# ilya16/isp-tts

Hardware: AMD Instinct MI355X
Metric: mel-frames/s (whole node), batch=64 x 512-frame utterances per GPU, full forward incl. MAS (higher is better)
Workload: dtype bf16; 1 GPU; BASELINE config 3: AcousticModel.forward (TextEncoder + Aligner/MAS + TemporalAdaptor 1 flow eval + MelDecoder + to_mel), fixed-length synthetic random-phoneme batch, random-init weights of the recipe architecture (23.2 M params); batch_per_gpu=64, global_batch=64, text_len=100, mel_len=512, parallelism=single GPU, device=gfx950:sramecc+:xnack-, compute_units=256, launch=HIP graph replay, batches_in_flight=1

## Files before the change

### include/ispk.h

```cpp
#ifndef ISPK_H
#define ISPK_H

#include <stdint.h>

#ifdef __cplusplus
extern "C" {
#endif

typedef struct ihipStream_t* ispk_stream_t;

#define ISPK_ABI_VERSION 2

#define ISPK_E_NULL (-1)
#define ISPK_E_SHAPE (-2)
#define ISPK_E_ALIGN (-3)
#define ISPK_E_UNSUPPORTED (-4)

int32_t ispk_abi_version(void);
const char* ispk_last_error_string(void);
int32_t ispk_device_info(char* name, int32_t cap);

int32_t ispk_mas_f32(const float* logits, const int64_t* text_len, const int64_t* mel_len, int16_t* attn_hard,
                     int64_t* dur, int16_t* path, int32_t B, int32_t M_max, int32_t L_max, int64_t stride_b,
                     int64_t stride_m, ispk_stream_t stream);
// ... 12 lines not shown
#define ISPK_EP_MASK_ACC 4u
#define ISPK_EP_MASK_OUT 8u
#define ISPK_EP_BIAS_ROW 16u
#define ISPK_EP_MASK_COL 32u
#define ISPK_EP_OUT_BF16 64u
#define ISPK_EP_RESID_BF16 128u
#define ISPK_EP_DUAL_GELU 1024u
#define ISPK_EP_GELU_BWD 2048u
#define ISPK_EP_OUT_SPLIT 512u
#define ISPK_EP_ROWS_T 256u

int32_t ispk_gemm_f32_tile(int32_t M, int32_t N, int32_t K);
int32_t ispk_gemm_f32(const float* A, int64_t lda, const float* W, int64_t ldw, float* C, int64_t ldc, const float* bias,
                      const float* resid, int64_t ldr, const uint8_t* mask, int32_t M, int32_t N, int32_t K,
                      uint32_t flags, int32_t cols_per_batch, int64_t batch_stride, ispk_stream_t stream);
int32_t ispk_gemm_f32_batched(const float* A, int64_t lda, int64_t stride_a, const float* W, int64_t ldw, int64_t stride_w,
                              float* C, int64_t ldc, int64_t stride_c, int32_t batch, int32_t M, int32_t N, int32_t K,
                              ispk_stream_t stream);
int32_t ispk_gemm_bf16_gelu_train(const uint16_t* A, int64_t lda, const uint16_t* W, int64_t ldw, uint16_t* u, int64_t ldu,
                                  uint16_t* a, int64_t ld_a, int32_t M, int32_t N, int32_t K, float dropout_p, uint64_t seed,
                                  ispk_stream_t stream);
int32_t ispk_gemm_bf16_gelu_bwd(const uint16_t* dY, int64_t lddy, const uint16_t* W2t, int64_t ldw, const uint16_t* u,
                                int64_t ldu, uint16_t* du, int64_t lddu, const uint8_t* row_mask, int32_t M, int32_t N,
                                int32_t K, float dropout_p, uint64_t seed, ispk_stream_t stream);
int32_t ispk_gemm_bf16_last_variant(void);
int32_t ispk_gemm_bf16(const uint16_t* A, int64_t lda, const uint16_t* W, int64_t ldw, void* C, int64_t ldc,
                       const float* bias, const void* resid, int64_t ldr, const uint8_t* mask, int32_t M, int32_t N,
                       int32_t K, uint32_t flags, int32_t cols_per_batch, int64_t batch_stride, ispk_stream_t stream);
int32_t ispk_gemm_bf16_splitk_plan(int32_t M, int32_t N, int32_t K, uint32_t flags);
int32_t ispk_gemm_bf16_splitk(const uint16_t* A, int64_t lda, const uint16_t* W, int64_t ldw, void* C, int64_t ldc,
                              const float* bias, const void* resid, int64_t ldr, const uint8_t* mask, int32_t M, int32_t N,
                              int32_t K, uint32_t flags, float* workspace, int32_t ksplit, ispk_stream_t stream);

int32_t ispk_ffn_bf16(const uint16_t* x, int64_t ldx, const uint16_t* W1, int64_t ldw1, const float* bias1,
                      const uint16_t* W2, int64_t ldw2, const float* bias2, const float* resid, int64_t ldr,
                      const uint8_t* mask, float* out, int64_t ldo, int32_t rows, int32_t dim, int32_t inner, uint32_t flags,
                      ispk_stream_t stream);

int32_t ispk_ffn_bf16_prenorm(const float* x, int64_t ldx, const float* norm_gamma, const float* norm_beta, float norm_eps,
                              const uint16_t* W1, int64_t ldw1, const uint16_t* W2_packed, const float* bias2,
                              const uint8_t* mask, float* out, int64_t ldo, int32_t rows, int32_t dim, int32_t inner,
                              uint32_t flags, float* row_stats, float stats_eps, ispk_stream_t stream);

int32_t ispk_ffn_chunk_w2_bf16(const uint16_t* W2, int64_t ldw2, int32_t dim, int32_t inner, uint16_t* out,
                               ispk_stream_t stream);
int32_t ispk_ffn_bf16_prenorm2_split(const float* x, int64_t ldx, const float* norm_gamma, const float* norm_beta,
                                     float norm_eps, const uint16_t* W1, const uint16_t* W2_chunks, float* parts,
                                     int64_t part_stride, int32_t splits, int32_t rows, int32_t dim, int32_t inner,
                                     ispk_stream_t stream);
int32_t ispk_ffn_combine_ln_f32(const float* x, int64_t ldx, const float* parts, int64_t part_stride, int32_t splits,
                                const uint8_t* mask, float* y, int64_t ldy, const float* ln_gamma, const float* ln_beta,
                                float ln_eps, int32_t ln_mask, void* ln_out, int64_t ld_ln, int32_t ln_bf16, int32_t rows,
                                int32_t dim, ispk_stream_t stream);
int32_t ispk_ffn_bf16_prenorm2(const float* x, int64_t ldx, const float* norm_gamma, const float* norm_beta, float norm_eps,
                               const uint16_t* W1, const uint16_t* W2_chunks, const uint8_t* mask, float* out, int64_t ldo,
                               int32_t rows, int32_t dim, int32_t inner, uint32_t flags, float* row_stats, float stats_eps,
                               ispk_stream_t stream);
int32_t ispk_attn_out_ffn_bf16(const float* x, int64_t ldx, const uint16_t* attn_out, int64_t ld_attn,
                               const uint16_t* Wo_chunks, const float* norm_gamma, const float* norm_beta, float norm_eps,
                               const uint16_t* W1, const uint16_t* W2_chunks, const uint8_t* mask, float* out, int64_t ldo,
                               int32_t rows, int32_t dim, int32_t inner, uint32_t flags, float* row_stats, float stats_eps,
                               ispk_stream_t stream);

int32_t ispk_attn_out_ffn_norm_bf16(const float* x, int64_t ldx, const uint16_t* attn_out, int64_t ld_attn,
                                    const uint16_t* Wo_chunks, const float* norm_gamma, const float* norm_beta, float norm_eps,
                                    const uint16_t* W1, const uint16_t* W2_chunks, const uint8_t* mask, float* out, int64_t ldo,
                                    int32_t rows, int32_t dim, int32_t inner, uint32_t flags, const float* final_gamma,
                                    const float* final_beta, float final_eps, int32_t ln_mask, void* ln_out, int64_t ld_ln,
                                    int32_t ln_bf16, ispk_stream_t stream);
int32_t ispk_attn_out_ffn_split_bf16(const float* x, int64_t ldx, const uint16_t* attn_out, int64_t ld_attn,
                                     const uint16_t* Wo_chunks, const float* norm_gamma, const float* norm_beta, float norm_eps,
                                     const uint16_t* W1, const uint16_t* W2_chunks, const uint8_t* mask, uint32_t flags,
                                     float* parts, int64_t part_stride, int32_t splits, int32_t rows, int32_t dim, int32_t inner,
                                     ispk_stream_t stream);
int32_t ispk_chunk_k16_bf16(const uint16_t* W, int64_t ldw, int32_t N, int32_t K, uint16_t* out, ispk_stream_t stream);
int32_t ispk_attn_out_ffn_qkv_bf16(const float* x, int64_t ldx, const uint16_t* attn_out, int64_t ld_attn,
                                   const uint16_t* Wo_chunks, const float* norm_gamma, const float* norm_beta, float norm_eps,
                                   const uint16_t* W1, const uint16_t* W2_chunks, const uint8_t* mask, float* out, int64_t ldo,
                                   int32_t rows, int32_t dim, int32_t inner, uint32_t flags, const float* next_gamma,
                                   const float* next_beta, float next_eps, const uint16_t* Wqkv_chunks, uint16_t* qkv,
                                   int64_t ld_qkv, ispk_stream_t stream);

int32_t ispk_gemm_bf16_lnin(const float* x, int64_t ldx, const float* row_stats, const float* ln_gamma, const float* ln_beta,
                            float ln_eps, const uint16_t* W, int64_t ldw, void* C, int64_t ldc, const float* bias, const void* resid,
                            int64_t ldr, const uint8_t* mask, int32_t M, int32_t N, int32_t K, uint32_t flags,
                            ispk_stream_t stream);

int32_t ispk_ffn_pack_w2_bf16(const uint16_t* W2, int64_t ldw2, int32_t dim, int32_t inner, uint16_t* packed,
                              ispk_stream_t stream);

int32_t ispk_linear_small_f32(const float* a, int64_t lda, const float* w, int64_t ldw, const float* bias,
                              const float* resid, int64_t ldr, float* out, int64_t ldo, int32_t M, int32_t N, int32_t K,
                              uint32_t act, ispk_stream_t stream);

int32_t ispk_alibi_mqa_attn_f32(const float* q, int64_t ldq, const float* k, const float* v, int64_t ldkv,
                                const float* slopes, const int64_t* key_len, float* out, int64_t ldo, int32_t B,
                                int32_t N, int32_t H, ispk_stream_t stream);
int32_t ispk_alibi_mqa_attn_bf16(const uint16_t* q, int64_t ldq, const uint16_t* k, const uint16_t* v, int64_t ldkv,
                                 const float* slopes, const int64_t* key_len, uint16_t* out, int64_t ldo, int32_t B,
                                 int32_t N, int32_t H, ispk_stream_t stream);
int32_t ispk_alibi_mqa_attn_bf16_tiles(const uint16_t* q, int64_t ldq, const uint16_t* k, const uint16_t* v, int64_t ldkv,
                                       const float* slopes, const int64_t* key_len, uint16_t* out, int64_t ldo, int32_t B,
                                       int32_t N, int32_t H, int32_t q_tiles_per_workgroup, ispk_stream_t stream);

int32_t ispk_attn_block_short_bf16(const uint16_t* x, int64_t ldx, const uint16_t* Wqkv_chunks, uint16_t* qkv, int64_t ld_qkv,
                                   const float* slopes, const int64_t* key_len, const uint16_t* Wo_chunks, const float* resid,
                                   int64_t ldr, const uint8_t* mask, float* out, int64_t ldo, int32_t B, int32_t N, int32_t H,
                                   ispk_stream_t stream);

int32_t ispk_pad_rows_f32(const float* x, int64_t stride_b, int64_t stride_t, int64_t stride_c, const int64_t* len,
                          void* out, int32_t out_bf16, int32_t B, int32_t T, int32_t C, ispk_stream_t stream);
int32_t ispk_masked_instnorm_f32(const float* y, const float* weight, const float* bias, const int64_t* len, void* out,
                                 int32_t out_bf16, int32_t B, int32_t T, int32_t C, float eps, ispk_stream_t stream);
int32_t ispk_aligner_scores_f32(const float* q_enc, int64_t q_stride_b, const float* k_enc, int64_t k_stride_b,
                                const int64_t* text_len, const int64_t* mel_len, float* attn_logits, float* attn_soft,
                                int32_t B, int32_t M, int32_t L, int32_t D, ispk_stream_t stream);
int32_t ispk_aligner_scores_fast_f32(const float* q_enc, int64_t q_stride_b, const float* k_enc, int64_t k_stride_b,
                                const int64_t* text_len, const int64_t* mel_len, float* attn_logits, float* attn_soft,
                                int32_t B, int32_t M, int32_t L, int32_t D, ispk_stream_t stream);
int32_t ispk_soft_average_f32(const float* attn_soft, const float* pitch, const float* energy, const int64_t* duration,
                              const int64_t* text_len, float* feats, int32_t B, int32_t M, int32_t L,
                              ispk_stream_t stream);

int32_t ispk_flow_head_f32(const float* y, int64_t ldy, const float* norm_gamma, const float* norm_beta, float norm_eps,
                           const float* W, const float* bias, const float* flow, const float* x0, const uint8_t* mask,
                           float* pred, float* duration, float* loss_ratio, float* loss_mean, float* workspace, int32_t B,
                           int32_t L, int32_t D, int32_t C, ispk_stream_t stream);
int32_t ispk_flow_euler_f32(const float* x_t, const float* velocity, float dt, const uint8_t* mask, float* out, int32_t B,
                            int32_t L, int32_t C, ispk_stream_t stream);
int32_t ispk_infer_features_f32(const float* pred, const float* duration_target_f32, const int64_t* duration_target_i64,
                                const float* pitch_target, const float* energy_target, float duration_factor, float pitch_factor,
                                float pitch_delta, float energy_factor, float energy_delta, float* duration, float* features,
                                int32_t B, int32_t L, ispk_stream_t stream);
int32_t ispk_infer_features_round_f32(const float* pred, const float* duration_target_f32, const int64_t* duration_target_i64,
                                      const float* pitch_target, const float* energy_target, float duration_factor,
                                      float pitch_factor, float pitch_delta, float energy_factor, float energy_delta,
                                      float* duration, float* features, int32_t B, int32_t L, ispk_stream_t stream);
int32_t ispk_infer_features_items_f32(const float* pred, const float* duration_target_f32, const int64_t* duration_target_i64,
                                      const float* pitch_target, const float* energy_target, const float* controls,
                                      int32_t round, float* duration, float* features, int64_t* frames_wanted, int32_t B,
                                      int32_t L, ispk_stream_t stream);
int32_t ispk_infer_features_tokens_f32(const float* pred, const float* duration_target_f32, const int64_t* duration_target_i64,
                                       const float* pitch_target, const float* energy_target, const float* controls,
                                       int32_t round, float* duration, float* features, int64_t* frames_wanted, int32_t B,
                                       int32_t L, ispk_stream_t stream);
int32_t ispk_flow_mix_f32(const float* x0, const float* x1, const float* t, float sigma, float* x_t, float* flow, int32_t B,
                          int32_t L, int32_t C, ispk_stream_t stream);
int32_t ispk_flow_finish_f32(const float* pred_raw, const float* flow, const float* x0, const uint8_t* mask, float* pred,
                             float* duration, float* loss_ratio, float* loss_mean, int32_t B, int32_t L, int32_t C,
                             ispk_stream_t stream);

int32_t ispk_embed_tokens_f32(const int64_t* text, const float* table, int64_t ld_table, int32_t vocab,
                              const int64_t* text_len, float* emb, uint8_t* mask, int32_t B, int32_t L, int32_t D,
                              ispk_stream_t stream);
int32_t ispk_embed_tokens_qkv(const int64_t* text, const float* table, int64_t ld_table, int32_t vocab, const int64_t* text_len,
                              float* emb, uint8_t* mask, const uint16_t* qkv_table, int64_t ld_qkv_table, uint16_t* qkv,
                              int32_t B, int32_t L, int32_t D, int32_t N, ispk_stream_t stream);
int32_t ispk_add_speaker_f32(float* x, const float* table, int64_t ld_table, int32_t speakers, const int64_t* speaker,
                             int32_t id_stride, int32_t B, int32_t L, int32_t D, ispk_stream_t stream);
int32_t ispk_add_speaker_out_f32(const float* x, float* out, const float* table, int64_t ld_table, int32_t speakers,
                                 const int64_t* speaker, int32_t id_stride, int32_t B, int32_t L, int32_t D, ispk_stream_t stream);
int32_t ispk_speaker_grad_f32(const float* d_x, const int64_t* speaker, int32_t id_stride, const int64_t* text_len,
                              float* workspace, int64_t workspace_floats, float* d_table, int64_t ld_table, int32_t speakers,
                              int32_t B, int32_t L, int32_t D, int32_t accumulate, ispk_stream_t stream);
int32_t ispk_time_embedding_f32(const float* t, int32_t n, const float* inv_freq, const float* freq_scale, int32_t half_dim,
                                const float* w0, const float* b0, const float* w1, const float* b1, int32_t emb_dim,
                                float* out, ispk_stream_t stream);
int32_t ispk_length_regulate_f32(const float* alignment, const float* dur_f32, const int64_t* dur_i64, const int64_t* enc_len,
                                 const float* x, int64_t ldx, float* out, int64_t* dec_len, uint8_t* dec_mask, int32_t B,
                                 int32_t M, int32_t L, int32_t D, int32_t max_len, int32_t dur_cols, ispk_stream_t stream);
int32_t ispk_length_regulate_split_bf16(const float* alignment, const float* dur_f32, const int64_t* dur_i64, const int64_t* enc_len,
                                 const float* x, int64_t ldx, float* out, int64_t* dec_len, uint8_t* dec_mask, int32_t B,
                                 int32_t M, int32_t L, int32_t D, int32_t max_len, int32_t dur_cols, ispk_stream_t stream);
int32_t ispk_length_regulate_qkv_bf16(const float* alignment, const float* dur_f32, const int64_t* dur_i64, const int64_t* enc_len,
                                      const float* x, int64_t ldx, float* out, int64_t* dec_len, uint8_t* dec_mask,
                                      const float* norm_gamma, const float* norm_beta, float norm_eps, const uint16_t* Wqkv_chunks,
                                      uint16_t* qkv, int64_t ld_qkv, int32_t B, int32_t M, int32_t L, int32_t D, int32_t max_len,
                                      int32_t dur_cols, ispk_stream_t stream);
int32_t ispk_length_regulate_split_f16(const float* alignment, const float* dur_f32, const int64_t* dur_i64, const int64_t* enc_len,
                                const float* x, int64_t ldx, float* out, int64_t* dec_len, uint8_t* dec_mask, int32_t B,
                                int32_t M, int32_t L, int32_t D, int32_t max_len, int32_t dur_cols, ispk_stream_t stream);

int32_t ispk_hard_regulate_f32(const float* dur_f32, const int64_t* dur_i64, const float* x, int64_t ldx, float* out,
                               int64_t* dec_len, uint8_t* dec_mask, int32_t B, int32_t frames, int32_t L, int32_t D,
                               int32_t max_len, ispk_stream_t stream);
int32_t ispk_hard_regulate_bwd_f32(const float* dur_f32, const int64_t* dur_i64, const float* d_out, float* d_x, int32_t B,
                                   int32_t rows, int32_t L, int32_t D, int32_t max_len, ispk_stream_t stream);
int32_t ispk_hard_average_f32(const float* pitch, const float* energy, const int64_t* duration, const int64_t* text_len,
                              float* feats, int32_t B, int32_t M, int32_t L, ispk_stream_t stream);

int32_t ispk_transpose_f32(const float* x, int64_t ldx, float* y, int64_t ldy, int32_t rows, int32_t cols,
                           ispk_stream_t stream);
int32_t ispk_gemm_tn_f32(const float* A, int64_t lda, const float* B, int64_t ldb, float* C, int64_t ldc, int32_t M,
                         int32_t N1, int32_t N2, const uint8_t* row_mask, int32_t accumulate, float* workspace,
                         int64_t workspace_floats, ispk_stream_t stream);
int32_t ispk_gemm_tn_bf16(const float* A, int64_t lda, const float* B, int64_t ldb, float* C, int64_t ldc, int32_t M,
                          int32_t N1, int32_t N2, const uint8_t* row_mask, int32_t accumulate, float* workspace,
                          int64_t workspace_floats, ispk_stream_t stream);
int32_t ispk_gemm_tn_b16(const uint16_t* A, int64_t lda, const uint16_t* B, int64_t ldb, float* C, int64_t ldc, int32_t M,
                         int32_t N1, int32_t N2, const uint8_t* row_mask, int32_t accumulate, float* workspace,
// ... 229 lines not shown
```

### isp_tts_amd/acoustic/alignment.py

```python
from __future__ import annotations

from collections.abc import Sequence
from typing import NamedTuple, Optional

import torch
import torch.nn as nn
from torch import Tensor

from .. import runtime
from ..staging import StagedWeights
from ..modules.aligner import mas_device
from ..modules.constructor import Constructor


_NOT_A_PATH = ("{} only owns parameters (the reference's state_dict names); its arithmetic runs inside the fused HIP "
               "kernels that ConvAttention launches (csrc/aligner.hip) - there is no PyTorch/MIOpen path to fall back to")


class MaskedInstanceNorm1d(nn.Module):

    def __init__(self, num_features: int, eps: float = 1e-5):
        super().__init__()
        self.eps = eps
        self.weight = nn.Parameter(torch.ones(num_features))
# ... 22 lines not shown


class ConvAttention(nn.Module, Constructor):
    def __init__(self, mel_dim: int, text_dim: int = 512, attention_dim: int = 80, key_kernel_size: int = 3,
                 query_kernel_size=(3, 3), dropout: float = 0.0, normalization: Optional[str] = "instance",
                 activation: str = "relu", attention_prior: bool = True):
        super().__init__()
        self.mel_dim, self.text_dim = mel_dim, text_dim
        self.scale = attention_dim ** -0.5
        if isinstance(query_kernel_size, int):
            query_kernel_size = [query_kernel_size] * 2
        self.key_proj = nn.ModuleList([
            ConvBlock1D(text_dim, text_dim * 2, key_kernel_size, activation, normalization, bias=False),
            ConvBlock1D(text_dim * 2, attention_dim, 1, "linear", None, bias=False)])
        self.query_proj = nn.ModuleList([
            ConvBlock1D(mel_dim, mel_dim * 2, query_kernel_size[0], activation, normalization, bias=False),
            ConvBlock1D(mel_dim * 2, mel_dim, query_kernel_size[1], activation, normalization, bias=False),
            ConvBlock1D(mel_dim, attention_dim, 1, "linear", None, bias=False)])
        self.attention_prior = attention_prior
        self.compute_dtype = torch.float32
        self._cache = StagedWeights()

    def _staged(self):
        ps = [c.conv.weight for c in list(self.key_proj) + list(self.query_proj)]
        dt = self.compute_dtype

        def build():
            if dt == torch.float16:
                w2d = [runtime.split_f16(p.detach().permute(0, 2, 1).reshape(p.shape[0], -1).float().contiguous()) for p in ps]
            else:
                w2d = [p.detach().permute(0, 2, 1).reshape(p.shape[0], -1).to(dt).contiguous() for p in ps]
            return w2d[:2], w2d[2:]
        return self._cache.get(dt, ps, build)

    def project_queries(self, queries: Tensor, query_len: Tensor) -> Tensor:
        _, wq = self._staged()
        gelu, dt = runtime.EP_GELU, self.compute_dtype
        if dt == torch.float16:
            q = runtime.pad_rows(queries.float(), query_len, channel_first=True, out_dtype=dt)
            for i in (0, 1):
                q = runtime.conv5_padded_split(q, wq[i], gelu)
                q = runtime.masked_instnorm(q, self.query_proj[i].norm.weight, self.query_proj[i].norm.bias, query_len,
                                            out_dtype=dt)
            return runtime.conv5_padded_split(q, wq[2])
        q = runtime.pad_rows(queries.float(), query_len, channel_first=True, out_dtype=dt)
        q = runtime.conv5_padded(q, wq[0], gelu)
        q = runtime.masked_instnorm(q, self.query_proj[0].norm.weight, self.query_proj[0].norm.bias, query_len,
                                    out_dtype=dt)
        q = runtime.conv5_padded(q, wq[1], gelu)
        q = runtime.masked_instnorm(q, self.query_proj[1].norm.weight, self.query_proj[1].norm.bias, query_len,
                                    out_dtype=dt)
        return runtime.conv5_padded(q, wq[2])

    def forward(self, queries: Tensor, keys: Tensor, query_len: Tensor, key_len: Tensor, q_proj: Optional[Tensor] = None):
        if not self.attention_prior:
            raise NotImplementedError("the aligner is built with its diagonal prior (recipes: attention_prior default)")
        wk, _ = self._staged()
        max_q, max_k = queries.shape[2], keys.shape[2]
        gelu, dt = runtime.EP_GELU, self.compute_dtype
        if dt == torch.float16:
            k = runtime.pad_rows(keys.float(), key_len, channel_first=True, out_dtype=dt)
            k = runtime.conv5_padded_split(k, wk[0], gelu)
            k = runtime.masked_instnorm(k, self.key_proj[0].norm.weight, self.key_proj[0].norm.bias, key_len, out_dtype=dt)
            k = runtime.conv5_padded_split(k, wk[1])
            q = q_proj if q_proj is not None else self.project_queries(queries, query_len)
            return runtime.aligner_scores(q, k, key_len, query_len, max_q, max_k)
        k = runtime.pad_rows(keys.float(), key_len, channel_first=True, out_dtype=dt)
        k = runtime.conv5_padded(k, wk[0], gelu)
        k = runtime.masked_instnorm(k, self.key_proj[0].norm.weight, self.key_proj[0].norm.bias, key_len, out_dtype=dt)
        k = runtime.conv5_padded(k, wk[1])
        q = q_proj if q_proj is not None else self.project_queries(queries, query_len)
        return runtime.aligner_scores(q, k, key_len, query_len, max_q, max_k, fast=dt == torch.bfloat16)


class AlignerOutput(NamedTuple):
    attn_soft: Tensor
    attn_logits: Tensor
    attn_hard: Tensor
    attn_hard_duration: Tensor


class Aligner(nn.Module, Constructor):
    def __init__(self, mel_dim: int, text_dim: int = 512, attention_dim: int = 80, key_kernel_size: int = 3,
                 query_kernel_size=(3, 3), dropout: float = 0.0, normalization: Optional[str] = "instance",
                 activation: str = "relu", attention_prior: bool = True):
        super().__init__()
        self.attention = ConvAttention(mel_dim=mel_dim, text_dim=text_dim, attention_dim=attention_dim,
                                       key_kernel_size=key_kernel_size, query_kernel_size=query_kernel_size,
                                       dropout=dropout, normalization=normalization, activation=activation,
                                       attention_prior=attention_prior)

    def forward(self, mel: Tensor, enc_text: Tensor, mel_len: Tensor, text_len: Tensor,
                q_proj: Optional[Tensor] = None, mas_stream=None) -> AlignerOutput:
        attn_soft, attn_logits = self.attention(mel, enc_text, mel_len, text_len, q_proj=q_proj)
        if mas_stream is not None and attn_logits.is_cuda:
            mas_stream.wait_stream(torch.cuda.current_stream())
            with torch.cuda.stream(mas_stream):
                attn_hard, dur = self.binarize_attention_parallel(attn_logits, text_len, mel_len, return_duration=True)
            attn_logits.record_stream(mas_stream)
        else:
            attn_hard, dur = self.binarize_attention_parallel(attn_logits, text_len, mel_len, return_duration=True)
        return AlignerOutput(attn_soft=attn_soft, attn_logits=attn_logits, attn_hard=attn_hard, attn_hard_duration=dur)

    @torch.no_grad()
    def binarize_attention_parallel(self, attn_logits: Tensor, text_len: Tensor, mel_len: Tensor,
                                    return_duration: bool = False):
        hard, dur, _ = mas_device(attn_logits.detach(), text_len, mel_len, want_dur=return_duration)
        return (hard, dur) if return_duration else hard
```

### isp_tts_amd/acoustic/model.py

```python
from __future__ import annotations

import warnings
from typing import NamedTuple, Optional

import torch
import torch.nn as nn
import torch.nn.functional as F
from torch import Tensor

from .. import runtime
from ..staging import StagedWeights
from ..modules.constructor import Constructor
from ..modules.transformer import Transformer
from ..modules.transformer.plan import Hand, Handed
from ..utils import get_mask_from_lengths
from .alignment import Aligner, AlignerOutput
from .temporal_adaptor import FlowTemporalAdaptor, TemporalAdaptorOutput


class AcousticModelOutput(NamedTuple):
    mel: Tensor
    adaptor_output: TemporalAdaptorOutput
    aligner_output: AlignerOutput
    loss: Optional[Tensor] = None
    losses: Optional[dict] = None


class AcousticModel(nn.Module, Constructor):
    def __init__(self, encoding_map: dict, mel_dim: int, text_dim: int = 384, encoder=None, decoder=None,
                 temporal_adaptor=None, aligner=None, num_speakers: Optional[int] = 0, pitch_mean=None, pitch_std=None,
                 speaker_in_forward: bool = False):
        super().__init__()
        self.encoding_map = dict(encoding_map)
        self.mel_dim, self.text_dim = mel_dim, text_dim
        self.text_embedding = nn.Embedding(len(encoding_map), text_dim, padding_idx=0)
        self.encoder = Transformer.init(encoder, emb_dim=text_dim)
        enc_dim = self.encoder.dim
        self.aligner = Aligner.init(aligner, mel_dim=mel_dim, text_dim=enc_dim)
        self.speaker_embedding = None
        if (num_speakers or 0) > 0:
            self.speaker_embedding = nn.Embedding(num_speakers, enc_dim)
            nn.init.xavier_uniform_(self.speaker_embedding.weight)
        self.speaker_in_forward = bool(speaker_in_forward)
        self.train_amp: Optional[bool] = None
        self.temporal_adaptor = FlowTemporalAdaptor.init(temporal_adaptor, encoder_dim=enc_dim)
        self.decoder = Transformer.init(decoder, emb_dim=enc_dim)
        self.to_mel = nn.Linear(self.decoder.dim, mel_dim)
        self.token_qkv_table = True
        self.overlap_streams = True
        self._side_streams: dict = {}
        self.register_buffer("pitch_mean", torch.tensor(float(pitch_mean or 0.)))
        self.register_buffer("pitch_std", torch.tensor(float(pitch_std or 1.)))
        self.compute_dtype = torch.float32
        self._cache = StagedWeights()

    def set_compute_dtype(self, dtype: torch.dtype, *, alignment_dtype: Optional[torch.dtype] = None):
        chain = alignment_dtype if alignment_dtype is not None else dtype
        assert chain in (torch.float32, torch.bfloat16, torch.float16)
        self.encoder.set_compute_dtype(chain)
        self.decoder.set_compute_dtype(dtype)
        self.temporal_adaptor.predictor.transformer.set_compute_dtype(dtype)
        self.temporal_adaptor.embedding.transformer.set_compute_dtype(dtype)
        self.aligner.attention.compute_dtype = chain
        self.temporal_adaptor.length_regulator.split_bf16 = (True if dtype == torch.bfloat16 else
                                                             "f16" if dtype == torch.float16 else False)
        self.compute_dtype = dtype
        return self

    def _to_mel(self, dec_out: Tensor, dec_mask: Optional[Tensor]) -> Tensor:
        w = self.to_mel.weight
        if dec_out.dtype == torch.float16:
            ws = self._cache.get(torch.float16, (w,), lambda: runtime.split_f16(w.detach().float().contiguous()))
            return runtime.to_mel_split(dec_out, ws, self.to_mel.bias, dec_mask)
        if dec_out.dtype == torch.bfloat16:
            w = self._cache.get(torch.bfloat16, (w,), lambda: w.detach().to(torch.bfloat16).contiguous())
        return runtime.to_mel(dec_out, w, self.to_mel.bias, dec_mask)

    def _embed(self, text: Tensor, text_len: Optional[Tensor], want_mask: bool = True):
        table, enc = self.text_embedding.weight, self.encoder
        first = enc.layers[0]
        norm, att = first.attention_norm, first.attention
        if not (self.token_qkv_table and text.is_cuda and att.compute_dtype == torch.bfloat16 and not first.adaptive_norm
                and norm.weight is not None and norm.bias is not None and isinstance(enc.project_emb, nn.Identity)
                and (att.heads * 64 + 128) % 8 == 0):
            return (*runtime.embed_tokens(text, table, text_len, want_mask=want_mask), Handed())

        def build():
            with torch.no_grad():
                rows = runtime.layernorm(table.detach().float().contiguous(), norm.weight, norm.bias, eps=norm.eps,
                                         out_dtype=torch.bfloat16)
                return runtime.gemm(rows, att._staged(torch.bfloat16)[0])
        qkv_table = self._cache.get("token_qkv", (table, norm.weight, norm.bias, att.to_q.weight, att.to_kv.weight), build)
        emb, mask, qkv = runtime.embed_tokens_qkv(text, table, qkv_table, text_len, want_mask=want_mask)
        return emb, mask, Handed(Hand.QKV, qkv)

    def _decoder_first(self):
        dec = self.decoder
        first = dec.layers[0]
        norm, att = first.attention_norm, first.attention
        ok = (att.compute_dtype == torch.bfloat16 and not first.adaptive_norm and norm.weight is not None and norm.bias is not None
              and isinstance(dec.project_emb, nn.Identity) and dec.dim == 384 and att.heads * 64 + 128 == 512)
        return first if ok else None

    def _decoder_handed(self) -> Handed:
        qkv = self.temporal_adaptor.length_regulator.qkv
        return Handed(Hand.QKV, qkv) if qkv is not None else Handed()

    def forward(self, text: Tensor, text_len: Tensor, mel: Tensor, mel_len: Tensor, pitch: Optional[Tensor] = None,
                energy: Optional[Tensor] = None, speaker: Optional[Tensor] = None, sigma: float = 0., steps: int = 1, *,
                flow_noise: Optional[Tensor] = None, flow_time: Optional[Tensor] = None) -> AcousticModelOutput:
        if self.speaker_embedding is None:
            speaker = None
        elif not self.speaker_in_forward:
            raise AttributeError(f"'{type(self).__name__}' object has no attribute 'speaker_encoder'")
        elif speaker is None:
            raise ValueError("speaker_in_forward is on and the model has a speaker table: forward() needs `speaker` "
                             "([B, 1] int64 ids, or a single id for the whole batch)")
        if torch.is_grad_enabled() and text.is_cuda and any(p.requires_grad for p in self.parameters()):
            from ..train.model import acoustic_train_outputs
            amp = self.train_amp if self.train_amp is not None else torch.is_autocast_enabled("cuda")
            train_aligner = any(p.requires_grad for p in self.aligner.parameters())
            with torch.autocast("cuda", enabled=False):
                return acoustic_train_outputs(self, text, text_len, mel, mel_len, pitch, energy, flow_noise, flow_time, amp=amp,
                                              train_aligner=train_aligner, speaker=speaker)
        with torch.no_grad():
            return self._forward_values(text, text_len, mel, mel_len, pitch, energy, flow_noise=flow_noise, flow_time=flow_time,
                                        speaker=speaker)

    def _forward_values(self, text: Tensor, text_len: Tensor, mel: Tensor, mel_len: Tensor, pitch: Optional[Tensor] = None,
                        energy: Optional[Tensor] = None, *, flow_noise: Optional[Tensor] = None,
                        flow_time: Optional[Tensor] = None, speaker: Optional[Tensor] = None) -> AcousticModelOutput:
        q_proj = None
        if mel.is_cuda and self.overlap_streams:
            main = torch.cuda.current_stream()
            side = self._side_streams.setdefault(mel.device, torch.cuda.Stream(device=mel.device))
            side.wait_stream(main)
            with torch.cuda.stream(side):
                q_proj = self.aligner.attention.project_queries(mel, mel_len)
        token_emb, enc_mask, handed = self._embed(text, text_len)
        enc_out = self.encoder(token_emb, mask=enc_mask, key_len=text_len, handed=handed).out
        if q_proj is not None:
            main.wait_stream(side)
            q_proj.record_stream(main)
        branch = side if q_proj is not None else None
        hard = not self.temporal_adaptor.soft_duration
        aligner_output = self.aligner(mel=mel, enc_text=enc_out.transpose(1, 2).detach(), mel_len=mel_len,
                                      text_len=text_len, q_proj=q_proj, mas_stream=None if hard else branch)
        if speaker is not None:
            enc_out = runtime.add_speaker(enc_out, self.speaker_embedding.weight, speaker)
        adaptor_output = self.temporal_adaptor(
            enc_out=enc_out, enc_mask=enc_mask, max_dec_len=mel.size(2),
            duration_target=aligner_output.attn_hard_duration, alignment=aligner_output.attn_soft,
            pitch_target_dense=pitch, energy_target_dense=energy, noise=flow_noise, time_steps=flow_time,
            enc_len=text_len, predictor_stream=branch, duration_sum=mel_len if branch is not None and not hard else None,
            qkv_for=self._decoder_first())
        dec_len = adaptor_output.dec_lengths
        dec_mask = adaptor_output.dec_mask
        dec_out = self.decoder(adaptor_output.enc_out, mask=dec_mask, key_len=dec_len, out_dtype=self.compute_dtype,
                               handed=self._decoder_handed()).out
        mel_out = self._to_mel(dec_out, dec_mask)
        if q_proj is not None:
            main.wait_stream(side)
            for t in (adaptor_output.log_duration, adaptor_output.duration, adaptor_output.pitch, adaptor_output.energy,
                      aligner_output.attn_hard, aligner_output.attn_hard_duration, *(adaptor_output.losses or {}).values()):
                if isinstance(t, Tensor):
                    t.record_stream(main)
        return AcousticModelOutput(mel=mel_out, adaptor_output=adaptor_output, aligner_output=aligner_output)

    @torch.no_grad()
    def forward_front(self, text: Tensor, text_len: Tensor, mel: Tensor, mel_len: Tensor, pitch: Tensor, energy: Tensor):
        main = torch.cuda.current_stream()
        side = self._side_streams.setdefault(mel.device, torch.cuda.Stream(device=mel.device))
        side.wait_stream(main)
        with torch.cuda.stream(side):
            q_proj = self.aligner.attention.project_queries(mel, mel_len)
        token_emb, enc_mask, handed = self._embed(text, text_len)
        enc_out = self.encoder(token_emb, mask=enc_mask, key_len=text_len, handed=handed).out
        main.wait_stream(side)
        q_proj.record_stream(main)
        attn_soft, attn_logits = self.aligner.attention(mel, enc_out.transpose(1, 2).detach(), mel_len, text_len,
                                                        q_proj=q_proj)
        feats = runtime.soft_average(attn_soft, pitch, energy, None, text_len)
        return {"enc_out": enc_out, "enc_mask": enc_mask, "attn_soft": attn_soft, "attn_logits": attn_logits, "feats": feats}

    @torch.no_grad()
    def forward_side(self, st: dict, text_len: Tensor, mel_len: Tensor, pitch: Tensor, energy: Tensor,
                     flow_noise: Optional[Tensor], flow_time: Optional[Tensor]):
        attn_hard, dur = self.aligner.binarize_attention_parallel(st["attn_logits"], text_len, mel_len, return_duration=True)
        ad = self.temporal_adaptor
        targets = runtime.soft_average(st["attn_soft"], pitch, energy, dur, text_len)
        pred, losses = ad.predictor(st["enc_out"], targets, st["enc_mask"][..., None], noise=flow_noise, time_steps=flow_time,
                                    key_len=text_len)
        return {"attn_hard": attn_hard, "dur": dur, "pred": pred, "losses": losses,
                "duration_pred": ad.predictor._duration_estimate}

    @torch.no_grad()
    def forward_back(self, st: dict, text_len: Tensor, mel_len: Tensor, max_dec_len: int):
        ad = self.temporal_adaptor
        feats = st["feats"]
        x = ad.embedding(feats[..., 1:3], mask=st["enc_mask"][..., None], key_len=text_len, residual=st["enc_out"])
        dec_in, dec_len = ad.length_regulator(x, mel_len.view(-1, 1), max_len=max_dec_len, alignment=st["attn_soft"],
                                              qkv_for=self._decoder_first())
        dec_mask = ad.length_regulator.dec_mask
        dec_out = self.decoder(dec_in, mask=dec_mask, key_len=dec_len, out_dtype=self.compute_dtype,
                               handed=self._decoder_handed()).out
        return {"mel": self._to_mel(dec_out, dec_mask), "dec_in": dec_in, "dec_len": dec_len, "dec_mask": dec_mask}

    @staticmethod
# ... 97 lines not shown
```

### isp_tts_amd/acoustic/temporal_adaptor.py

```python
from __future__ import annotations

from typing import NamedTuple, Optional

import torch
import torch.nn as nn
import torch.nn.functional as F
from torch import Tensor

from .. import runtime
from ..staging import StagedWeights
from ..modules.constructor import Constructor
from ..modules.transformer import Transformer, TimePositionalEmbedding
from ..utils import get_float_mask_from_lengths, get_mask_3d, masked_mean


class TransformerTemporalModule(nn.Module, Constructor):

    def __init__(self, input_dim: int = 256, output_dim: int = 256, transformer=None, detach_inputs: bool = False):
        super().__init__()
        self.transformer = Transformer.init(transformer, emb_dim=input_dim)
        for layer in self.transformer.layers:
            layer.attention.short_block = False
        self.linear_layer = nn.Linear(self.transformer.dim, output_dim, bias=True)
        self.detach_inputs = detach_inputs
        self._cache = StagedWeights()

    def _weight(self, dtype: torch.dtype) -> Tensor:
        w = self.linear_layer.weight
        if dtype == torch.float16:
            return self._cache.get(dtype, (w,), lambda: runtime.split_f16(w.detach().float().contiguous()))
        return self._cache.get(dtype, (w,), lambda: w.detach().to(dtype).contiguous())

    def forward(self, x: Tensor, mask: Optional[Tensor] = None, *, key_len: Optional[Tensor] = None,
                residual: Optional[Tensor] = None) -> Tensor:
        m2 = mask[..., 0] if mask is not None else None
        cdt = self.transformer.layers[0].attention.compute_dtype
        out = self.transformer(x, mask=m2, out_dtype=cdt, key_len=key_len if m2 is not None else None).out
        flags = runtime.EP_MASK_ACC if m2 is not None else 0
        if cdt == torch.float16:
            return runtime.gemm_split(out, self._weight(cdt), bias=self.linear_layer.bias, mask=m2, flags=flags, resid=residual)
        return runtime.gemm(out, self._weight(cdt), bias=self.linear_layer.bias, mask=m2, flags=flags, resid=residual,
                            out_dtype=torch.float32)

    def infer(self, x: Tensor, mask: Optional[Tensor] = None, steps: int = 4) -> Tensor:
        return self.forward(x, mask)


class FlowTransformerTemporalModule(nn.Module, Constructor):

    def __init__(self, input_dim: int = 256, output_dim: int = 256, transformer=None,
                 time_embedding_dim: Optional[int] = None, sigma: float = 1e-5, detach_inputs: bool = False):
        super().__init__()
        time_embedding_dim = time_embedding_dim or input_dim
        self.time_embedding = TimePositionalEmbedding(freq_dim=64, emb_dim=time_embedding_dim, with_steps=True)
        self.transformer = Transformer.init(transformer, emb_dim=output_dim + input_dim, adaptive_norm=True,
                                            condition_dim=time_embedding_dim)
        self.linear_layer = nn.Linear(self.transformer.dim, output_dim, bias=True)
        self.output_dim, self.sigma, self.detach_inputs = output_dim, sigma, detach_inputs
        self.fused_head = True
        self._cache = StagedWeights()
        self._grids: dict = {}

    def _cond_weight(self, dtype: torch.dtype) -> Tensor:
        w = self.transformer.project_emb.weight
        if dtype == torch.float16:
            return self._cache.get(dtype, (w,), lambda: runtime.split_f16(w.detach()[:, self.output_dim:].float().contiguous()))
        return self._cache.get(dtype, (w,), lambda: w.detach()[:, self.output_dim:].to(dtype).contiguous())

    def _project(self, x_t: Tensor, cond_proj: Tensor) -> Tensor:
        w = self.transformer.project_emb.weight
        return runtime.linear_small(x_t.contiguous(), w[:, :self.output_dim], None, resid=cond_proj)

    def _cond_projection(self, cond: Tensor) -> Tensor:
        cdt = self.transformer.layers[0].attention.compute_dtype
        c = cond.float().contiguous()
        if cdt == torch.float16:
            return runtime.gemm_split(runtime.split_f16(c), self._cond_weight(cdt), bias=self.transformer.project_emb.bias)
        if cdt == torch.bfloat16:
            c = runtime.cast_bf16(c)
        return runtime.gemm(c, self._cond_weight(cdt), bias=self.transformer.project_emb.bias, out_dtype=torch.float32)

    def forward(self, x: Tensor, targets: Tensor, mask: Optional[Tensor] = None, *, noise: Optional[Tensor] = None,
                time_steps: Optional[Tensor] = None, key_len: Optional[Tensor] = None):
        cond = x
        have_mask = mask is not None
        if mask is None:
            mask = torch.ones(x.shape[:2], dtype=torch.bool, device=x.device)
        elif mask.ndim == 3:
            mask = mask[..., 0]
        x1 = targets.detach()
        x0 = torch.randn_like(x1) if noise is None else noise.to(x1)
        t = torch.rand((x1.shape[0],), dtype=x1.dtype, device=x1.device) if time_steps is None else time_steps.to(x1)
        time_emb = self.time_embedding(t)
        x_t, flow = runtime.flow_mix(x0, x1, t, self.sigma)
        proj = self._project(x_t, self._cond_projection(cond))
        tr = self.transformer
        head = (self.fused_head and tr.dim == 256 and self.output_dim == 3 and tr.norm.weight is not None and tr.norm.bias is not None
                and self.linear_layer.bias is not None)
        out = tr(None, mask=mask, adaptive_condition=time_emb, projected=proj, key_len=key_len if have_mask else None,
                 final_norm=not head).out
        if head:
            pred, self._duration_estimate, _, loss = runtime.flow_head(out, tr.norm.weight, tr.norm.bias, tr.norm.eps,
                                                                       self.linear_layer.weight, self.linear_layer.bias, flow, x0, mask)
            return pred, {"flow_loss": loss}
        raw = runtime.linear_small(out, self.linear_layer.weight, self.linear_layer.bias)
        pred, self._duration_estimate, _, loss = runtime.flow_finish(raw, flow, x0, mask)
        return pred, {"flow_loss": loss}

    def euler_grid(self, steps: int, step_factor: float, device=None) -> Tensor:
        assert step_factor <= 1.
        key = (int(steps), float(step_factor))
        grid = self._grids.get(key)
        if grid is None:
            if step_factor == 1.:
                grid = torch.linspace(0, 1, steps + 1)
            else:
                ts = -torch.diff(torch.logspace(0, steps, steps + 1, base=step_factor))
                ts = torch.cat([torch.zeros(1), ts])
                grid = torch.cumsum(ts / ts.sum(), dim=0)
            self._grids[key] = grid
        return grid if device is None else grid.to(device)

    def infer(self, x: Tensor, mask: Optional[Tensor] = None, steps: int = 4, step_factor: float = 0.75, *,
              noise: Optional[Tensor] = None, key_len: Optional[Tensor] = None) -> Tensor:
        dev = x.device
        if mask is not None and mask.ndim == 3:
            mask = mask.squeeze(-1)
        x_t = (torch.randn(x.shape[0], x.shape[1], self.output_dim, device=dev) if noise is None
               else noise.to(device=dev, dtype=torch.float32))
        dts = self._grids.get(("dt", int(steps), float(step_factor)))
        if dts is None:
            ts = self.euler_grid(steps, step_factor)
            dts = self._grids[("dt", int(steps), float(step_factor))] = (ts[1:] - ts[:-1]).tolist()
        temb = self.time_embedding(self._grid_on(dev, steps, step_factor)[:steps])
        cond_proj = self._cond_projection(x)
        if mask is not None and key_len is None:
            key_len = mask.sum(dim=1)
        for i in range(steps):
            out = self.transformer(None, mask=mask, adaptive_condition=temb[i].view(1, 1, -1),
                                   projected=self._project(x_t, cond_proj), key_len=key_len).out
            vel = runtime.linear_small(out, self.linear_layer.weight, self.linear_layer.bias)
            x_t = runtime.flow_euler(x_t, vel, dts[i], mask if i == steps - 1 else None)
        return x_t

    def _grid_on(self, device, steps: int, step_factor: float) -> Tensor:
        key = (str(device), int(steps), float(step_factor))
        g = self._grids.get(key)
        if g is None:
# ... 26 lines not shown
            if frames is None:
                frames = int((durations.float() + 0.5).long().sum(dim=1).max().item())
            if max_len is not None:
                frames = min(frames, max_len)
            if frames == 0:
                self.dec_mask = torch.zeros((x.shape[0], 0), dtype=torch.bool, device=x.device)
                return x.new_zeros((x.shape[0], 0, x.shape[2])), torch.zeros((x.shape[0],), dtype=torch.int64, device=x.device)
            out, dec_lens, self.dec_mask = runtime.hard_regulate(x.float(), durations, frames,
                                                                 max_len=-1 if max_len is None else max_len)
            return out, dec_lens
        rows = alignment.shape[1] if alignment is not None else frames
        if max_len is not None and alignment is not None:
            rows = min(rows, max_len)
            alignment = alignment[:, :rows]
        if self.hand_qkv and qkv_for is not None and self.split_bf16 is True and x.is_cuda and x.shape[-1] == 384:
            norm, att = qkv_for.attention_norm, qkv_for.attention
            out, dec_lens, self.dec_mask, self.qkv = runtime.length_regulate(
                x.float(), durations, alignment, rows, max_len=-1 if max_len is None else max_len, enc_len=enc_len,
                split_bf16=True, next_qkv=(norm.weight, norm.bias, norm.eps, att._chunked_wqkv()))
            return out, dec_lens
        out, dec_lens, self.dec_mask = runtime.length_regulate(x.float(), durations, alignment, rows,
                                                               max_len=-1 if max_len is None else max_len, enc_len=enc_len,
                                                               split_bf16=self.split_bf16)
        return out, dec_lens


class TemporalAverager(nn.Module):

    def forward(self, x: Tensor, durations: Tensor, alignment: Optional[Tensor] = None) -> Tensor:
        if alignment is None:
            b, c, _ = x.shape
            if durations.dtype != torch.int64:
                ends = torch.cumsum(durations, dim=1).long()
                durations = torch.diff(ends, dim=1, prepend=torch.zeros_like(ends[:, :1]))
            every = torch.full((b,), durations.shape[1], dtype=torch.int64, device=x.device)
            cols = []
            for i in range(0, c, 2):
                f = runtime.hard_average(x[:, i], x[:, min(i + 1, c - 1)], durations, every)
                cols.append(f[..., 1:min(3, 1 + c - i)])
            return torch.cat(cols, dim=-1).transpose(1, 2)
        return x @ alignment / (alignment.sum(dim=1, keepdim=True) + 1e-5)


def generate_soft_path(duration: Tensor, mask: Tensor) -> Tensor:
    b, t_x, t_y = mask.shape
    cum = torch.cumsum(duration, 1).view(b * t_x)
    path = get_float_mask_from_lengths(cum, t_y).to(mask.dtype).view(b, t_x, t_y)
    path = path - F.pad(path, [0, 0, 1, 0, 0, 0])[:, :-1]
    return path * mask


class FlowTemporalAdaptor(nn.Module, Constructor):
    predictor_first = False

    def __init__(self, encoder_dim: int = 384, predictor=None, embedding=None, pitch: bool = True, energy: bool = True,
                 soft_duration: bool = False):
        super().__init__()
        if not (pitch and energy):
            raise NotImplementedError("built with pitch and energy both on (either duration mode): without one of them the "
                                      "feature tensors change shape")
        self.length_regulator = LengthRegulator()
        self.averager = TemporalAverager()
        self.encoder_dim = encoder_dim
        self.feature_dim = 3
        self.pitch, self.energy, self.soft_duration = pitch, energy, soft_duration
        self.pitch_idx, self.energy_idx = 1, 2
        self.predictor = FlowTransformerTemporalModule.init(predictor, input_dim=encoder_dim, output_dim=self.feature_dim)
        self.embedding = TransformerTemporalModule.init(embedding, input_dim=self.feature_dim - 1, output_dim=encoder_dim)

    def _process_target(self, dense: Tensor, duration_target: Tensor, alignment: Tensor, enc_mask: Tensor) -> Tensor:
        if dense.ndim == 2:
            dense = dense[:, None]
        return self.averager(dense, duration_target, alignment).transpose(1, 2) * enc_mask

    def forward(self, enc_out: Tensor, enc_mask: Tensor, max_dec_len: int, duration_target: Optional[Tensor] = None,
                alignment: Optional[Tensor] = None, pitch_target_dense: Optional[Tensor] = None,
                energy_target_dense: Optional[Tensor] = None, *, noise: Optional[Tensor] = None,
                time_steps: Optional[Tensor] = None, enc_len: Optional[Tensor] = None,
                predictor_stream=None, duration_sum: Optional[Tensor] = None, qkv_for=None) -> TemporalAdaptorOutput:
        assert duration_target is not None and (alignment is not None or not self.soft_duration)
        assert pitch_target_dense is not None and energy_target_dense is not None
        hard = not self.soft_duration
        m3 = enc_mask[..., None]
        if enc_len is None:
            enc_len = enc_mask.sum(dim=1)
        side = predictor_stream if (predictor_stream is not None and enc_out.is_cuda) else None
        cond = enc_out
        if hard:
            alignment = None
            targets = runtime.hard_average(pitch_target_dense, energy_target_dense, duration_target, enc_len)
            feats = targets
            len_src = duration_target
        elif side is None or duration_sum is None:
            targets = runtime.soft_average(alignment, pitch_target_dense, energy_target_dense, duration_target, enc_len)
            feats = targets
            len_src = duration_target
        else:
            feats = runtime.soft_average(alignment, pitch_target_dense, energy_target_dense, None, enc_len)
            targets = None
            len_src = duration_sum.view(-1, 1)
        if side is not None:
            ready = torch.cuda.Event()
            ready.record()
        pitch_target, energy_target = feats[..., 1:2], feats[..., 2:3]
        features = feats[..., 1:3]

        def decoder_input(enc_out_):
            enc_out_ = self.embedding(features, mask=m3, key_len=enc_len, residual=enc_out_)
            return self.length_regulator(enc_out_, len_src, max_len=max_dec_len, alignment=alignment,
                                         frames=max_dec_len if hard else None, qkv_for=qkv_for)

        if not (side is not None and self.predictor_first):
            enc_out, dec_lens = decoder_input(enc_out)

        def predict():
            tg = targets
            if tg is None:
                tg = runtime.soft_average(alignment, pitch_target_dense, energy_target_dense, duration_target, enc_len)
            pred_, losses_ = self.predictor(cond, tg, m3, noise=noise, time_steps=time_steps, key_len=enc_len)
            return pred_, losses_, self.predictor._duration_estimate

        if side is not None:
            side.wait_event(ready)
            with torch.cuda.stream(side):
                pred, losses, duration_pred = predict()
            for t in (cond, feats, alignment, pitch_target_dense, energy_target_dense):
                if t is not None:
                    t.record_stream(side)
            if self.predictor_first:
                enc_out, dec_lens = decoder_input(enc_out)
        else:
            pred, losses, duration_pred = predict()
        log_duration_pred = pred[..., 0]
        return TemporalAdaptorOutput(enc_out=enc_out, log_duration=log_duration_pred, duration=duration_pred,
                                     dec_lengths=dec_lens, pitch=pred[..., 1], energy=pred[..., 2],
                                     pitch_target=pitch_target.squeeze(-1), energy_target=energy_target.squeeze(-1),
                                     losses=losses, dec_mask=self.length_regulator.dec_mask)

    def infer(self, enc_out: Tensor, enc_mask: Optional[Tensor] = None, duration_target: Optional[Tensor] = None,
              duration_factor: float = 1.0, pitch_target: Optional[Tensor] = None, pitch_factor: float = 1.0,
              pitch_delta: float = 0., energy_target: Optional[Tensor] = None, energy_factor: float = 1.0,
              energy_delta: float = 0., steps: int = 4, *, noise: Optional[Tensor] = None,
              max_dec_len: Optional[int] = None, enc_len: Optional[Tensor] = None, qkv_for=None,
              controls: Optional[Tensor] = None) -> TemporalAdaptorOutput:
        if controls is not None:
            return self._infer_items(enc_out, enc_mask, duration_target, pitch_target, energy_target, controls, steps, noise,
                                     max_dec_len, enc_len, qkv_for,
                                     (duration_factor, pitch_factor, pitch_delta, energy_factor, energy_delta))
        m3 = enc_mask[..., None] if enc_mask is not None else None
        pred = self.predictor.infer(enc_out, mask=m3, steps=steps, noise=noise, key_len=enc_len)
        duration_pred, feats = runtime.infer_features(pred, duration_target, pitch_target, energy_target, duration_factor,
                                                      pitch_factor, pitch_delta, energy_factor, energy_delta,
                                                      round_duration=not self.soft_duration)
        pitch, energy = feats[..., 0:1], feats[..., 1:2]
        enc_out = self.embedding(feats, residual=enc_out)
        enc_lens = enc_len
        if enc_lens is None and enc_mask is not None:
            enc_lens = enc_mask.sum(dim=1)
        if not self.soft_duration:
            enc_out, dec_lens = self.length_regulator(enc_out, duration_pred, alignment=None, frames=max_dec_len, hard=True)
            return TemporalAdaptorOutput(enc_out=enc_out, log_duration=None, duration=duration_pred, dec_lengths=dec_lens,
                                         pitch=pitch.squeeze(-1), energy=energy.squeeze(-1), pitch_target=pitch_target,
                                         energy_target=energy_target, dec_mask=self.length_regulator.dec_mask)
        if max_dec_len is None:
            max_dec_len = int((duration_pred.sum(dim=1) + 0.5).long().max().item())
        enc_out, dec_lens = self.length_regulator(enc_out, duration_pred, alignment=None, enc_len=enc_lens,
                                                  frames=max_dec_len, qkv_for=qkv_for)
        return TemporalAdaptorOutput(enc_out=enc_out, log_duration=None, duration=duration_pred, dec_lengths=dec_lens,
                                     pitch=pitch.squeeze(-1), energy=energy.squeeze(-1), pitch_target=pitch_target,
                                     energy_target=energy_target, dec_mask=self.length_regulator.dec_mask)

    frames_wanted: Optional[Tensor] = None

    def _infer_items(self, enc_out, enc_mask, duration_target, pitch_target, energy_target, controls, steps, noise, max_dec_len,
                     enc_len, qkv_for, scalars) -> TemporalAdaptorOutput:
        if tuple(float(v) for v in scalars) != (1.0, 1.0, 0.0, 1.0, 0.0):
            raise ValueError("infer: with `controls` the scalar controls stay at their defaults (duration_factor, pitch_factor, "
                             f"pitch_delta, energy_factor, energy_delta = 1, 1, 0, 1, 0), got {tuple(scalars)}")
        per_token = controls.ndim == 3
# ... 28 lines not shown
```

### isp_tts_amd/bindings/adaptor.py

```python
from typing import Optional

import torch
from torch import Tensor

from .. import runtime as _rt

__all__ = ["mas", "pad_rows", "conv5_padded", "masked_instnorm", "aligner_scores", "soft_average", "flow_mix", "flow_finish",
           "flow_head", "flow_euler", "infer_features", "infer_features_items", "infer_features_tokens", "embed_tokens", "embed_tokens_qkv", "_speaker_ids", "add_speaker_",
           "add_speaker", "speaker_grad", "time_embedding", "length_regulate", "_hard_durations", "hard_regulate",
           "hard_regulate_bwd", "hard_average"]


def mas(logits: Tensor, text_len: Tensor, mel_len: Tensor, want_dur: bool = True, want_path: bool = False):
    _rt._dev(logits, text_len, mel_len)
    assert logits.dtype == torch.float32 and logits.ndim == 3
    if logits.stride(2) != 1:
        logits = logits.contiguous()
    B, M, L = logits.shape
    text_len = _rt._i64(text_len)
    mel_len = _rt._i64(mel_len)
    hard = torch.empty((B, M, L), dtype=torch.int16, device=logits.device)
    dur = torch.empty((B, L), dtype=torch.int64, device=logits.device) if want_dur else None
    path = torch.empty((B, M), dtype=torch.int16, device=logits.device) if want_path else None
    _rt._launch(f"mas_kernel<{(L + 63) // 64}>", 0.0, 6.0 * B * M * L, _rt.lib().ispk_mas_f32, logits.data_ptr(),
                text_len.data_ptr(), mel_len.data_ptr(), hard.data_ptr(), _rt._ptr(dur), _rt._ptr(path), B, M, L, logits.stride(0),
                logits.stride(1), _rt._stream())
    return hard, dur, path


def pad_rows(x: Tensor, lengths: Tensor, channel_first: bool = False, out_dtype: torch.dtype = torch.float32) -> Tensor:
    _rt._dev(x, lengths)
    assert x.dtype == torch.float32 and x.ndim == 3
    if channel_first:
        B, C, T = x.shape
        sb, sc, st = x.stride()
    else:
        B, T, C = x.shape
        sb, st, sc = x.stride()
    lengths = _rt._i64(lengths)
    split = out_dtype == torch.float16
    out = torch.empty((2, B, T + 4, C) if split else (B, T + 4, C), dtype=out_dtype, device=x.device)
    _rt._launch("pad_rows_kernel", 0.0, 8.0 * B * T * C, _rt.lib().ispk_pad_rows_f32, x.data_ptr(), sb, st, sc,
                lengths.data_ptr(), out.data_ptr(), 2 if split else int(out_dtype == torch.bfloat16), B, T, C, _rt._stream())
    return out


def conv5_padded(xpad: Tensor, w2d: Tensor, flags: int = 0) -> Tensor:
    _rt._dev(xpad, w2d)
    B, TP, C = xpad.shape
    O, K = w2d.shape
    taps = K // C
    assert taps * C == K and taps in (1, 5) and xpad.is_contiguous() and w2d.is_contiguous()
    assert xpad.dtype == w2d.dtype
    bf16 = xpad.dtype == torch.bfloat16
    out = torch.empty((B, TP, O), dtype=torch.float32, device=xpad.device)
    a_ptr = xpad.data_ptr() + (0 if taps == 5 else 2 * C * xpad.element_size())
    M = B * TP - 4
    fn = _rt.lib().ispk_gemm_bf16 if bf16 else _rt.lib().ispk_gemm_f32
    _rt._launch(_rt._gemm_label(bf16, M, O, K), 2.0 * M * O * K, float(xpad.element_size()) * (M * C + O * K) + 4.0 * M * O, fn,
                a_ptr, C, w2d.data_ptr(), K, out.data_ptr(), O, None, None, 0, None, M, O, K, flags, 0, 0, _rt._stream())
    return out


def masked_instnorm(y: Tensor, weight: Tensor, bias: Tensor, lengths: Tensor, eps: float = 1e-5,
                    out_dtype: torch.dtype = torch.float32) -> Tensor:
    _rt._dev(y, weight, bias, lengths)
    B, TP, C = y.shape
    split = out_dtype == torch.float16
    out = torch.empty((2, *y.shape) if split else y.shape, dtype=out_dtype, device=y.device)
    lengths = _rt._i64(lengths)
    _rt._launch("masked_instnorm_kernel", 0.0, 16.0 * B * TP * C, _rt.lib().ispk_masked_instnorm_f32, y.data_ptr(),
                weight.data_ptr(), bias.data_ptr(), lengths.data_ptr(), out.data_ptr(), 2 if split else int(out_dtype == torch.bfloat16), B,
                TP - 4, C, eps, _rt._stream())
    return out


def aligner_scores(q_enc: Tensor, k_enc: Tensor, text_len: Tensor, mel_len: Tensor, M: int, L: int, fast: bool = False):
    _rt._dev(q_enc, k_enc, text_len, mel_len)
    B, D = q_enc.shape[0], q_enc.shape[2]
    logits = torch.empty((B, M, L), dtype=torch.float32, device=q_enc.device)
    soft = torch.empty((B, M, L), dtype=torch.float32, device=q_enc.device)
    text_len = _rt._i64(text_len)
    mel_len = _rt._i64(mel_len)
    _rt._launch("aligner_scores_kernel<bf16x3>" if fast else "aligner_scores_kernel", 2.0 * B * M * L * D, 4.0 * B * (M * D + L * D + 2 * M * L),
                _rt.lib().ispk_aligner_scores_fast_f32 if fast else _rt.lib().ispk_aligner_scores_f32, q_enc.data_ptr(), q_enc.stride(0),
                k_enc.data_ptr(), k_enc.stride(0), text_len.data_ptr(), mel_len.data_ptr(), logits.data_ptr(), soft.data_ptr(), B, M, L, D,
                _rt._stream())
    return soft, logits


def soft_average(attn_soft: Tensor, pitch: Tensor, energy: Tensor, duration: Optional[Tensor], text_len: Tensor) -> Tensor:
    _rt._dev(attn_soft, pitch, energy, duration, text_len)
    B, M, L = attn_soft.shape
    feats = torch.empty((B, L, 3), dtype=torch.float32, device=attn_soft.device)
    dur = _rt._i64(duration)
    if B == 0:
        return feats
    _rt._launch("soft_average_kernel", 0.0, 4.0 * B * M * L, _rt.lib().ispk_soft_average_f32, attn_soft.contiguous().data_ptr(),
                pitch.contiguous().data_ptr(), energy.contiguous().data_ptr(), _rt._ptr(dur),
                _rt._i64(text_len).data_ptr(), feats.data_ptr(), B, M, L, _rt._stream())
    return feats


def flow_mix(x0: Tensor, x1: Tensor, t: Tensor, sigma: float):
    _rt._dev(x0, x1, t)
    B, L, C = x1.shape
    x0c, x1c, tc = x0.float().contiguous(), x1.float().contiguous(), t.float().contiguous()
    xt, flow = torch.empty_like(x1c), torch.empty_like(x1c)
    if B == 0:
        return xt, flow
    _rt._launch("flow_mix_kernel", 0.0, 16.0 * B * L * C, _rt.lib().ispk_flow_mix_f32, x0c.data_ptr(), x1c.data_ptr(), tc.data_ptr(),
                float(sigma), xt.data_ptr(), flow.data_ptr(), B, L, C, _rt._stream())
    return xt, flow


def flow_finish(pred_raw: Tensor, flow: Tensor, x0: Tensor, mask: Tensor):
    _rt._dev(pred_raw, flow, x0, mask)
    B, L, C = pred_raw.shape
    assert mask.dtype == torch.bool and mask.shape == (B, L)
    pr, fl, x0c, mk = pred_raw.float().contiguous(), flow.contiguous(), x0.float().contiguous(), mask.contiguous()
    pred = torch.empty_like(pr)
    dur = torch.empty((B, L), dtype=torch.float32, device=pr.device)
    ratio = torch.empty((B,), dtype=torch.float32, device=pr.device)
    loss = torch.empty((), dtype=torch.float32, device=pr.device)
    if B == 0:
        return pred, dur, ratio, loss.fill_(float("nan"))
    _rt._launch("flow_finish_kernel", 0.0, 20.0 * B * L * C, _rt.lib().ispk_flow_finish_f32, pr.data_ptr(), fl.data_ptr(),
                x0c.data_ptr(), mk.data_ptr(), pred.data_ptr(), dur.data_ptr(), ratio.data_ptr(), loss.data_ptr(), B, L, C,
                _rt._stream())
    return pred, dur, ratio, loss


def flow_head(y: Tensor, norm_weight: Tensor, norm_bias: Tensor, norm_eps: float, weight: Tensor, bias: Tensor, flow: Tensor,
              x0: Tensor, mask: Tensor):
    _rt._dev(y, norm_weight, norm_bias, weight, bias, flow, x0, mask)
    B, L, D = y.shape
    C = weight.shape[0]
    assert y.dtype == torch.float32 and y.stride(2) == 1 and y.stride(0) == L * y.stride(1) and weight.shape == (C, D) and weight.is_contiguous()
    assert mask.dtype == torch.bool and mask.shape == (B, L)
    fl, x0c, mk = flow.contiguous(), x0.float().contiguous(), mask.contiguous()
    pred = torch.empty((B, L, C), dtype=torch.float32, device=y.device)
    dur = torch.empty((B, L), dtype=torch.float32, device=y.device)
    ratio = torch.empty((B,), dtype=torch.float32, device=y.device)
    loss = torch.empty((), dtype=torch.float32, device=y.device)
    if B == 0:
        return pred, dur, ratio, loss.fill_(float("nan"))
    ws = torch.empty((2 * B * ((L + 15) // 16),), dtype=torch.float32, device=y.device)
    _rt._launch("flow_head_kernels", 0.0, 4.0 * B * L * D, _rt.lib().ispk_flow_head_f32, y.data_ptr(), y.stride(1), norm_weight.data_ptr(),
                norm_bias.data_ptr(), float(norm_eps), weight.data_ptr(), bias.data_ptr(), fl.data_ptr(), x0c.data_ptr(), mk.data_ptr(),
                pred.data_ptr(), dur.data_ptr(), ratio.data_ptr(), loss.data_ptr(), ws.data_ptr(), B, L, D, C, _rt._stream())
    return pred, dur, ratio, loss


def flow_euler(x_t: Tensor, velocity: Tensor, dt: float, mask: Optional[Tensor] = None) -> Tensor:
# ... 295 lines not shown
```

### isp_tts_amd/bindings/layers.py

```python
from typing import Optional

import torch
from torch import Tensor

from .. import runtime as _rt

__all__ = ["layernorm", "ffn_pack_w2", "ffn_fused", "ffn_prenorm", "ffn_chunk_w2", "ffn_prenorm2", "chunk_k16", "attn_out_ffn",
           "ffn_prenorm2_split", "alibi_mqa_attention_raw", "alibi_mqa_attention", "attn_block_short", "split_f16", "layernorm_split", "_split_label",
           "gemm_split", "to_mel_split", "conv5_padded_split", "alibi_mqa_attention_split", "cast_bf16"]


def layernorm(x: Tensor, gamma: Optional[Tensor], beta: Optional[Tensor], ada_scale: Optional[Tensor] = None,
              ada_shift: Optional[Tensor] = None, rows_per_batch: int = 1, row_mask: Optional[Tensor] = None,
              eps: float = 1e-5, out_dtype: torch.dtype = torch.float32) -> Tensor:
    _rt._dev(x, gamma, beta, ada_scale, ada_shift, row_mask)
    assert x.dtype == torch.float32
    x2 = _rt._rows2d(x)
    rows, D = x2.shape
    y = torch.empty(x.shape, dtype=out_dtype, device=x.device)
    ada_stride = 0
    if ada_scale is not None:
        ada_scale = ada_scale.reshape(-1, D) if ada_scale.ndim != 2 else ada_scale
        if ada_scale.stride(1) != 1:
            ada_scale = ada_scale.contiguous()
# ... 111 lines not shown
                _rt._stream())
    return out


def attn_out_ffn(x: Tensor, attn_out: Tensor, woc: Tensor, norm_weight: Tensor, norm_bias: Tensor, w1: Tensor, w2c: Tensor,
                 mask: Optional[Tensor] = None, norm_eps: float = 1e-5, want_stats: bool = False, stats_eps: float = 1e-5,
                 next_qkv: Optional[tuple] = None, final_norm: Optional[tuple] = None, want_out: bool = True):
    _rt._dev(x, attn_out, woc, norm_weight, norm_bias, w1, w2c, mask)
    assert x.dtype == torch.float32 and attn_out.dtype == torch.bfloat16 and w1.dtype == torch.bfloat16
    assert woc.dtype == torch.bfloat16 and w2c.dtype == torch.bfloat16
    x2, o2 = _rt._rows2d(x), _rt._rows2d(attn_out)
    R, D = x2.shape
    Fi = w1.shape[0]
    assert o2.shape == (R, D) and woc.shape == (D // 32, D, 32) and woc.is_contiguous()
    assert w1.shape == (Fi, D) and w1.is_contiguous() and w2c.shape == (Fi // 32, D, 32) and w2c.is_contiguous()
    out = torch.empty((*x.shape[:-1], D), dtype=torch.float32, device=x.device)
    stats = torch.empty((R, 2), dtype=torch.float32, device=x.device) if want_stats else None
    flags = 0
    if mask is not None:
        mask = _rt._mask1d(mask)
        flags = _rt.EP_MASK_ACC | _rt.EP_MASK_OUT
    nb = x2.numel() * 4 + o2.numel() * 2 + (woc.numel() + w1.numel() + w2c.numel()) * 2 + out.numel() * 4 + (R * 8 if want_stats else 0)
    if final_norm is not None:
        assert not want_stats and next_qkv is None
        fw, fb, feps, fmask, fdtype = final_norm
        _rt._dev(fw, fb)
        assert fdtype in (torch.float32, torch.bfloat16)
        ln = torch.empty(x.shape, dtype=fdtype, device=x.device)
        outp = out if want_out else None
        _rt._launch("ffn2_bf16_kernel<50>", 4.0 * R * D * Fi + 2.0 * R * D * D,
                    float(nb - (0 if want_out else out.numel() * 4) + ln.numel() * ln.element_size()), _rt.lib().ispk_attn_out_ffn_norm_bf16,
                    x2.data_ptr(), x2.stride(0), o2.data_ptr(), o2.stride(0), woc.data_ptr(), norm_weight.data_ptr(), norm_bias.data_ptr(),
                    norm_eps, w1.data_ptr(), w2c.data_ptr(), _rt._ptr(mask), _rt._ptr(outp), D, R, D, Fi, flags, fw.data_ptr(), fb.data_ptr(), feps,
                    int(bool(fmask) and mask is not None), ln.data_ptr(), D, int(fdtype == torch.bfloat16), _rt._stream())
        return outp, ln
    if next_qkv is not None:
        assert not want_stats
        ng, nbeta, neps, wqc = next_qkv
        _rt._dev(ng, nbeta, wqc)
        assert wqc.dtype == torch.bfloat16 and wqc.shape == (D // 16, 512, 16) and wqc.is_contiguous()
        qkv = torch.empty((*x.shape[:-1], 512), dtype=torch.bfloat16, device=x.device)
        _rt._launch("ffn2_bf16_kernel<51>", 4.0 * R * D * Fi + 2.0 * R * D * D + 2.0 * R * D * 512, float(nb + wqc.numel() * 2 + R * 1024),
                    _rt.lib().ispk_attn_out_ffn_qkv_bf16, x2.data_ptr(), x2.stride(0), o2.data_ptr(), o2.stride(0), woc.data_ptr(),
                    norm_weight.data_ptr(), norm_bias.data_ptr(), norm_eps, w1.data_ptr(), w2c.data_ptr(), _rt._ptr(mask), out.data_ptr(), D,
                    R, D, Fi, flags, ng.data_ptr(), nbeta.data_ptr(), neps, wqc.data_ptr(), qkv.data_ptr(), 512, _rt._stream())
        return out, qkv
    _rt._launch("ffn2_bf16_kernel<50>", 4.0 * R * D * Fi + 2.0 * R * D * D, float(nb), _rt.lib().ispk_attn_out_ffn_bf16, x2.data_ptr(),
                x2.stride(0), o2.data_ptr(), o2.stride(0), woc.data_ptr(), norm_weight.data_ptr(), norm_bias.data_ptr(), norm_eps,
                w1.data_ptr(), w2c.data_ptr(), _rt._ptr(mask), out.data_ptr(), D, R, D, Fi, flags, _rt._ptr(stats), stats_eps, _rt._stream())
    return (out, stats) if want_stats else out


def ffn_prenorm2_split(x: Tensor, norm_weight: Tensor, norm_bias: Tensor, w1: Tensor, w2c: Tensor, mask: Optional[Tensor],
                       splits: int, next_norm: Optional[tuple] = None, norm_eps: float = 1e-5, attn_proj: Optional[tuple] = None):
    _rt._dev(x, norm_weight, norm_bias, w1, w2c, mask)
    assert x.dtype == torch.float32 and w1.dtype == torch.bfloat16 and w2c.dtype == torch.bfloat16
    x2 = _rt._rows2d(x)
    R, D = x2.shape
    Fi = w1.shape[0]
    parts = torch.empty((splits, R, D), dtype=torch.float32, device=x.device)
    if attn_proj is not None:
        o, woc = attn_proj
        _rt._dev(o, woc)
        o2 = _rt._rows2d(o)
        assert o.dtype == torch.bfloat16 and o2.shape == (R, D) and woc.dtype == torch.bfloat16 and woc.shape == (D // 32, D, 32)
        mflat = _rt._mask1d(mask)
        _rt._launch("ffn2_bf16_kernel<21>", (4.0 * R * D * Fi) + 2.0 * R * D * D * splits,
                    float((x2.numel() * 4 + o2.numel() * 2 + woc.numel() * 2) * splits + (w1.numel() + w2c.numel()) * 2 + splits * R * D * 4),
                    _rt.lib().ispk_attn_out_ffn_split_bf16, x2.data_ptr(), x2.stride(0), o2.data_ptr(), o2.stride(0), woc.data_ptr(),
                    norm_weight.data_ptr(), norm_bias.data_ptr(), norm_eps, w1.data_ptr(), w2c.data_ptr(), _rt._ptr(mflat),
                    _rt.EP_MASK_ACC if mflat is not None else 0, parts.data_ptr(), R * D, splits, R, D, Fi, _rt._stream())
    else:
        nbytes = x2.numel() * 4 * splits + (w1.numel() + w2c.numel()) * 2 + splits * R * D * 4
        _rt._launch("ffn2_bf16_kernel<20>", 4.0 * R * D * Fi, float(nbytes), _rt.lib().ispk_ffn_bf16_prenorm2_split, x2.data_ptr(),
                    x2.stride(0), norm_weight.data_ptr(), norm_bias.data_ptr(), norm_eps, w1.data_ptr(), w2c.data_ptr(),
                    parts.data_ptr(), R * D, splits, R, D, Fi, _rt._stream())
    y = torch.empty(x.shape, dtype=torch.float32, device=x.device)
    mask = _rt._mask1d(mask)
    ln = None
    nw = nb = None
    neps, nmask, nbf16 = 1e-5, 0, 0
    if next_norm is not None:
        nw, nb, neps, apply_mask, ndtype = next_norm
        ln = torch.empty(x.shape, dtype=ndtype, device=x.device)
        nmask, nbf16 = int(bool(apply_mask) and mask is not None), int(ndtype == torch.bfloat16)
    _rt._launch("ffn_combine_ln_kernel", 0.0, float(R * D * 4 * (2 + splits) + (R * D * ln.element_size() if ln is not None else 0)),
                _rt.lib().ispk_ffn_combine_ln_f32, None if attn_proj is not None else x2.data_ptr(), x2.stride(0), parts.data_ptr(), R * D,
                splits, _rt._ptr(mask), y.data_ptr(),
                D, _rt._ptr(nw), _rt._ptr(nb), neps, nmask, _rt._ptr(ln), D, nbf16, R, D, _rt._stream())
    return y, ln


def alibi_mqa_attention_raw(q: Tensor, ldq: int, k: Tensor, v: Tensor, ldkv: int, slopes: Tensor,
                            key_len: Optional[Tensor], B: int, N: int, heads: int, q_tiles: int = 0) -> Tensor:
    _rt._dev(q, k, v, slopes, key_len)
    out = torch.empty((B, N, heads * 64), dtype=q.dtype, device=q.device)
    if B == 0:
        return out
    key_len = _rt._i64(key_len)
    slopes = slopes.to(torch.float32).contiguous()
    es = q.element_size()
    if es == 4:
        label = "attn_f32_kernel" + ("<384,16>" if heads <= 3 else "<768>" if heads <= 6 else "<1024>")
    else:
        label = "attn_bf16_kernel" + ("<768>" if heads <= 6 else "<1024>")
    flops, nbytes = 256.0 * B * N * N * heads, float(B) * N * (2 * heads * 64 + 128) * es
    if q_tiles:
        assert es == 2
        _rt._launch(label, flops, nbytes, _rt.lib().ispk_alibi_mqa_attn_bf16_tiles, q.data_ptr(), ldq, k.data_ptr(), v.data_ptr(),
                    ldkv, slopes.data_ptr(), _rt._ptr(key_len), out.data_ptr(), heads * 64, B, N, heads, q_tiles, _rt._stream())
        return out
    fn = _rt.lib().ispk_alibi_mqa_attn_f32 if es == 4 else _rt.lib().ispk_alibi_mqa_attn_bf16
    _rt._launch(label, flops, nbytes, fn, q.data_ptr(), ldq, k.data_ptr(), v.data_ptr(), ldkv,
                slopes.data_ptr(), _rt._ptr(key_len), out.data_ptr(), heads * 64, B, N, heads, _rt._stream())
    return out


def alibi_mqa_attention(qkv: Tensor, heads: int, slopes: Tensor, key_len: Optional[Tensor], q_tiles: int = 0) -> Tensor:
    B, N, W = qkv.shape
    assert W == heads * 64 + 128 and qkv.is_contiguous()
    return _rt.alibi_mqa_attention_raw(qkv, W, qkv[..., heads * 64:], qkv[..., heads * 64 + 64:], W, slopes, key_len, B, N,
                                       heads, q_tiles)


def attn_block_short(x: Optional[Tensor], wqkv_c: Optional[Tensor], qkv: Optional[Tensor], heads: int, slopes: Tensor,
                     key_len: Optional[Tensor], wo_c: Tensor, resid: Tensor, mask: Optional[Tensor]):
    _rt._dev(x, wqkv_c, qkv, slopes, key_len, wo_c, resid, mask)
    D = heads * 64
    src = x if x is not None else qkv
    B, N = src.shape[:2]
    assert (x is None) != (qkv is None) and src.dim() == 3 and src.dtype == torch.bfloat16 and src.is_contiguous()
    assert resid.dtype == torch.float32 and resid.shape == (B, N, D) and resid.is_contiguous()
    assert wo_c.dtype == torch.bfloat16 and wo_c.shape == (D // 16, D, 16) and wo_c.is_contiguous()
    if x is not None:
        assert x.shape == (B, N, D) and wqkv_c.dtype == torch.bfloat16 and wqkv_c.shape == (D // 16, D + 128, 16) and wqkv_c.is_contiguous()
        qkv = torch.empty((B, N, D + 128), dtype=torch.bfloat16, device=x.device)
    else:
        assert qkv.shape == (B, N, D + 128)
# ... 141 lines not shown
```

### isp_tts_amd/csrc/aligner.hip

```cpp
#include "common.h"
#include "dec_len.h"

namespace {

template <typename T_> __device__ __forceinline__ void put(T_* p, float v);
template <> __device__ __forceinline__ void put<float>(float* p, float v) { *p = v; }
template <> __device__ __forceinline__ void put<uint16_t>(uint16_t* p, float v) { *p = f32_to_bf16(v); }
__device__ __forceinline__ void put_split(_Float16* p, float v, int64_t plane) {
    v = __builtin_amdgcn_fmed3f(v, -65504.0f, 65504.0f);
    const _Float16 hi = (_Float16)v;
    p[0] = hi;
    p[plane] = (_Float16)(v - (float)hi);
}
template <typename OutT> __device__ __forceinline__ void put_any(OutT* p, float v, int64_t plane) {
    if constexpr (std::is_same<OutT, _Float16>::value) put_split(p, v, plane);
    else put<OutT>(p, v);
}

template <typename OutT>
__global__ __launch_bounds__(256) void pad_rows_kernel(const float* __restrict__ x, int64_t sb, int64_t st, int64_t sc,
                                                       const int64_t* __restrict__ len, OutT* __restrict__ out, int T,
                                                       int C, int64_t total, int64_t plane) {
    const int64_t idx = (int64_t)blockIdx.x * 256 + threadIdx.x;
    if (idx >= total) return;
    const int c = (int)(idx % C);
    const int64_t row = idx / C;
    const int tp = (int)(row % (T + 4)), b = (int)(row / (T + 4));
    const int t = tp - 2;
    float v = 0.f;
    if (t >= 0 && t < T && t < (int)len[b]) v = x[b * sb + t * st + c * sc];
    put_any<OutT>(out + idx, v, plane);
}

template <typename OutT>
__global__ __launch_bounds__(256) void pad_rows_cf_kernel(const float* __restrict__ x, int64_t sb, int64_t sc,
                                                          const int64_t* __restrict__ len, OutT* __restrict__ out, int T,
                                                          int C, int64_t plane) {
    __shared__ float tile[32][33];
    const int tx = threadIdx.x, ty = threadIdx.y, b = blockIdx.z;
    const int tp0 = blockIdx.x * 32, c0 = blockIdx.y * 32;
    int n = (int)len[b];
    n = n < T ? n : T;
#pragma unroll
    for (int k = 0; k < 4; ++k) {
        const int c = c0 + ty + 8 * k, t = tp0 + tx - 2;
        tile[ty + 8 * k][tx] = (c < C && t >= 0 && t < n) ? x[b * sb + c * sc + t] : 0.f;
    }
    __syncthreads();
#pragma unroll
    for (int k = 0; k < 4; ++k) {
        const int tp = tp0 + ty + 8 * k, c = c0 + tx;
        if (tp < T + 4 && c < C) put_any<OutT>(out + ((int64_t)b * (T + 4) + tp) * C + c, tile[tx][ty + 8 * k], plane);
    }
}
// ... 241 lines not shown
        }
    smax = fmaxf(smax, __shfl_xor(smax, 32, 64));
    float esum = 0.f;
#pragma unroll
    for (int kb_ = 0; kb_ < NB; ++kb_)
#pragma unroll
        for (int r = 0; r < 16; ++r) {
            const int key = kb_ * 32 + (r & 3) + 8 * (r >> 2) + 4 * h;
            if (key < tl) esum += as_exp<kFast>(s[kb_][r] - smax);
        }
    esum += __shfl_xor(esum, 32, 64);
    const float einv = (m < ml) ? 1.0f / esum : 0.f;

    float* lb = logits + (int64_t)b * M * L;
    float* sbp = soft + (int64_t)b * M * L;
    const int c = lane & 7;
    const bool vec = (L % 4) == 0;
#pragma unroll
    for (int kb_ = 0; kb_ < NB; ++kb_) {
#pragma unroll
        for (int pass = 0; pass < 2; ++pass) {
#pragma unroll
            for (int g = 0; g < 4; ++g) {
                float4 v;
                float* pv = &v.x;
#pragma unroll
                for (int e = 0; e < 4; ++e) {
                    const int key = kb_ * 32 + 8 * g + 4 * h + e;
                    const float lg = s[kb_][4 * g + e];
                    pv[e] = pass == 0 ? lg : (key < tl ? as_exp<kFast>(lg - smax) * einv : 0.f);
                }
                *reinterpret_cast<float4*>(stage + l31 * 144 + (8 * g + 4 * h) * 4) = v;
            }
            float* dst = pass == 0 ? lb : sbp;
#pragma unroll
            for (int i = 0; i < 4; ++i) {
                const int r = 8 * i + (lane >> 3), mm = m0 + r, key = kb_ * 32 + 4 * c;
                const float4 v = *reinterpret_cast<const float4*>(stage + r * 144 + c * 16);
                if (mm < M && key < L) {
                    float* o = dst + (int64_t)mm * L + key;
                    if (vec) {
                        *reinterpret_cast<float4*>(o) = v;
                    } else {
                        const float* pv = &v.x;
                        for (int e = 0; e < 4 && key + e < L; ++e) o[e] = pv[e];
                    }
                }
            }
        }
    }
}

constexpr int kSaLanes = 16;
__global__ __launch_bounds__(64 * kSaLanes) void soft_average_kernel(const float* __restrict__ attn,
                                                                     const float* __restrict__ pitch,
                                                                     const float* __restrict__ energy,
                                                                     const int64_t* __restrict__ dur,
                                                                     const int64_t* __restrict__ text_len,
                                                                     float* __restrict__ feats, int M, int L) {
    __shared__ float red[3][kSaLanes][64];
    const int b = blockIdx.y, j = threadIdx.x & 63, l = blockIdx.x * 64 + j, ml = threadIdx.x >> 6;
    const bool ok = l < L;
    const float* ab = attn + (int64_t)b * M * L;
    const float* pb = pitch + (int64_t)b * M;
    const float* eb = energy + (int64_t)b * M;
    float sa = 0.f, sp = 0.f, se = 0.f;
    if (ok) {
        int mm = ml;
        for (; mm + 7 * kSaLanes < M; mm += 8 * kSaLanes) {
            float a[8], pv[8], ev[8];
#pragma unroll
            for (int u = 0; u < 8; ++u) {
                a[u] = ab[(int64_t)(mm + u * kSaLanes) * L + l];
                pv[u] = pb[mm + u * kSaLanes];
                ev[u] = eb[mm + u * kSaLanes];
            }
#pragma unroll
            for (int u = 0; u < 8; ++u) {
                sa += a[u];
                sp = fmaf(pv[u], a[u], sp);
                se = fmaf(ev[u], a[u], se);
            }
        }
        for (; mm < M; mm += kSaLanes) {
            const float a = ab[(int64_t)mm * L + l];
            sa += a;
            sp = fmaf(pb[mm], a, sp);
            se = fmaf(eb[mm], a, se);
        }
    }
    red[0][ml][j] = sa;
    red[1][ml][j] = sp;
    red[2][ml][j] = se;
    __syncthreads();
    if (ml == 0 && ok) {
        float a = 0.f, pp = 0.f, ee = 0.f;
#pragma unroll
        for (int u = 0; u < kSaLanes; ++u) {
            a += red[0][u][j];
            pp += red[1][u][j];
            ee += red[2][u][j];
        }
        const float mk = l < (int)text_len[b] ? 1.0f : 0.0f;
        float* f = feats + ((int64_t)b * L + l) * 3;
        f[0] = dur ? log1pf((float)dur[(int64_t)b * L + l]) : 0.0f;
        f[1] = pp / (a + 1e-5f) * mk;
        f[2] = ee / (a + 1e-5f) * mk;
    }
}


__global__ __launch_bounds__(256) void flow_mix_kernel(const float* __restrict__ x0, const float* __restrict__ x1,
                                                       const float* __restrict__ t, float s, float* __restrict__ xt,
                                                       float* __restrict__ flow, int per_batch, int64_t total) {
#pragma clang fp contract(off)
    const int64_t i = (int64_t)blockIdx.x * 256 + threadIdx.x;
    if (i >= total) return;
    const float tb = t[i / per_batch], a = x0[i], b = x1[i];
    const float w0 = 1.0f - s * tb;
    const float p0 = w0 * a, p1 = tb * b;
    xt[i] = p0 + p1;
    const float sa = s * a;
    flow[i] = b - sa;
}

__global__ __launch_bounds__(1024) void flow_finish_kernel(const float* __restrict__ raw, const float* __restrict__ flow,
                                                           const float* __restrict__ x0, const uint8_t* __restrict__ mask,
                                                           float* __restrict__ pred, float* __restrict__ dur,
                                                           float* __restrict__ ratio, float* __restrict__ loss, int B, int L,
                                                           int C) {
    __shared__ float sratio[1024];
    const int tid = threadIdx.x, sub = tid & 15, grp = tid >> 4;
    const int n = L * C;
    for (int b0 = 0; b0 < B; b0 += 64) {
        const int b = b0 + grp;
        float num = 0.f, den = 0.f;
        if (b < B) {
            const float* rb = raw + (int64_t)b * n;
            const float* fb = flow + (int64_t)b * n;
            const float* xb = x0 + (int64_t)b * n;
            const uint8_t* mb = mask + (int64_t)b * L;
            float* pb = pred + (int64_t)b * n;
#pragma unroll 4
            for (int e = sub; e < n; e += 16) {
                const int l = e / C, c = e - l * C;
                const bool m = mb[l] != 0;
                const float r = rb[e], f = fb[e], x = xb[e];
                const float pf = m ? r : 0.f;
                const float pr = m ? x + pf : 0.f;
                pb[e] = pr;
                if (c == 0) dur[(int64_t)b * L + l] = fmaxf(expf(pr) - 1.0f, 0.f);
                const float d = pf - f;
                num += m ? d * d : 0.f;
                den += m ? 1.0f : 0.f;
            }
        }
#pragma unroll
        for (int off = 8; off > 0; off >>= 1) {
            num += __shfl_xor(num, off, 64);
            den += __shfl_xor(den, off, 64);
        }
        if (b < B && sub == 0) {
            const float q = num / fmaxf(den, 1e-5f);
            ratio[b] = q;
            if (b < 1024) sratio[b] = q;
        }
    }
    __syncthreads();
    if (loss && tid == 0) {
        float s = 0.f;
        if (B <= 1024) {
            for (int b = 0; b < B; ++b) s += sratio[b];
        } else {
            for (int b = 0; b < B; ++b) s += ratio[b];
        }
        loss[0] = s / (float)B;
// ... 261 lines not shown
    ISPK_REQUIRE(ispk_aligned(q_enc, 16) && ispk_aligned(k_enc, 16) && ispk_aligned(attn_logits, 16) &&
                     ispk_aligned(attn_soft, 16) && q_stride_b % 4 == 0 && k_stride_b % 4 == 0,
                 ISPK_E_ALIGN, "aligner_scores: 16-byte alignment required");
    if (B == 0) return 0;
    const int nb = (L + 31) / 32;
    size_t lds = (size_t)nb * 32 * kAD * 4;
    if (lds < kAsWaves * 32 * 144) lds = kAsWaves * 32 * 144;
    const float scale = 1.0f / sqrtf((float)D);
    dim3 grid((M + 32 * kAsWaves - 1) / (32 * kAsWaves), B), block(64 * kAsWaves);
    hipStream_t s = reinterpret_cast<hipStream_t>(stream);
#define ISPK_AL_CASE(NB)                                                                                              \
    case NB:                                                                                                          \
        if (fast) {                                                                                                   \
            ISPK_RESERVE_LDS((&aligner_scores_kernel<NB, true>), lds, "aligner_scores");                              \
            hipLaunchKernelGGL((aligner_scores_kernel<NB, true>), grid, block, lds, s, q_enc, q_stride_b, k_enc,      \
                               k_stride_b, text_len, mel_len, attn_logits, attn_soft, M, L, scale);                   \
        } else {                                                                                                      \
            ISPK_RESERVE_LDS((&aligner_scores_kernel<NB, false>), lds, "aligner_scores");                             \
            hipLaunchKernelGGL((aligner_scores_kernel<NB, false>), grid, block, lds, s, q_enc, q_stride_b, k_enc,     \
                               k_stride_b, text_len, mel_len, attn_logits, attn_soft, M, L, scale);                   \
        }                                                                                                             \
        break;
    switch (nb) {
        ISPK_AL_CASE(1) ISPK_AL_CASE(2) ISPK_AL_CASE(3) ISPK_AL_CASE(4) ISPK_AL_CASE(5) ISPK_AL_CASE(6) ISPK_AL_CASE(7)
        ISPK_AL_CASE(8) ISPK_AL_CASE(9) ISPK_AL_CASE(10)
        default: ISPK_FAIL(ISPK_E_SHAPE, "aligner_scores: unsupported L=%d", L);
    }
#undef ISPK_AL_CASE
    return ispk_launch_status();
}

extern "C" int32_t ispk_aligner_scores_f32(const float* q_enc, int64_t q_stride_b, const float* k_enc,
                                           int64_t k_stride_b, const int64_t* text_len, const int64_t* mel_len,
                                           float* attn_logits, float* attn_soft, int32_t B, int32_t M, int32_t L,
                                           int32_t D, ispk_stream_t stream) {
    return aligner_scores_launch(q_enc, q_stride_b, k_enc, k_stride_b, text_len, mel_len, attn_logits, attn_soft, B, M, L, D, stream,
                                 false);
}

extern "C" int32_t ispk_aligner_scores_fast_f32(const float* q_enc, int64_t q_stride_b, const float* k_enc,
                                                int64_t k_stride_b, const int64_t* text_len, const int64_t* mel_len,
                                                float* attn_logits, float* attn_soft, int32_t B, int32_t M, int32_t L,
                                                int32_t D, ispk_stream_t stream) {
    return aligner_scores_launch(q_enc, q_stride_b, k_enc, k_stride_b, text_len, mel_len, attn_logits, attn_soft, B, M, L, D, stream,
                                 true);
}

extern "C" int32_t ispk_soft_average_f32(const float* attn_soft, const float* pitch, const float* energy,
                                         const int64_t* duration, const int64_t* text_len, float* feats, int32_t B,
                                         int32_t M, int32_t L, ispk_stream_t stream) {
    ISPK_REQUIRE(attn_soft && pitch && energy && text_len && feats, ISPK_E_NULL, "soft_average: null pointer");
    ISPK_REQUIRE(B >= 0 && M >= 1 && L >= 1 && B <= 65535, ISPK_E_SHAPE, "soft_average: bad shape B=%d M=%d L=%d", B, M, L);
    if (B == 0) return 0;
    hipLaunchKernelGGL(soft_average_kernel, dim3((L + 63) / 64, B), dim3(64 * kSaLanes), 0, reinterpret_cast<hipStream_t>(stream),
                       attn_soft, pitch, energy, duration, text_len, feats, M, L);
    return ispk_launch_status();
}

extern "C" int32_t ispk_flow_mix_f32(const float* x0, const float* x1, const float* t, float sigma, float* x_t, float* flow,
                                     int32_t B, int32_t L, int32_t C, ispk_stream_t stream) {
    ISPK_REQUIRE(x0 && x1 && t && x_t && flow, ISPK_E_NULL, "flow_mix: null pointer");
    ISPK_REQUIRE(B >= 0 && L >= 1 && C >= 1, ISPK_E_SHAPE, "flow_mix: bad shape B=%d L=%d C=%d", B, L, C);
    if (B == 0) return 0;
    const int64_t total = (int64_t)B * L * C;
    const float s = (float)(1.0 - (double)sigma);
    hipLaunchKernelGGL(flow_mix_kernel, dim3((unsigned)((total + 255) / 256)), dim3(256), 0,
                       reinterpret_cast<hipStream_t>(stream), x0, x1, t, s, x_t, flow, L * C, total);
    return ispk_launch_status();
}

extern "C" int32_t ispk_flow_finish_f32(const float* pred_raw, const float* flow, const float* x0, const uint8_t* mask,
                                        float* pred, float* duration, float* loss_ratio, float* loss_mean, int32_t B,
                                        int32_t L, int32_t C, ispk_stream_t stream) {
    ISPK_REQUIRE(pred_raw && flow && x0 && mask && pred && duration && loss_ratio, ISPK_E_NULL, "flow_finish: null pointer");
    ISPK_REQUIRE(B >= 0 && L >= 1 && C >= 1 && B <= 65535, ISPK_E_SHAPE, "flow_finish: bad shape B=%d L=%d C=%d", B, L, C);
    if (B == 0) return 0;
    hipLaunchKernelGGL(flow_finish_kernel, dim3(1), dim3(1024), 0, reinterpret_cast<hipStream_t>(stream), pred_raw, flow, x0,
                       mask, pred, duration, loss_ratio, loss_mean, B, L, C);
    return ispk_launch_status();
}

extern "C" int32_t ispk_flow_head_f32(const float* y, int64_t ldy, const float* norm_gamma, const float* norm_beta, float norm_eps,
                                      const float* W, const float* bias, const float* flow, const float* x0, const uint8_t* mask,
                                      float* pred, float* duration, float* loss_ratio, float* loss_mean, float* workspace,
                                      int32_t B, int32_t L, int32_t D, int32_t C, ispk_stream_t stream) {
    ISPK_REQUIRE(y && norm_gamma && norm_beta && W && bias && flow && x0 && mask && pred && duration && loss_ratio && workspace,
                 ISPK_E_NULL, "flow_head: null pointer");
    ISPK_REQUIRE(D == 256 && C == 3, ISPK_E_UNSUPPORTED, "flow_head: built for dim 256 -> 3 flow channels (got %d -> %d)", D, C);
    ISPK_REQUIRE(B >= 0 && L >= 1 && B <= 65535 && ldy >= D && ldy % 4 == 0, ISPK_E_SHAPE, "flow_head: bad shape B=%d L=%d", B, L);
    ISPK_REQUIRE(ispk_aligned(y, 16) && ispk_aligned(norm_gamma, 16) && ispk_aligned(norm_beta, 16) && ispk_aligned(W, 16), ISPK_E_ALIGN,
                 "flow_head: y / gamma / beta / W must be 16-byte aligned");
    if (B == 0) return 0;
    const int nblk = (L + kFhRows - 1) / kFhRows;
    hipStream_t s = reinterpret_cast<hipStream_t>(stream);
    hipLaunchKernelGGL(flow_head_kernel, dim3(nblk, B), dim3(256), 0, s, y, ldy, norm_gamma, norm_beta, norm_eps, W, bias, flow, x0, mask,
                       pred, duration, workspace, L, nblk);
    if (int32_t rc = ispk_launch_status()) return rc;
    hipLaunchKernelGGL(flow_head_finalize_kernel, dim3(1), dim3(1024), 0, s, workspace, nblk, loss_ratio, loss_mean, B);
    return ispk_launch_status();
}

extern "C" int32_t ispk_flow_euler_f32(const float* x_t, const float* velocity, float dt, const uint8_t* mask, float* out,
                                       int32_t B, int32_t L, int32_t C, ispk_stream_t stream) {
    ISPK_REQUIRE(x_t && velocity && out, ISPK_E_NULL, "flow_euler: null pointer");
    ISPK_REQUIRE(B >= 0 && L >= 1 && C >= 1, ISPK_E_SHAPE, "flow_euler: bad shape B=%d L=%d C=%d", B, L, C);
    if (B == 0) return 0;
    const int64_t total = (int64_t)B * L * C;
    hipLaunchKernelGGL(flow_euler_kernel, dim3((unsigned)((total + 255) / 256)), dim3(256), 0,
                       reinterpret_cast<hipStream_t>(stream), x_t, velocity, dt, mask, out, C, total);
    return ispk_launch_status();
}

static int32_t infer_features_launch(const float* pred, const float* duration_target_f32, const int64_t* duration_target_i64,
                                     const float* pitch_target, const float* energy_target, float duration_factor,
                                     float pitch_factor, float pitch_delta, float energy_factor, float energy_delta,
                                     float* duration, float* features, int32_t B, int32_t L, ispk_stream_t stream, bool round) {
    ISPK_REQUIRE(pred && duration && features, ISPK_E_NULL, "infer_features: null pointer");
    ISPK_REQUIRE(!(duration_target_f32 && duration_target_i64), ISPK_E_UNSUPPORTED, "infer_features: one duration target at most");
    ISPK_REQUIRE(B >= 0 && L >= 1, ISPK_E_SHAPE, "infer_features: bad shape B=%d L=%d", B, L);
    if (B == 0) return 0;
// ... 71 lines not shown
```

### isp_tts_amd/csrc/ffn2.hip

```cpp
#include "common.h"

namespace {

constexpr int kD = 384, kHC = 32;
constexpr int kW1Row = kD * 2 + 16;
constexpr int kW1Dma = 25;
constexpr int kW1Bytes = kW1Dma * 1024;
constexpr int kW1Src = kHC * kD * 2;
constexpr int kW2Bytes = kD * kHC * 2;
constexpr int kWbuf = kW1Bytes + kW2Bytes;
constexpr int kDmaPerWave = 7;
constexpr int kPOff = 2 * kWbuf;
constexpr int kXcOff = kPOff + 2 * 4 * 2048;
constexpr int kLds = kXcOff + 2 * 8 * 2048;
constexpr int kXtOff = kWbuf;
constexpr int kLdT = 388;
static_assert(kXtOff + 128 * kD * 2 <= kLds && 64 * kLdT * 4 <= kLds, "LDS carve-up");

constexpr int kSplitMode = 20;
constexpr int kProjMode = 50;
constexpr int kSplitProjMode = 21;
constexpr int kProjQkvMode = 51;
constexpr int kProbeNoDma = 1;
constexpr int kProbeDmaOnly = 2;
// ... 740 lines not shown
        }
    }
}

__global__ __launch_bounds__(256) void ffn_chunk_w2_kernel(const uint16_t* __restrict__ W2, int64_t ldw2,
                                                           uint16_t* __restrict__ out, int dim, int inner) {
    const int64_t i = (int64_t)blockIdx.x * 256 + threadIdx.x;
    const int64_t total = (int64_t)dim * inner / 8;
    if (i >= total) return;
    const int piece = (int)(i & 3);
    const int64_t rest = i >> 2;
    const int d = (int)(rest % dim), c = (int)(rest / dim);
    *reinterpret_cast<u32x4*>(out + (((int64_t)c * dim + d) * 32 + piece * 8)) =
        *reinterpret_cast<const u32x4*>(W2 + (int64_t)d * ldw2 + c * 32 + piece * 8);
}

__global__ __launch_bounds__(256) void chunk_k16_kernel(const uint16_t* __restrict__ W, int64_t ldw, uint16_t* __restrict__ out,
                                                        int N, int K) {
    const int64_t i = (int64_t)blockIdx.x * 256 + threadIdx.x;
    const int64_t total = (int64_t)N * K / 8;
    if (i >= total) return;
    const int piece = (int)(i & 1);
    const int64_t rest = i >> 1;
    const int n = (int)(rest % N), c = (int)(rest / N);
    *reinterpret_cast<u32x4*>(out + (((int64_t)c * N + n) * 16 + piece * 8)) =
        *reinterpret_cast<const u32x4*>(W + (int64_t)n * ldw + c * 16 + piece * 8);
}

}

extern "C" int32_t ispk_chunk_k16_bf16(const uint16_t* W, int64_t ldw, int32_t N, int32_t K, uint16_t* out, ispk_stream_t stream) {
    ISPK_REQUIRE(W && out, ISPK_E_NULL, "chunk_k16: null pointer");
    ISPK_REQUIRE(N >= 1 && K >= 16 && K % 16 == 0 && ldw >= K, ISPK_E_SHAPE, "chunk_k16: bad shape %d x %d", N, K);
    ISPK_REQUIRE(ldw % 8 == 0 && ispk_aligned(W, 16) && ispk_aligned(out, 16), ISPK_E_ALIGN, "chunk_k16: 16-byte alignment required");
    const int64_t total = (int64_t)N * K / 8;
    hipLaunchKernelGGL(chunk_k16_kernel, dim3((unsigned)((total + 255) / 256)), dim3(256), 0, reinterpret_cast<hipStream_t>(stream),
                       W, ldw, out, N, K);
    return ispk_launch_status();
}

extern "C" int32_t ispk_ffn_chunk_w2_bf16(const uint16_t* W2, int64_t ldw2, int32_t dim, int32_t inner, uint16_t* out,
                                          ispk_stream_t stream) {
    ISPK_REQUIRE(W2 && out, ISPK_E_NULL, "ffn_chunk_w2: null pointer");
    ISPK_REQUIRE(dim >= 1 && inner >= 32 && inner % 32 == 0 && ldw2 >= inner, ISPK_E_SHAPE, "ffn_chunk_w2: bad shape %d x %d",
                 dim, inner);
    ISPK_REQUIRE(ldw2 % 8 == 0 && ispk_aligned(W2, 16) && ispk_aligned(out, 16), ISPK_E_ALIGN,
                 "ffn_chunk_w2: 16-byte alignment required");
    const int64_t total = (int64_t)dim * inner / 8;
    hipLaunchKernelGGL(ffn_chunk_w2_kernel, dim3((unsigned)((total + 255) / 256)), dim3(256), 0,
                       reinterpret_cast<hipStream_t>(stream), W2, ldw2, out, dim, inner);
    return ispk_launch_status();
}

template <typename TOut>
__global__ __launch_bounds__(256) void ffn_combine_ln_kernel(const float* __restrict__ x, int64_t ldx, const float* __restrict__ part,
                                                             int64_t part_stride, int splits, const uint8_t* __restrict__ mask,
                                                             float* __restrict__ y, int64_t ldy, const float* __restrict__ gamma,
                                                             const float* __restrict__ beta, float eps, int ln_mask,
                                                             TOut* __restrict__ ln_out, int64_t ld_ln, int rows) {
    const int row = blockIdx.x * 8 + (threadIdx.x >> 5), l = threadIdx.x & 31;
    if (row >= rows) return;
    const float mk = mask ? (mask[row] ? 1.f : 0.f) : 1.f;
    f32x4 v[3];
#pragma unroll
    for (int j = 0; j < 3; ++j)
        v[j] = x ? *reinterpret_cast<const f32x4*>(x + (int64_t)row * ldx + 4 * (l + 32 * j)) : f32x4{0.f, 0.f, 0.f, 0.f};
    for (int s = 0; s < splits; ++s) {
        const float* ps = part + (int64_t)s * part_stride + (int64_t)row * kD;
#pragma unroll
        for (int j = 0; j < 3; ++j) v[j] += *reinterpret_cast<const f32x4*>(ps + 4 * (l + 32 * j));
    }
    float sum = 0.f;
#pragma unroll
    for (int j = 0; j < 3; ++j) {
        v[j] *= mk;
        *reinterpret_cast<f32x4*>(y + (int64_t)row * ldy + 4 * (l + 32 * j)) = v[j];
        sum += (v[j][0] + v[j][1]) + (v[j][2] + v[j][3]);
    }
    if (!ln_out) return;
#pragma unroll
    for (int off = 16; off > 0; off >>= 1) sum += __shfl_xor(sum, off, 64);
    const float mean = sum * (1.0f / kD);
    float q = 0.f;
#pragma unroll
    for (int j = 0; j < 3; ++j)
#pragma unroll
        for (int e = 0; e < 4; ++e) {
            const float d = v[j][e] - mean;
            q = fmaf(d, d, q);
        }
#pragma unroll
    for (int off = 16; off > 0; off >>= 1) q += __shfl_xor(q, off, 64);
    const float rstd = 1.0f / sqrtf(q * (1.0f / kD) + eps), om = ln_mask ? mk : 1.f;
#pragma unroll
    for (int j = 0; j < 3; ++j) {
        const int c = 4 * (l + 32 * j);
        const f32x4 g = *reinterpret_cast<const f32x4*>(gamma + c), bt = *reinterpret_cast<const f32x4*>(beta + c);
        float o[4];
#pragma unroll
        for (int e = 0; e < 4; ++e) o[e] = ((v[j][e] - mean) * rstd * g[e] + bt[e]) * om;
        if constexpr (std::is_same<TOut, float>::value) {
            *reinterpret_cast<f32x4*>(ln_out + (int64_t)row * ld_ln + c) = f32x4{o[0], o[1], o[2], o[3]};
        } else {
            uint2 pk;
            pk.x = (uint32_t)f32_to_bf16(o[0]) | ((uint32_t)f32_to_bf16(o[1]) << 16);
            pk.y = (uint32_t)f32_to_bf16(o[2]) | ((uint32_t)f32_to_bf16(o[3]) << 16);
            *reinterpret_cast<uint2*>(ln_out + (int64_t)row * ld_ln + c) = pk;
        }
    }
}

struct Ffn2Entry {
    const char* name;
    int min_inner;
    uint32_t flags_ok;
    bool proj;
    bool out_optional = false;
    int32_t no_mask = ISPK_E_NULL;
};

static int32_t ffn2_check(const Ffn2Entry& e, const Ffn2Params& p, int32_t dim, bool more_present = true, bool more_shape = true,
                          bool more_aligned = true) {
    ISPK_REQUIRE(p.x && p.gamma && p.beta && p.W1 && p.W2c && (!e.proj || (p.o && p.WoC)) && (e.out_optional || p.out) && more_present,
                 ISPK_E_NULL, "%s: null pointer", e.name);
    ISPK_REQUIRE(dim == kD, ISPK_E_UNSUPPORTED, "%s: dim %d (built for 384)", e.name, dim);
    ISPK_REQUIRE(p.rows >= 0 && p.inner >= e.min_inner && p.inner % 32 == 0 && more_shape, ISPK_E_SHAPE,
                 "%s: bad shape rows=%d inner=%d (inner: a multiple of 32, at least %d; split: the chunks of 32 divide evenly among "
                 "the splits, >= 2 each, and part_stride >= rows * 384)", e.name, p.rows, p.inner, e.min_inner);
    ISPK_REQUIRE((p.flags & ~e.flags_ok) == 0, ISPK_E_UNSUPPORTED, "%s: unsupported flags", e.name);
    ISPK_REQUIRE(!(((p.flags & (ISPK_EP_MASK_OUT | ISPK_EP_MASK_ACC)) || p.ln_mask) && !p.mask), e.no_mask,
                 "%s: mask flag without mask", e.name);
    ISPK_REQUIRE(p.ldx % 4 == 0 && p.ldx >= dim && ispk_aligned(p.x, 16) && ispk_aligned(p.W1, 16) && ispk_aligned(p.W2c, 16) &&
                     ispk_aligned(p.gamma, 16) && ispk_aligned(p.beta, 16) &&
                     (!e.proj || (p.ld_o % 8 == 0 && p.ld_o >= dim && ispk_aligned(p.o, 16) && ispk_aligned(p.WoC, 16))) &&
                     (!p.out || (p.ldo % 4 == 0 && p.ldo >= dim && ispk_aligned(p.out, 16))) &&
                     (!p.stats || ispk_aligned(p.stats, 8)) && more_aligned,
                 ISPK_E_ALIGN, "%s: 16-byte alignment / strides that are multiples of 4 (fp32) and 8 (bf16) required", e.name);
    return 0;
}

template <int MODE>
static int32_t ffn2_launch(const Ffn2Params& p, dim3 grid, hipStream_t stream, const char* what) {
    static std::atomic<bool> reserved{false};
    if (!reserved.load(std::memory_order_acquire)) {
        const hipError_t e = hipFuncSetAttribute(reinterpret_cast<const void*>(&ffn2_bf16_kernel<MODE>),
                                                 hipFuncAttributeMaxDynamicSharedMemorySize, kLds);
        if (e != hipSuccess) ISPK_FAIL((int32_t)e, "%s: cannot reserve %d B of LDS: %s", what, kLds, hipGetErrorString(e));
        reserved.store(true, std::memory_order_release);
    }
    hipLaunchKernelGGL(ffn2_bf16_kernel<MODE>, grid, dim3(512), kLds, stream, p);
    return ispk_launch_status();
}

static bool ffn2_splits_ok(int32_t splits, int32_t rows, int32_t inner, int64_t part_stride) {
    return splits >= 1 && (inner / 32) % splits == 0 && (inner / 32) / splits >= 2 && part_stride >= (int64_t)rows * kD;
}

extern "C" int32_t ispk_ffn_bf16_prenorm2_split(const float* x, int64_t ldx, const float* norm_gamma, const float* norm_beta,
                                                float norm_eps, const uint16_t* W1, const uint16_t* W2_chunks, float* parts,
                                                int64_t part_stride, int32_t splits, int32_t rows, int32_t dim, int32_t inner,
                                                ispk_stream_t stream) {
    Ffn2Params p{x, ldx, norm_gamma, norm_beta, norm_eps, W1, W2_chunks, nullptr, parts, kD, rows, inner, 0u, nullptr, 0.f};
    if (int32_t rc = ffn2_check({"ffn_prenorm2_split", 32, 0u, false}, p, dim, true, ffn2_splits_ok(splits, rows, inner, part_stride),
                                part_stride % 4 == 0))
        return rc;
    if (rows == 0) return 0;
    p.chunk_count = (inner / 32) / splits;
    p.part_stride = part_stride;
    return ffn2_launch<kSplitMode>(p, dim3((rows + 127) / 128, splits), reinterpret_cast<hipStream_t>(stream), "ffn_prenorm2_split");
}

extern "C" int32_t ispk_attn_out_ffn_split_bf16(const float* x, int64_t ldx, const uint16_t* attn_out, int64_t ld_attn,
                                                const uint16_t* Wo_chunks, const float* norm_gamma, const float* norm_beta,
                                                float norm_eps, const uint16_t* W1, const uint16_t* W2_chunks,
                                                const uint8_t* mask, uint32_t flags, float* parts, int64_t part_stride,
                                                int32_t splits, int32_t rows, int32_t dim, int32_t inner, ispk_stream_t stream) {
    Ffn2Params p{x, ldx, norm_gamma, norm_beta, norm_eps, W1, W2_chunks, mask, parts, kD, rows, inner, flags, nullptr, 0.f};
    p.o = attn_out;
    p.ld_o = ld_attn;
    p.WoC = Wo_chunks;
    if (int32_t rc = ffn2_check({"attn_out_ffn_split", 32, ISPK_EP_MASK_ACC, true, false, ISPK_E_UNSUPPORTED}, p, dim, true,
                                ffn2_splits_ok(splits, rows, inner, part_stride), part_stride % 4 == 0))
        return rc;
    if (rows == 0) return 0;
    p.chunk_count = (inner / 32) / splits;
    p.part_stride = part_stride;
    return ffn2_launch<kSplitProjMode>(p, dim3((rows + 127) / 128, splits), reinterpret_cast<hipStream_t>(stream), "attn_out_ffn_split");
}

extern "C" int32_t ispk_ffn_combine_ln_f32(const float* x, int64_t ldx, const float* parts, int64_t part_stride, int32_t splits,
                                           const uint8_t* mask, float* y, int64_t ldy, const float* ln_gamma,
                                           const float* ln_beta, float ln_eps, int32_t ln_mask, void* ln_out, int64_t ld_ln,
                                           int32_t ln_bf16, int32_t rows, int32_t dim, ispk_stream_t stream) {
    ISPK_REQUIRE(parts && y, ISPK_E_NULL, "ffn_combine_ln: null pointer");
    if (!x) ldx = dim;
    ISPK_REQUIRE(dim == kD && rows >= 0 && splits >= 1 && ldx >= dim && ldy >= dim && ldx % 4 == 0 && ldy % 4 == 0 &&
                     part_stride % 4 == 0, ISPK_E_SHAPE, "ffn_combine_ln: bad shape rows=%d dim=%d splits=%d", rows, dim, splits);
    ISPK_REQUIRE(!ln_out || (ln_gamma && ln_beta && ld_ln >= dim && ld_ln % 4 == 0), ISPK_E_NULL,
                 "ffn_combine_ln: LayerNorm output without gamma / beta");
    ISPK_REQUIRE((!x || ispk_aligned(x, 16)) && ispk_aligned(parts, 16) && ispk_aligned(y, 16) && (!ln_out || ispk_aligned(ln_out, 8)),
                 ISPK_E_ALIGN, "ffn_combine_ln: 16-byte alignment required");
    if (rows == 0) return 0;
    hipStream_t s = reinterpret_cast<hipStream_t>(stream);
    const dim3 grid((rows + 7) / 8);
    if (ln_out && ln_bf16)
        hipLaunchKernelGGL(ffn_combine_ln_kernel<uint16_t>, grid, dim3(256), 0, s, x, ldx, parts, part_stride, splits, mask, y, ldy,
                           ln_gamma, ln_beta, ln_eps, ln_mask, static_cast<uint16_t*>(ln_out), ld_ln, rows);
    else
        hipLaunchKernelGGL(ffn_combine_ln_kernel<float>, grid, dim3(256), 0, s, x, ldx, parts, part_stride, splits, mask, y, ldy,
                           ln_gamma, ln_beta, ln_eps, ln_mask, static_cast<float*>(ln_out), ld_ln, rows);
    return ispk_launch_status();
}

static int32_t attn_out_ffn_launch(const float* x, int64_t ldx, const uint16_t* attn_out, int64_t ld_attn,
                                   const uint16_t* Wo_chunks, const float* norm_gamma, const float* norm_beta, float norm_eps,
                                   const uint16_t* W1, const uint16_t* W2_chunks, const uint8_t* mask, float* out, int64_t ldo,
                                   int32_t rows, int32_t dim, int32_t inner, uint32_t flags, float* row_stats, float stats_eps,
                                   const float* next_gamma, const float* next_beta, float next_eps, const uint16_t* Wqkv_chunks,
                                   uint16_t* qkv, int64_t ld_qkv, bool with_qkv, ispk_stream_t stream) {
    Ffn2Params p{x, ldx, norm_gamma, norm_beta, norm_eps, W1, W2_chunks, mask, out, ldo, rows, inner, flags, row_stats, stats_eps};
    p.o = attn_out;
    p.ld_o = ld_attn;
    p.WoC = Wo_chunks;
    if (int32_t rc = ffn2_check({"attn_out_ffn", 64, ISPK_EP_MASK_OUT | ISPK_EP_MASK_ACC, true}, p, dim)) return rc;
    if (with_qkv) {
        ISPK_REQUIRE(next_gamma && next_beta && Wqkv_chunks && qkv, ISPK_E_NULL, "attn_out_ffn_qkv: null pointer");
        ISPK_REQUIRE(ld_qkv >= kNq && ld_qkv % 8 == 0 && ispk_aligned(qkv, 16) && ispk_aligned(Wqkv_chunks, 16) &&
                         ispk_aligned(next_gamma, 16) && ispk_aligned(next_beta, 16),
                     ISPK_E_ALIGN, "attn_out_ffn_qkv: q/kv rows of 512 bf16, 16-byte aligned, row stride a multiple of 8");
    }
    if (rows == 0) return 0;
    const dim3 grid((rows + 127) / 128);
    hipStream_t s = reinterpret_cast<hipStream_t>(stream);
    if (!with_qkv) return ffn2_launch<kProjMode>(p, grid, s, "attn_out_ffn");
    p.gamma2 = next_gamma;
    p.beta2 = next_beta;
    p.eps2 = next_eps;
    p.WqC = Wqkv_chunks;
    p.qkv = qkv;
    p.ld_qkv = ld_qkv;
    return ffn2_launch<kProjQkvMode>(p, grid, s, "attn_out_ffn_qkv");
}

extern "C" int32_t ispk_attn_out_ffn_bf16(const float* x, int64_t ldx, const uint16_t* attn_out, int64_t ld_attn,
                                          const uint16_t* Wo_chunks, const float* norm_gamma, const float* norm_beta,
                                          float norm_eps, const uint16_t* W1, const uint16_t* W2_chunks, const uint8_t* mask,
                                          float* out, int64_t ldo, int32_t rows, int32_t dim, int32_t inner, uint32_t flags,
                                          float* row_stats, float stats_eps, ispk_stream_t stream) {
    return attn_out_ffn_launch(x, ldx, attn_out, ld_attn, Wo_chunks, norm_gamma, norm_beta, norm_eps, W1, W2_chunks, mask, out, ldo,
                               rows, dim, inner, flags, row_stats, stats_eps, nullptr, nullptr, 0.f, nullptr, nullptr, 0, false, stream);
}

extern "C" int32_t ispk_attn_out_ffn_norm_bf16(const float* x, int64_t ldx, const uint16_t* attn_out, int64_t ld_attn,
                                               const uint16_t* Wo_chunks, const float* norm_gamma, const float* norm_beta,
                                               float norm_eps, const uint16_t* W1, const uint16_t* W2_chunks, const uint8_t* mask,
                                               float* out, int64_t ldo, int32_t rows, int32_t dim, int32_t inner, uint32_t flags,
                                               const float* final_gamma, const float* final_beta, float final_eps, int32_t ln_mask,
                                               void* ln_out, int64_t ld_ln, int32_t ln_bf16, ispk_stream_t stream) {
    Ffn2Params p{x, ldx, norm_gamma, norm_beta, norm_eps, W1, W2_chunks, mask, out, ldo, rows, inner, flags, nullptr, 0.f};
    p.o = attn_out;
    p.ld_o = ld_attn;
    p.WoC = Wo_chunks;
    p.gamma2 = final_gamma;
// ... 50 lines not shown
```

### isp_tts_amd/csrc/norm.hip

```cpp
#include "common.h"

namespace {

template <typename OutT>
__device__ __forceinline__ void store_out(OutT* p, float v);
template <>
__device__ __forceinline__ void store_out<float>(float* p, float v) { *p = v; }
template <>
__device__ __forceinline__ void store_out<uint16_t>(uint16_t* p, float v) { *p = f32_to_bf16(v); }

template <int NV, typename OutT>
__global__ __launch_bounds__(256) void layernorm_kernel(const float* __restrict__ x, int64_t ldx,
                                                        const float* __restrict__ gamma, const float* __restrict__ beta,
                                                        const float* __restrict__ ada_scale,
                                                        const float* __restrict__ ada_shift, int64_t ada_stride,
                                                        int rows_per_batch, const uint8_t* __restrict__ row_mask,
                                                        OutT* __restrict__ y, int64_t ldy, int rows, float eps,
                                                        int64_t y_plane) {
    const int lane = threadIdx.x & 63;
    const int row = blockIdx.x * 4 + (threadIdx.x >> 6);
    if (row >= rows) return;
    constexpr int D = NV * 64;
    const float* xr = x + (int64_t)row * ldx;
    float v[NV];
    float s = 0.f;
#pragma unroll
    for (int c = 0; c < NV; ++c) {
        v[c] = xr[lane + 64 * c];
        s += v[c];
    }
    const float mean = wave_sum(s) * (1.0f / D);
    float ss = 0.f;
#pragma unroll
    for (int c = 0; c < NV; ++c) {
        const float d = v[c] - mean;
        ss += d * d;
    }
    const float rstd = 1.0f / sqrtf(wave_sum(ss) * (1.0f / D) + eps);
    const float mk = row_mask ? (row_mask[row] ? 1.0f : 0.0f) : 1.0f;
    const float* sc = gamma;
    const float* sh = beta;
    if (ada_scale) {
        const int64_t off = (int64_t)(row / rows_per_batch) * ada_stride;
        sc = ada_scale + off;
        sh = ada_shift ? ada_shift + off : nullptr;
    }
    OutT* yr = y + (int64_t)row * ldy;
#pragma unroll
    for (int c = 0; c < NV; ++c) {
        const int col = lane + 64 * c;
        float o = (v[c] - mean) * rstd;
        if (sc) o *= sc[col];
        if (sh) o += sh[col];
// ... 100 lines not shown
                           OutT* y, int64_t ldy, int32_t rows, int32_t D, float eps, ispk_stream_t stream,
                           int64_t y_plane = 0) {
    ISPK_REQUIRE(x && y, ISPK_E_NULL, "layernorm: null x/y");
    ISPK_REQUIRE(y_plane % 4 == 0 && (y_plane == 0 || sizeof(OutT) == 2), ISPK_E_ALIGN, "layernorm: y_plane %% 4 (split output)");
    ISPK_REQUIRE(rows >= 0 && D >= 64 && D <= 1024 && D % 64 == 0, ISPK_E_SHAPE,
                 "layernorm: D=%d must be a multiple of 64 in [64, 1024]", D);
    ISPK_REQUIRE(ldx >= D && ldy >= D, ISPK_E_SHAPE, "layernorm: leading stride < D");
    ISPK_REQUIRE(!ada_scale || rows_per_batch >= 1, ISPK_E_SHAPE, "layernorm: rows_per_batch must be >= 1");
    if (rows == 0) return 0;
    hipStream_t s = reinterpret_cast<hipStream_t>(stream);
    const bool vec_ok = D % 128 == 0 && D <= 512 && ldx % 4 == 0 && ldy % 4 == 0 && ispk_aligned(x, 16) &&
                        ispk_aligned(y, sizeof(OutT) * 4) && (!gamma || ispk_aligned(gamma, 16)) &&
                        (!beta || ispk_aligned(beta, 16)) &&
                        (!ada_scale || (ispk_aligned(ada_scale, 16) && ada_stride % 4 == 0)) &&
                        (!ada_shift || ispk_aligned(ada_shift, 16)) && ispk_knob("ISPK_LN_SCALAR") == nullptr;
    if (vec_ok) {
        dim3 grid8((rows + 7) / 8), block8(256);
#define ISPK_LNV_CASE(NV4)                                                                                               \
    case NV4:                                                                                                           \
        hipLaunchKernelGGL((layernorm_vec_kernel<NV4, OutT>), grid8, block8, 0, s, x, ldx, gamma, beta, ada_scale,      \
                           ada_shift, ada_stride, rows_per_batch, row_mask, y, ldy, rows, eps, y_plane);                \
        break;
        switch (D / 128) { ISPK_LNV_CASE(1) ISPK_LNV_CASE(2) ISPK_LNV_CASE(3) ISPK_LNV_CASE(4) }
#undef ISPK_LNV_CASE
        return ispk_launch_status();
    }
    dim3 grid((rows + 3) / 4), block(256);
#define ISPK_LN_CASE(NV)                                                                                              \
    case NV:                                                                                                          \
        hipLaunchKernelGGL((layernorm_kernel<NV, OutT>), grid, block, 0, s, x, ldx, gamma, beta, ada_scale, ada_shift, \
                           ada_stride, rows_per_batch, row_mask, y, ldy, rows, eps, y_plane);                         \
        break;
    switch (D / 64) {
        ISPK_LN_CASE(1) ISPK_LN_CASE(2) ISPK_LN_CASE(3) ISPK_LN_CASE(4) ISPK_LN_CASE(5) ISPK_LN_CASE(6)
        ISPK_LN_CASE(7) ISPK_LN_CASE(8) ISPK_LN_CASE(9) ISPK_LN_CASE(10) ISPK_LN_CASE(11) ISPK_LN_CASE(12)
        ISPK_LN_CASE(13) ISPK_LN_CASE(14) ISPK_LN_CASE(15) ISPK_LN_CASE(16)
        default: ISPK_FAIL(ISPK_E_SHAPE, "layernorm: unsupported D=%d", D);
    }
#undef ISPK_LN_CASE
    return ispk_launch_status();
}

__global__ __launch_bounds__(256) void linear_small_kernel(const float* __restrict__ a, int64_t lda,
                                                           const float* __restrict__ w, int64_t ldw,
                                                           const float* __restrict__ bias,
                                                           const float* __restrict__ resid, int64_t ldr,
                                                           float* __restrict__ out, int64_t ldo, int M, int N, int K,
                                                           uint32_t act) {
    const int64_t idx = (int64_t)blockIdx.x * 256 + threadIdx.x;
    if (idx >= (int64_t)M * N) return;
    const int i = (int)(idx / N), j = (int)(idx - (int64_t)i * N);
    const float* ar = a + (int64_t)i * lda;
    const float* wr = w + (int64_t)j * ldw;
    float acc = 0.f;
    int k = 0;
    for (; k + 8 <= K; k += 8) {
        float av[8], wv[8];
#pragma unroll
        for (int u = 0; u < 8; ++u) { av[u] = ar[k + u]; wv[u] = wr[k + u]; }
#pragma unroll
        for (int u = 0; u < 8; ++u) acc = fmaf(av[u], wv[u], acc);
    }
    if (k < K) {
        float av[8], wv[8];
#pragma unroll
        for (int u = 0; u < 7; ++u) {
            const int kk = k + u < K ? k + u : K - 1;
            av[u] = ar[kk];
            wv[u] = k + u < K ? wr[kk] : 0.0f;
        }
#pragma unroll
        for (int u = 0; u < 7; ++u) acc = fmaf(av[u], wv[u], acc);
    }
    if (bias) acc += bias[j];
    if (act & ISPK_EP_GELU) acc = gelu_erf(acc);
    if (act & ISPK_EP_SILU) acc = silu(acc);
    if (resid) acc += resid[(int64_t)i * ldr + j];
    out[(int64_t)i * ldo + j] = acc;
}

__global__ __launch_bounds__(256) void cast_bf16_kernel(const float* __restrict__ x, int64_t ldx,
                                                        uint16_t* __restrict__ y, int64_t ldy, int rows, int cols4) {
    const int64_t idx = (int64_t)blockIdx.x * 256 + threadIdx.x;
    if (idx >= (int64_t)rows * cols4) return;
    const int r = (int)(idx / cols4), c = (int)(idx - (int64_t)r * cols4) * 4;
    const float4 v = *reinterpret_cast<const float4*>(x + (int64_t)r * ldx + c);
    uint2 o;
    o.x = f32_to_bf16(v.x) | ((uint32_t)f32_to_bf16(v.y) << 16);
    o.y = f32_to_bf16(v.z) | ((uint32_t)f32_to_bf16(v.w) << 16);
    *reinterpret_cast<uint2*>(y + (int64_t)r * ldy + c) = o;
}

}

extern "C" int32_t ispk_layernorm_f32(const float* x, int64_t ldx, const float* gamma, const float* beta,
                                      const float* ada_scale, const float* ada_shift, int64_t ada_stride,
                                      int32_t rows_per_batch, const uint8_t* row_mask, float* y, int64_t ldy,
                                      int32_t rows, int32_t D, float eps, ispk_stream_t stream) {
    return layernorm_dispatch<float>(x, ldx, gamma, beta, ada_scale, ada_shift, ada_stride, rows_per_batch, row_mask, y,
                                     ldy, rows, D, eps, stream);
}

extern "C" int32_t ispk_layernorm_f32_bf16(const float* x, int64_t ldx, const float* gamma, const float* beta,
                                           const float* ada_scale, const float* ada_shift, int64_t ada_stride,
                                           int32_t rows_per_batch, const uint8_t* row_mask, uint16_t* y, int64_t ldy,
                                           int32_t rows, int32_t D, float eps, ispk_stream_t stream) {
    return layernorm_dispatch<uint16_t>(x, ldx, gamma, beta, ada_scale, ada_shift, ada_stride, rows_per_batch, row_mask,
                                        y, ldy, rows, D, eps, stream);
}

extern "C" int32_t ispk_layernorm_f32_split(const float* x, int64_t ldx, const float* gamma, const float* beta,
                                            const float* ada_scale, const float* ada_shift, int64_t ada_stride,
                                            int32_t rows_per_batch, const uint8_t* row_mask, uint16_t* y_hi, int64_t ldy,
                                            int64_t y_plane, int32_t rows, int32_t D, float eps, ispk_stream_t stream) {
    ISPK_REQUIRE(y_plane > 0, ISPK_E_SHAPE, "layernorm_split: y_plane must be positive");
    return layernorm_dispatch<uint16_t>(x, ldx, gamma, beta, ada_scale, ada_shift, ada_stride, rows_per_batch, row_mask,
                                        y_hi, ldy, rows, D, eps, stream, y_plane);
}

extern "C" int32_t ispk_linear_small_f32(const float* a, int64_t lda, const float* w, int64_t ldw, const float* bias,
                                         const float* resid, int64_t ldr, float* out, int64_t ldo, int32_t M, int32_t N,
                                         int32_t K, uint32_t act, ispk_stream_t stream) {
    ISPK_REQUIRE(a && w && out, ISPK_E_NULL, "linear_small: null pointer");
    ISPK_REQUIRE(M >= 0 && N >= 1 && K >= 1, ISPK_E_SHAPE, "linear_small: bad shape M=%d N=%d K=%d", M, N, K);
    ISPK_REQUIRE(lda >= K && ldw >= K && ldo >= N && (!resid || ldr >= N), ISPK_E_SHAPE, "linear_small: bad strides");
    if (M == 0) return 0;
// ... 19 lines not shown
```

### isp_tts_amd/modules/transformer/feedforward.py

```python
from __future__ import annotations

from dataclasses import dataclass
from typing import Optional

import torch
import torch.nn as nn
from torch import Tensor

from ... import runtime
from ...staging import StagedWeights
from ..constructor import Constructor, ModuleConfig
from . import plan
from .plan import Consumer, Form

_ACTS = {"gelu": runtime.EP_GELU, "swish": runtime.EP_SILU, "linear": 0}


@dataclass
class FeedForwardConfig(ModuleConfig):
    dim: int = 384
    inner_dim: int = 1536
    dropout: float = 0.0
    activation: str = "relu"
    bias: bool = False
# ... 10 lines not shown
        self.act_flag = _ACTS[activation]
        self.dropout_p = dropout
        self.net = nn.Sequential(nn.Linear(dim, inner_dim, bias=bias), nn.GELU() if activation == "gelu" else nn.Identity(),
                                 nn.Dropout(dropout) if dropout > 0. else nn.Identity(),
                                 nn.Linear(inner_dim, dim, bias=bias))
        self.compute_dtype = torch.float32
        self._cache = StagedWeights()

    def _staged(self, dtype: torch.dtype):
        ps = (self.net[0].weight, self.net[3].weight)
        if dtype == torch.float16:
            return self._cache.get(dtype, ps, lambda: (runtime.split_f16(ps[0].detach().float().contiguous()),
                                                       runtime.split_f16(ps[1].detach().float().contiguous())))
        if dtype == torch.bfloat16 and ps[0].is_cuda and ps[0].dtype == torch.float32:
            return self._cache.get(dtype, ps, lambda: (runtime.cast_bf16(ps[0].detach()), runtime.cast_bf16(ps[1].detach())))
        return self._cache.get(dtype, ps, lambda: (ps[0].detach().to(dtype).contiguous(),
                                                   ps[1].detach().to(dtype).contiguous()))

    def _packed_w2(self) -> Tensor:
        return self._cache.get("w2p", (self.net[3].weight,),
                               lambda: runtime.ffn_pack_w2(self._staged(torch.bfloat16)[1]))

    def _chunked_w2(self) -> Tensor:
        return self._cache.get("w2c", (self.net[3].weight,),
                               lambda: runtime.ffn_chunk_w2(self._staged(torch.bfloat16)[1]))


    def attn_out_ffn(self, x: Tensor, attn_out: Tensor, woc: Tensor, norm, mask: Optional[Tensor], form: Form,
                     consumer: Optional[Consumer] = None, store_out: bool = True):
        w1, _ = self._staged(torch.bfloat16)
        kw = {}
        if form is Form.ATTN_OUT_FFN_NORM:
            kw = dict(final_norm=(consumer.weight, consumer.bias, consumer.eps, consumer.apply_mask, consumer.dtype),
                      want_out=store_out)
        elif form is Form.ATTN_OUT_FFN_QKV:
            kw = dict(next_qkv=(consumer.weight, consumer.bias, consumer.eps, consumer.attention._chunked_wqkv()))
        elif form is Form.ATTN_OUT_FFN_STATS:
            kw = dict(want_stats=True, stats_eps=consumer.eps)
        res = runtime.attn_out_ffn(x, attn_out, woc, norm.weight, norm.bias, w1, self._chunked_w2(), mask=mask,
                                   norm_eps=norm.eps, **kw)
        return (res, None) if form is Form.ATTN_OUT_FFN else res

    def prenorm(self, x: Tensor, norm, mask: Optional[Tensor], pair: bool, stats_eps: Optional[float] = None):
        w1, _ = self._staged(torch.bfloat16)
        kw = dict(mask=mask, flags=runtime.EP_MASK_OUT if mask is not None else 0, norm_eps=norm.eps,
                  want_stats=stats_eps is not None, stats_eps=1e-5 if stats_eps is None else stats_eps)
        if pair:
            res = runtime.ffn_prenorm2(x, norm.weight, norm.bias, w1, self._chunked_w2(), **kw)
        else:
            res = runtime.ffn_prenorm(x, norm.weight, norm.bias, w1, self._packed_w2(), bias2=self.net[3].bias, **kw)
        return (res, None) if stats_eps is None else res

    def prenorm_split(self, x: Tensor, norm, mask: Optional[Tensor], splits: int, consumer: Optional[Consumer] = None,
                      dtype: Optional[torch.dtype] = None, attn_proj: Optional[tuple] = None):
        w1, _ = self._staged(torch.bfloat16)
        nn_ = None if consumer is None else (consumer.weight, consumer.bias, consumer.eps, consumer.apply_mask, dtype)
        return runtime.ffn_prenorm2_split(x, norm.weight, norm.bias, w1, self._chunked_w2(), mask, splits, next_norm=nn_,
                                          norm_eps=norm.eps, attn_proj=attn_proj)

    def lnin_gemm(self, x: Tensor, norm, mask: Optional[Tensor]) -> Tensor:
        w1, w2 = self._staged(torch.bfloat16)
        hidden = runtime.gemm_lnin(x, None, norm.weight, norm.bias, w1, bias=self.net[0].bias, flags=self.act_flag,
                                   ln_eps=norm.eps)
        return runtime.gemm(hidden, w2, bias=self.net[3].bias, resid=x, mask=mask,
                            flags=runtime.EP_MASK_OUT if mask is not None else 0, out_dtype=torch.float32)

    def forward(self, x: Tensor, *, residual: Optional[Tensor] = None, mask: Optional[Tensor] = None,
                fused: Optional[bool] = None) -> Tensor:
        if self.training and self.dropout_p > 0:
            raise NotImplementedError("feed-forward dropout (training) is outside the forward-path scope")
        dt = self.compute_dtype
        w1, w2 = self._staged(dt)
        flags = runtime.EP_MASK_OUT if mask is not None else 0
        if dt == torch.float16:
            xs = x if x.dtype == torch.float16 else runtime.split_f16(x.float().contiguous())
            hidden = runtime.gemm_split(xs, w1, bias=self.net[0].bias, flags=self.act_flag, out_split=True)
            return runtime.gemm_split(hidden, w2, bias=self.net[3].bias, resid=residual, mask=mask, flags=flags)
        if x.dtype != dt:
            x = runtime.cast_bf16(x) if dt == torch.bfloat16 else x.float()
        if fused is None:
            fused = plan.ffn_fused_ok(dt, self.act_flag == runtime.EP_GELU, x.shape[-1], x.numel() // x.shape[-1], plan.SEAMS)
        if fused:
            return runtime.ffn_fused(x, w1, self._packed_w2(), resid=residual, mask=mask, bias1=self.net[0].bias,
                                     bias2=self.net[3].bias, flags=flags)
        hidden = runtime.gemm(x, w1, bias=self.net[0].bias, flags=self.act_flag)
        return runtime.gemm(hidden, w2, bias=self.net[3].bias, resid=residual, mask=mask, flags=flags,
                            out_dtype=torch.float32)
```

### isp_tts_amd/modules/transformer/transformer.py

```python
from __future__ import annotations

from dataclasses import dataclass, field
from typing import NamedTuple, Optional, Union

import torch
import torch.nn as nn
from torch import Tensor

from ... import runtime
from ...staging import StagedWeights
from ..constructor import Constructor, ModuleConfig
from .attend import AttentionIntermediates
from .attention import Attention, AttentionConfig, AttentionSharedIntermediates
from .feedforward import FeedForward, FeedForwardConfig
from .normalization import AdaptiveLayerNorm, LayerNorm
from .plan import ATTN_OUT_FFN_FORMS, Consumer, Form, Hand, Handed, Next, Plan, Qkv, Seams, select_plan


class TransformerLayerIntermediates(NamedTuple):
    attention: Optional[AttentionIntermediates] = None


class TransformerLayerOutput(NamedTuple):
    out: Optional[Tensor]
    intermediates: Optional[TransformerLayerIntermediates] = None
    shared_intermediates: Optional[AttentionSharedIntermediates] = None
    handed: Handed = Handed()


@dataclass
class TransformerLayerConfig(ModuleConfig):
    dim: int = 384
    attention: Union[AttentionConfig, dict] = field(default_factory=AttentionConfig)
    feed_forward: Union[FeedForwardConfig, dict] = field(default_factory=FeedForwardConfig)
    pre_norm: bool = True
    adaptive_norm: bool = False
    condition_dim: Optional[int] = None


class TransformerLayer(nn.Module, Constructor):
    def __init__(self, dim: int = 384, attention=None, feed_forward=None, pre_norm: bool = True,
                 adaptive_norm: bool = False, condition_dim: Optional[int] = None):
        super().__init__()
        if not pre_norm:
            raise NotImplementedError("post-norm layers are unused by the recipes and not built")
        assert not adaptive_norm or condition_dim is not None
        self.pre_norm, self.adaptive_norm = pre_norm, adaptive_norm
        norm = (lambda: AdaptiveLayerNorm(dim, condition_dim=condition_dim)) if adaptive_norm else (lambda: LayerNorm(dim))
        self.attention_norm = norm()
        self.attention = Attention.init(attention if attention is not None else AttentionConfig(), dim=dim)
        self.feed_forward_norm = norm()
        self.feed_forward = FeedForward.init(feed_forward if feed_forward is not None else FeedForwardConfig(), dim=dim)

    def _plan(self, dim: int, rows: int, prev: Handed, consumer: Consumer, seams: Optional[Seams]) -> Plan:
        att, ff = self.attention, self.feed_forward
        plain = all(isinstance(n, nn.LayerNorm) and n.weight is not None and n.bias is not None
                    for n in (self.attention_norm, self.feed_forward_norm))
        nxt = consumer.attention
        return select_plan(cdt=att.compute_dtype, dim=dim, heads=att.heads, out_dim=att.out_dim, inner=ff.net[0].weight.shape[0],
                           rows=rows, plain_norms=plain, bias1=ff.net[0].bias is not None, bias2=ff.net[3].bias is not None,
                           gelu=ff.act_flag == runtime.EP_GELU, dropout=ff.training and ff.dropout_p > 0, prev=prev.kind,
                           consumer=consumer.kind, consumer_dtype=consumer.dtype, next_heads=nxt.heads if nxt is not None else 0,
                           next_dim=nxt.dim if nxt is not None else 0, only_normed=consumer.only_normed, seams=seams)

    def forward(self, x: Tensor, mask: Optional[Tensor] = None, context: Optional[Tensor] = None,
                context_mask: Optional[Tensor] = None, attention_mask: Optional[Tensor] = None,
                adaptive_condition: Optional[Tensor] = None, cache: Optional[TransformerLayerIntermediates] = None,
                shared_cache: Optional[AttentionSharedIntermediates] = None, *, key_len: Optional[Tensor] = None,
                ada: Optional[tuple] = None, prev: Handed = Handed(), consumer: Consumer = Consumer(),
                seams: Optional[Seams] = None):
        assert not self.adaptive_norm or adaptive_condition is not None or ada is not None, \
            "`adaptive_condition` should be provided for AdaptiveLayerNorm"
        if cache is not None:
            raise NotImplementedError("KV caches are not on the acoustic-model forward path")
        if context is not None or context_mask is not None or attention_mask is not None:
            raise NotImplementedError("cross-attention / explicit attention masks are not on the forward path")
        x = x.float().contiguous()
        if mask is not None and key_len is None:
            key_len = mask.sum(dim=1)
        att, ff, fn = self.attention, self.feed_forward, self.feed_forward_norm
        cdt = att.compute_dtype
        p = self._plan(x.shape[-1], x.numel() // x.shape[-1], prev, consumer, seams)

        def norm(n, t: Tensor, scale_shift: Optional[tuple], row_mask: Optional[Tensor] = None) -> Tensor:
            if cdt == torch.float16:
                return self._norm_split(n, t, adaptive_condition, scale_shift, row_mask)
            kw = {} if scale_shift is None else {"scale_shift": scale_shift}
            return n(t, adaptive_condition, row_mask=row_mask, out_dtype=cdt, **kw)

        qkv = None
        if p.qkv is Qkv.HANDED_QKV:
            qkv = prev.tensor
        elif p.qkv in (Qkv.LNIN_STATS, Qkv.LNIN_SELF):
            qkv = att.qkv_lnin(x, self.attention_norm, prev.tensor if p.qkv is Qkv.LNIN_STATS else None)
        h = x if qkv is not None else prev.tensor if p.qkv is Qkv.HANDED_ROWS else norm(self.attention_norm, x, ada and ada[0])
        x1, inter, shared = att(h, mask=mask, key_len=key_len, residual=x, qkv=qkv, defer_out=p.defer_out)

        second = None
        served = consumer if p.hands is not Hand.NONE else None
        if p.form in ATTN_OUT_FFN_FORMS:
            y, second = ff.attn_out_ffn(x, x1, att._chunked_wo(), fn, mask, p.form, served, p.store_out)
        elif p.form in (Form.FFN_PRENORM2, Form.FFN_PRENORM):
            y, second = ff.prenorm(x1, fn, mask, p.form is Form.FFN_PRENORM2, served.eps if served is not None else None)
        elif p.form is Form.SPLIT_PROJ:
            y, second = ff.prenorm_split(x, fn, mask, p.splits, served, p.hand_dtype, attn_proj=(x1, att._chunked_wo()))
        elif p.form is Form.SPLIT:
            y, second = ff.prenorm_split(x1, fn, mask, p.splits, served, p.hand_dtype)
        elif p.form is Form.LNIN_GEMM:
            y = ff.lnin_gemm(x1, fn, mask)
        else:
            y = ff(norm(fn, x1, ada and ada[1], mask), residual=x1, mask=mask, fused=p.form is Form.NORM_FFN_FUSED)
        return TransformerLayerOutput(out=y, intermediates=TransformerLayerIntermediates(attention=inter),
                                      shared_intermediates=shared, handed=Handed(p.hands, second))

    def _norm_split(self, norm, x: Tensor, condition: Optional[Tensor], scale_shift: Optional[tuple],
                    row_mask: Optional[Tensor]) -> Tensor:
        if isinstance(norm, AdaptiveLayerNorm):
            if scale_shift is None and condition is not None:
                cond = condition.reshape(-1, condition.shape[-1]).float().contiguous()
                scale_shift = (runtime.linear_small(cond, norm.weight.weight, norm.weight.bias),
                               runtime.linear_small(cond, norm.bias.weight, norm.bias.bias) if norm.bias is not None else None)
            if scale_shift is None:
                return runtime.layernorm_split(x, None, None, row_mask=row_mask, eps=norm.eps)
            rows_per_batch = x.numel() // (x.shape[0] * x.shape[-1])
            return runtime.layernorm_split(x, None, None, scale_shift[0], scale_shift[1], rows_per_batch, row_mask, norm.eps)
        return runtime.layernorm_split(x, norm.weight, norm.bias, row_mask=row_mask, eps=norm.eps)


class TransformerOutput(NamedTuple):
    out: Tensor
    intermediates: Optional[list] = None


@dataclass
class TransformerConfig(ModuleConfig):
    dim: int = 384
    depth: int = 6
    transformer_layer: Union[TransformerLayerConfig, dict] = field(default_factory=TransformerLayerConfig)
    emb_dim: Optional[int] = None
    use_abs_pos_emb: bool = True
    adaptive_norm: bool = False
    condition_dim: Optional[int] = None


class Transformer(nn.Module, Constructor):
    seams: Optional[Seams] = None

    def __init__(self, dim: int = 384, depth: int = 6, transformer_layer=None, emb_dim: Optional[int] = None,
                 use_abs_pos_emb: bool = True, adaptive_norm: bool = False, condition_dim: Optional[int] = None):
        super().__init__()
        self.dim = dim
        self.emb_dim = emb_dim = emb_dim or dim
        self.adaptive_norm = adaptive_norm
        layer_cfg = transformer_layer if transformer_layer is not None else TransformerLayerConfig()
        self.layers = nn.ModuleList([
            TransformerLayer.init(layer_cfg, dim=dim, adaptive_norm=adaptive_norm, condition_dim=condition_dim)
            for _ in range(depth)])
        if use_abs_pos_emb and self.layers[0].attention.rel_pos is None:
            raise NotImplementedError("absolute sinusoidal position embeddings (no ALiBi) are unused by the recipes")
        self.pos_emb = None
        self.project_emb = nn.Linear(emb_dim, dim) if emb_dim != dim else nn.Identity()
        self.norm = nn.LayerNorm(dim)
        self._ada_cache = StagedWeights()

    def _ada_all(self, condition: Tensor):
        norms = [n for layer in self.layers for n in (layer.attention_norm, layer.feed_forward_norm)]
        ps = [p for n in norms for p in (n.weight.weight, n.weight.bias, n.bias.weight, n.bias.bias)]

        def build():
            with torch.no_grad():
                return (torch.cat([torch.cat([n.weight.weight, n.bias.weight]) for n in norms]).contiguous(),
                        torch.cat([torch.cat([n.weight.bias, n.bias.bias]) for n in norms]).contiguous())
        w_all, b_all = self._ada_cache.get("ada", ps, build)
        cond = condition.reshape(-1, condition.shape[-1]).float().contiguous()
        proj = runtime.linear_small(cond, w_all, b_all)
        d = self.dim
        parts = [(proj[:, (2 * i) * d:(2 * i + 1) * d], proj[:, (2 * i + 1) * d:(2 * i + 2) * d])
                 for i in range(len(norms))]
        return [(parts[2 * li], parts[2 * li + 1]) for li in range(len(self.layers))]

    def set_compute_dtype(self, dtype: torch.dtype):
        assert dtype in (torch.float32, torch.bfloat16, torch.float16)
        for layer in self.layers:
            layer.attention.compute_dtype = dtype
            layer.feed_forward.compute_dtype = dtype
        return self

    def _consumer(self, li: int, mask: Optional[Tensor], out_dtype: torch.dtype, final_norm: bool) -> Consumer:
        if li + 1 < len(self.layers):
            nxt = self.layers[li + 1]
            c = Consumer(Next.LAYER, nxt.attention_norm.weight, nxt.attention_norm.bias, nxt.attention_norm.eps,
                         attention=nxt.attention)
        else:
            c = Consumer(Next.FINAL, self.norm.weight, self.norm.bias, self.norm.eps, mask is not None, out_dtype,
                         only_normed=True)
        served = not self.adaptive_norm and (li + 1 < len(self.layers) or final_norm)
        return c if served and c.weight is not None and c.bias is not None else Consumer()

    def forward(self, x: Tensor, mask: Optional[Tensor] = None, context: Optional[Tensor] = None,
                context_mask: Optional[Tensor] = None, attention_mask: Optional[Tensor] = None,
                adaptive_condition: Optional[Tensor] = None, return_intermediates: bool = False, *,
                key_len: Optional[Tensor] = None, projected: Optional[Tensor] = None,
                out_dtype: torch.dtype = torch.float32, final_norm: bool = True, handed: Handed = Handed()):
        if projected is not None:
            out = projected
        elif isinstance(self.project_emb, nn.Identity):
            out = x.float()
        else:
            out = runtime.linear(x.float(), self.project_emb.weight, self.project_emb.bias)
        if mask is not None and key_len is None:
            key_len = mask.sum(dim=1)
        intermediates = []
        ada = self._ada_all(adaptive_condition) if (self.adaptive_norm and adaptive_condition is not None) else None
        for li, layer in enumerate(self.layers):
            res = layer(out, mask=mask, context=context, context_mask=context_mask, attention_mask=attention_mask,
                        adaptive_condition=adaptive_condition, key_len=key_len, ada=None if ada is None else ada[li],
                        prev=handed, consumer=self._consumer(li, mask, out_dtype, final_norm), seams=self.seams)
            out, handed = res.out, res.handed
            if return_intermediates:
                intermediates.append(res.intermediates)
        if not final_norm:
            return TransformerOutput(out=out, intermediates=intermediates)
        if handed.kind is Hand.ROWS:
            normed = handed.tensor
        elif out_dtype == torch.float16:
            normed = runtime.layernorm_split(out, self.norm.weight, self.norm.bias, row_mask=mask, eps=self.norm.eps)
        else:
            normed = runtime.layernorm(out, self.norm.weight, self.norm.bias, row_mask=mask, eps=self.norm.eps,
                                       out_dtype=out_dtype)
        return TransformerOutput(out=normed, intermediates=intermediates)
```

Baseline: 16.87 million mel-frames/s.

## Fan out encoder final-norm into padded bf16 keys and fuse soft-average projection

The last encoder layer's FFN combine+LayerNorm kernel now also writes a channel-padded bf16 copy for the aligner key projection and a bf16 row copy for the flow predictor's condition projection. This removes the separate pad_rows and cast_bf16 launches. The soft average of pitch and energy is fused with the two-input embedding projection, so the embedding transformer receives the projected input directly. A flow_mix_targets path is also added but is disabled by default. Together these cut several small kernel launches and memory round trips, at the cost of more plumbing through the transformer and adaptor interfaces.

```diff
diff --git a/include/ispk.h b/include/ispk.h
--- a/include/ispk.h
+++ b/include/ispk.h
@@ -88,6 +88,11 @@
                                 const uint8_t* mask, float* y, int64_t ldy, const float* ln_gamma, const float* ln_beta,
                                 float ln_eps, int32_t ln_mask, void* ln_out, int64_t ld_ln, int32_t ln_bf16, int32_t rows,
                                 int32_t dim, ispk_stream_t stream);
+int32_t ispk_ffn_combine_ln_fan_f32(const float* x, int64_t ldx, const float* parts, int64_t part_stride, int32_t splits,
+                                    const uint8_t* mask, float* y, int64_t ldy, const float* ln_gamma, const float* ln_beta,
+                                    float ln_eps, int32_t ln_mask, float* ln_out, int64_t ld_ln, const int64_t* key_len,
+                                    int32_t positions, uint16_t* padded_bf16, uint16_t* rows_bf16, int64_t ld_rows, int32_t rows,
+                                    int32_t dim, ispk_stream_t stream);
 int32_t ispk_ffn_bf16_prenorm2(const float* x, int64_t ldx, const float* norm_gamma, const float* norm_beta, float norm_eps,
                                const uint16_t* W1, const uint16_t* W2_chunks, const uint8_t* mask, float* out, int64_t ldo,
                                int32_t rows, int32_t dim, int32_t inner, uint32_t flags, float* row_stats, float stats_eps,
@@ -157,6 +162,9 @@
 int32_t ispk_soft_average_f32(const float* attn_soft, const float* pitch, const float* energy, const int64_t* duration,
                               const int64_t* text_len, float* feats, int32_t B, int32_t M, int32_t L,
                               ispk_stream_t stream);
+int32_t ispk_soft_average_proj_f32(const float* attn_soft, const float* pitch, const float* energy, const int64_t* duration,
+                                   const int64_t* text_len, float* feats, const float* w, int64_t ldw, const float* bias,
+                                   float* proj, int64_t ldp, int32_t B, int32_t M, int32_t L, int32_t N, ispk_stream_t stream);
 
 int32_t ispk_flow_head_f32(const float* y, int64_t ldy, const float* norm_gamma, const float* norm_beta, float norm_eps,
                            const float* W, const float* bias, const float* flow, const float* x0, const uint8_t* mask,
@@ -182,6 +190,8 @@
                                        int32_t L, ispk_stream_t stream);
 int32_t ispk_flow_mix_f32(const float* x0, const float* x1, const float* t, float sigma, float* x_t, float* flow, int32_t B,
                           int32_t L, int32_t C, ispk_stream_t stream);
+int32_t ispk_flow_mix_targets_f32(const float* x0, const float* feats, const int64_t* duration, const float* t, float sigma,
+                                  float* x_t, float* flow, int32_t B, int32_t L, ispk_stream_t stream);
 int32_t ispk_flow_finish_f32(const float* pred_raw, const float* flow, const float* x0, const uint8_t* mask, float* pred,
                              float* duration, float* loss_ratio, float* loss_mean, int32_t B, int32_t L, int32_t C,
                              ispk_stream_t stream);
diff --git a/isp_tts_amd/acoustic/alignment.py b/isp_tts_amd/acoustic/alignment.py
--- a/isp_tts_amd/acoustic/alignment.py
+++ b/isp_tts_amd/acoustic/alignment.py
@@ -98,7 +98,8 @@
                                     out_dtype=dt)
         return runtime.conv5_padded(q, wq[2])
 
-    def forward(self, queries: Tensor, keys: Tensor, query_len: Tensor, key_len: Tensor, q_proj: Optional[Tensor] = None):
+    def forward(self, queries: Tensor, keys: Tensor, query_len: Tensor, key_len: Tensor, q_proj: Optional[Tensor] = None, *,
+                k_padded: Optional[Tensor] = None):
         if not self.attention_prior:
             raise NotImplementedError("the aligner is built with its diagonal prior (recipes: attention_prior default)")
         wk, _ = self._staged()
@@ -111,7 +112,10 @@
             k = runtime.conv5_padded_split(k, wk[1])
             q = q_proj if q_proj is not None else self.project_queries(queries, query_len)
             return runtime.aligner_scores(q, k, key_len, query_len, max_q, max_k)
-        k = runtime.pad_rows(keys.float(), key_len, channel_first=True, out_dtype=dt)
+        if k_padded is not None and dt == torch.bfloat16:
+            k = k_padded
+        else:
+            k = runtime.pad_rows(keys.float(), key_len, channel_first=True, out_dtype=dt)
         k = runtime.conv5_padded(k, wk[0], gelu)
         k = runtime.masked_instnorm(k, self.key_proj[0].norm.weight, self.key_proj[0].norm.bias, key_len, out_dtype=dt)
         k = runtime.conv5_padded(k, wk[1])
@@ -137,8 +141,8 @@
                                        attention_prior=attention_prior)
 
     def forward(self, mel: Tensor, enc_text: Tensor, mel_len: Tensor, text_len: Tensor,
-                q_proj: Optional[Tensor] = None, mas_stream=None) -> AlignerOutput:
-        attn_soft, attn_logits = self.attention(mel, enc_text, mel_len, text_len, q_proj=q_proj)
+                q_proj: Optional[Tensor] = None, mas_stream=None, *, k_padded: Optional[Tensor] = None) -> AlignerOutput:
+        attn_soft, attn_logits = self.attention(mel, enc_text, mel_len, text_len, q_proj=q_proj, k_padded=k_padded)
         if mas_stream is not None and attn_logits.is_cuda:
             mas_stream.wait_stream(torch.cuda.current_stream())
             with torch.cuda.stream(mas_stream):
diff --git a/isp_tts_amd/acoustic/model.py b/isp_tts_amd/acoustic/model.py
--- a/isp_tts_amd/acoustic/model.py
+++ b/isp_tts_amd/acoustic/model.py
@@ -48,6 +48,7 @@
         self.to_mel = nn.Linear(self.decoder.dim, mel_dim)
         self.token_qkv_table = True
         self.overlap_streams = True
+        self.encoder_fanout = True
         self._side_streams: dict = {}
         self.register_buffer("pitch_mean", torch.tensor(float(pitch_mean or 0.)))
         self.register_buffer("pitch_std", torch.tensor(float(pitch_std or 1.)))
@@ -138,14 +139,20 @@
             with torch.cuda.stream(side):
                 q_proj = self.aligner.attention.project_queries(mel, mel_len)
         token_emb, enc_mask, handed = self._embed(text, text_len)
-        enc_out = self.encoder(token_emb, mask=enc_mask, key_len=text_len, handed=handed).out
+        ad = self.temporal_adaptor
+        bf_keys = self.aligner.attention.compute_dtype == torch.bfloat16
+        bf_cond = ad.predictor.transformer.layers[0].attention.compute_dtype == torch.bfloat16 and speaker is None
+        fan = (text_len, bf_keys, bf_cond) if self.encoder_fanout and text.is_cuda and (bf_keys or bf_cond) else None
+        enc = self.encoder(token_emb, mask=enc_mask, key_len=text_len, handed=handed, fan=fan)
+        enc_out = enc.out
+        k_padded, cond_bf16 = enc.fanned if enc.fanned is not None else (None, None)
         if q_proj is not None:
             main.wait_stream(side)
             q_proj.record_stream(main)
         branch = side if q_proj is not None else None
         hard = not self.temporal_adaptor.soft_duration
         aligner_output = self.aligner(mel=mel, enc_text=enc_out.transpose(1, 2).detach(), mel_len=mel_len,
-                                      text_len=text_len, q_proj=q_proj, mas_stream=None if hard else branch)
+                                      text_len=text_len, q_proj=q_proj, mas_stream=None if hard else branch, k_padded=k_padded)
         if speaker is not None:
             enc_out = runtime.add_speaker(enc_out, self.speaker_embedding.weight, speaker)
         adaptor_output = self.temporal_adaptor(
@@ -153,7 +160,7 @@
             duration_target=aligner_output.attn_hard_duration, alignment=aligner_output.attn_soft,
             pitch_target_dense=pitch, energy_target_dense=energy, noise=flow_noise, time_steps=flow_time,
             enc_len=text_len, predictor_stream=branch, duration_sum=mel_len if branch is not None and not hard else None,
-            qkv_for=self._decoder_first())
+            qkv_for=self._decoder_first(), cond_bf16=cond_bf16)
         dec_len = adaptor_output.dec_lengths
         dec_mask = adaptor_output.dec_mask
         dec_out = self.decoder(adaptor_output.enc_out, mask=dec_mask, key_len=dec_len, out_dtype=self.compute_dtype,
diff --git a/isp_tts_amd/acoustic/temporal_adaptor.py b/isp_tts_amd/acoustic/temporal_adaptor.py
--- a/isp_tts_amd/acoustic/temporal_adaptor.py
+++ b/isp_tts_amd/acoustic/temporal_adaptor.py
@@ -32,10 +32,10 @@
         return self._cache.get(dtype, (w,), lambda: w.detach().to(dtype).contiguous())
 
     def forward(self, x: Tensor, mask: Optional[Tensor] = None, *, key_len: Optional[Tensor] = None,
-                residual: Optional[Tensor] = None) -> Tensor:
+                residual: Optional[Tensor] = None, projected: Optional[Tensor] = None) -> Tensor:
         m2 = mask[..., 0] if mask is not None else None
         cdt = self.transformer.layers[0].attention.compute_dtype
-        out = self.transformer(x, mask=m2, out_dtype=cdt, key_len=key_len if m2 is not None else None).out
+        out = self.transformer(x, mask=m2, out_dtype=cdt, key_len=key_len if m2 is not None else None, projected=projected).out
         flags = runtime.EP_MASK_ACC if m2 is not None else 0
         if cdt == torch.float16:
             return runtime.gemm_split(out, self._weight(cdt), bias=self.linear_layer.bias, mask=m2, flags=flags, resid=residual)
@@ -71,29 +71,33 @@
         w = self.transformer.project_emb.weight
         return runtime.linear_small(x_t.contiguous(), w[:, :self.output_dim], None, resid=cond_proj)
 
-    def _cond_projection(self, cond: Tensor) -> Tensor:
+    def _cond_projection(self, cond: Tensor, cond_bf16: Optional[Tensor] = None) -> Tensor:
         cdt = self.transformer.layers[0].attention.compute_dtype
         c = cond.float().contiguous()
         if cdt == torch.float16:
             return runtime.gemm_split(runtime.split_f16(c), self._cond_weight(cdt), bias=self.transformer.project_emb.bias)
         if cdt == torch.bfloat16:
-            c = runtime.cast_bf16(c)
+            c = cond_bf16 if cond_bf16 is not None else runtime.cast_bf16(c)
         return runtime.gemm(c, self._cond_weight(cdt), bias=self.transformer.project_emb.bias, out_dtype=torch.float32)
 
-    def forward(self, x: Tensor, targets: Tensor, mask: Optional[Tensor] = None, *, noise: Optional[Tensor] = None,
-                time_steps: Optional[Tensor] = None, key_len: Optional[Tensor] = None):
+    def forward(self, x: Tensor, targets: Optional[Tensor], mask: Optional[Tensor] = None, *, noise: Optional[Tensor] = None,
+                time_steps: Optional[Tensor] = None, key_len: Optional[Tensor] = None, cond_bf16: Optional[Tensor] = None,
+                target_parts: Optional[tuple] = None):
         cond = x
         have_mask = mask is not None
         if mask is None:
             mask = torch.ones(x.shape[:2], dtype=torch.bool, device=x.device)
         elif mask.ndim == 3:
             mask = mask[..., 0]
-        x1 = targets.detach()
+        x1 = (targets if targets is not None else target_parts[0]).detach()
         x0 = torch.randn_like(x1) if noise is None else noise.to(x1)
         t = torch.rand((x1.shape[0],), dtype=x1.dtype, device=x1.device) if time_steps is None else time_steps.to(x1)
         time_emb = self.time_embedding(t)
-        x_t, flow = runtime.flow_mix(x0, x1, t, self.sigma)
-        proj = self._project(x_t, self._cond_projection(cond))
+        if targets is None:
+            x_t, flow = runtime.flow_mix_targets(x0, x1, target_parts[1], t, self.sigma)
+        else:
+            x_t, flow = runtime.flow_mix(x0, x1, t, self.sigma)
+        proj = self._project(x_t, self._cond_projection(cond, cond_bf16))
         tr = self.transformer
         head = (self.fused_head and tr.dim == 256 and self.output_dim == 3 and tr.norm.weight is not None and tr.norm.bias is not None
                 and self.linear_layer.bias is not None)
@@ -226,6 +230,8 @@
 
 class FlowTemporalAdaptor(nn.Module, Constructor):
     predictor_first = False
+    average_projects = True
+    mix_targets = False
 
     def __init__(self, encoder_dim: int = 384, predictor=None, embedding=None, pitch: bool = True, energy: bool = True,
                  soft_duration: bool = False):
@@ -251,7 +257,8 @@
                 alignment: Optional[Tensor] = None, pitch_target_dense: Optional[Tensor] = None,
                 energy_target_dense: Optional[Tensor] = None, *, noise: Optional[Tensor] = None,
                 time_steps: Optional[Tensor] = None, enc_len: Optional[Tensor] = None,
-                predictor_stream=None, duration_sum: Optional[Tensor] = None, qkv_for=None) -> TemporalAdaptorOutput:
+                predictor_stream=None, duration_sum: Optional[Tensor] = None, qkv_for=None,
+                cond_bf16: Optional[Tensor] = None) -> TemporalAdaptorOutput:
         assert duration_target is not None and (alignment is not None or not self.soft_duration)
         assert pitch_target_dense is not None and energy_target_dense is not None
         hard = not self.soft_duration
@@ -260,6 +267,7 @@
             enc_len = enc_mask.sum(dim=1)
         side = predictor_stream if (predictor_stream is not None and enc_out.is_cuda) else None
         cond = enc_out
+        projected = target_parts = None
         if hard:
             alignment = None
             targets = runtime.hard_average(pitch_target_dense, energy_target_dense, duration_target, enc_len)
@@ -270,9 +278,17 @@
             feats = targets
             len_src = duration_target
         else:
-            feats = runtime.soft_average(alignment, pitch_target_dense, energy_target_dense, None, enc_len)
+            emb = self.embedding.transformer
+            bf16 = emb.layers[0].attention.compute_dtype == torch.bfloat16
+            if self.average_projects and bf16 and isinstance(emb.project_emb, nn.Linear) and emb.project_emb.in_features == 2:
+                feats, projected = runtime.soft_average_proj(alignment, pitch_target_dense, energy_target_dense, enc_len,
+                                                             emb.project_emb.weight, emb.project_emb.bias)
+            else:
+                feats = runtime.soft_average(alignment, pitch_target_dense, energy_target_dense, None, enc_len)
             targets = None
             len_src = duration_sum.view(-1, 1)
+            if self.mix_targets and self.predictor.transformer.layers[0].attention.compute_dtype == torch.bfloat16:
+                target_parts = (feats, duration_target)
         if side is not None:
             ready = torch.cuda.Event()
             ready.record()
@@ -280,7 +296,8 @@
         features = feats[..., 1:3]
 
         def decoder_input(enc_out_):
-            enc_out_ = self.embedding(features, mask=m3, key_len=enc_len, residual=enc_out_)
+            enc_out_ = self.embedding(features, mask=m3, key_len=enc_len, residual=enc_out_,
+                                      projected=projected)
             return self.length_regulator(enc_out_, len_src, max_len=max_dec_len, alignment=alignment,
                                          frames=max_dec_len if hard else None, qkv_for=qkv_for)
 
@@ -289,16 +306,17 @@
 
         def predict():
             tg = targets
-            if tg is None:
+            if tg is None and target_parts is None:
                 tg = runtime.soft_average(alignment, pitch_target_dense, energy_target_dense, duration_target, enc_len)
-            pred_, losses_ = self.predictor(cond, tg, m3, noise=noise, time_steps=time_steps, key_len=enc_len)
+            pred_, losses_ = self.predictor(cond, tg, m3, noise=noise, time_steps=time_steps, key_len=enc_len, cond_bf16=cond_bf16,
+                                            target_parts=target_parts if tg is None else None)
             return pred_, losses_, self.predictor._duration_estimate
 
         if side is not None:
             side.wait_event(ready)
             with torch.cuda.stream(side):
                 pred, losses, duration_pred = predict()
-            for t in (cond, feats, alignment, pitch_target_dense, energy_target_dense):
+            for t in (cond, cond_bf16, feats, alignment, pitch_target_dense, energy_target_dense):
                 if t is not None:
                     t.record_stream(side)
             if self.predictor_first:
diff --git a/isp_tts_amd/bindings/adaptor.py b/isp_tts_amd/bindings/adaptor.py
--- a/isp_tts_amd/bindings/adaptor.py
+++ b/isp_tts_amd/bindings/adaptor.py
@@ -5,7 +5,7 @@
 
 from .. import runtime as _rt
 
-__all__ = ["mas", "pad_rows", "conv5_padded", "masked_instnorm", "aligner_scores", "soft_average", "flow_mix", "flow_finish",
+__all__ = ["mas", "pad_rows", "conv5_padded", "masked_instnorm", "aligner_scores", "soft_average", "soft_average_proj", "flow_mix", "flow_mix_targets", "flow_finish",
            "flow_head", "flow_euler", "infer_features", "infer_features_items", "infer_features_tokens", "embed_tokens", "embed_tokens_qkv", "_speaker_ids", "add_speaker_",
            "add_speaker", "speaker_grad", "time_embedding", "length_regulate", "_hard_durations", "hard_regulate",
            "hard_regulate_bwd", "hard_average"]
@@ -100,6 +100,35 @@
                 pitch.contiguous().data_ptr(), energy.contiguous().data_ptr(), _rt._ptr(dur),
                 _rt._i64(text_len).data_ptr(), feats.data_ptr(), B, M, L, _rt._stream())
     return feats
+
+
+def soft_average_proj(attn_soft: Tensor, pitch: Tensor, energy: Tensor, text_len: Tensor, w: Tensor, bias: Optional[Tensor]):
+    _rt._dev(attn_soft, pitch, energy, text_len, w, bias)
+    assert w.dtype == torch.float32 and w.ndim == 2 and w.shape[1] == 2 and w.stride(1) == 1
+    B, M, L = attn_soft.shape
+    N = w.shape[0]
+    feats = torch.empty((B, L, 3), dtype=torch.float32, device=attn_soft.device)
+    proj = torch.empty((B, L, N), dtype=torch.float32, device=attn_soft.device)
+    if B == 0:
+        return feats, proj
+    _rt._launch("soft_average_proj_kernel", 4.0 * B * L * N, 4.0 * B * (M * L + L * N), _rt.lib().ispk_soft_average_proj_f32,
+                attn_soft.contiguous().data_ptr(), pitch.contiguous().data_ptr(), energy.contiguous().data_ptr(), None,
+                _rt._i64(text_len).data_ptr(), feats.data_ptr(), w.data_ptr(), w.stride(0), _rt._ptr(bias), proj.data_ptr(), N,
+                B, M, L, N, _rt._stream())
+    return feats, proj
+
+
+def flow_mix_targets(x0: Tensor, feats: Tensor, duration: Tensor, t: Tensor, sigma: float):
+    _rt._dev(x0, feats, duration, t)
+    B, L, C = feats.shape
+    assert C == 3 and feats.dtype == torch.float32 and tuple(duration.shape) == (B, L)
+    x0c, fc, tc, dur = x0.float().contiguous(), feats.contiguous(), t.float().contiguous(), _rt._i64(duration)
+    xt, flow = torch.empty_like(fc), torch.empty_like(fc)
+    if B == 0:
+        return xt, flow
+    _rt._launch("flow_mix_targets_kernel", 0.0, 4.0 * B * L * (4 * C + 2), _rt.lib().ispk_flow_mix_targets_f32, x0c.data_ptr(),
+                fc.data_ptr(), dur.data_ptr(), tc.data_ptr(), float(sigma), xt.data_ptr(), flow.data_ptr(), B, L, _rt._stream())
+    return xt, flow
 
 
 def flow_mix(x0: Tensor, x1: Tensor, t: Tensor, sigma: float):
diff --git a/isp_tts_amd/bindings/layers.py b/isp_tts_amd/bindings/layers.py
--- a/isp_tts_amd/bindings/layers.py
+++ b/isp_tts_amd/bindings/layers.py
@@ -187,7 +187,8 @@
 
 
 def ffn_prenorm2_split(x: Tensor, norm_weight: Tensor, norm_bias: Tensor, w1: Tensor, w2c: Tensor, mask: Optional[Tensor],
-                       splits: int, next_norm: Optional[tuple] = None, norm_eps: float = 1e-5, attn_proj: Optional[tuple] = None):
+                       splits: int, next_norm: Optional[tuple] = None, norm_eps: float = 1e-5, attn_proj: Optional[tuple] = None,
+                       fan: Optional[tuple] = None):
     _rt._dev(x, norm_weight, norm_bias, w1, w2c, mask)
     assert x.dtype == torch.float32 and w1.dtype == torch.bfloat16 and w2c.dtype == torch.bfloat16
     x2 = _rt._rows2d(x)
@@ -210,7 +211,7 @@
         _rt._launch("ffn2_bf16_kernel<20>", 4.0 * R * D * Fi, float(nbytes), _rt.lib().ispk_ffn_bf16_prenorm2_split, x2.data_ptr(),
                     x2.stride(0), norm_weight.data_ptr(), norm_bias.data_ptr(), norm_eps, w1.data_ptr(), w2c.data_ptr(),
                     parts.data_ptr(), R * D, splits, R, D, Fi, _rt._stream())
-    y = torch.empty(x.shape, dtype=torch.float32, device=x.device)
+    y = torch.empty(x.shape, dtype=torch.float32, device=x.device) if fan is None or fan[3] else None
     mask = _rt._mask1d(mask)
     ln = None
     nw = nb = None
@@ -219,6 +220,20 @@
         nw, nb, neps, apply_mask, ndtype = next_norm
         ln = torch.empty(x.shape, dtype=ndtype, device=x.device)
         nmask, nbf16 = int(bool(apply_mask) and mask is not None), int(ndtype == torch.bfloat16)
+    if fan is not None:
+        key_len, want_padded, want_rows, want_y = fan
+        assert ln is not None and ln.dtype == torch.float32 and x.ndim == 3
+        _rt._dev(key_len)
+        B, N = x.shape[:2]
+        key_len = _rt._i64(key_len)
+        padded = torch.empty((B, N + 4, D), dtype=torch.bfloat16, device=x.device) if want_padded else None
+        rows16 = torch.empty(x.shape, dtype=torch.bfloat16, device=x.device) if want_rows else None
+        _rt._launch("ffn_combine_ln_fan_kernel", 0.0,
+                    float(R * D * 4 * (2 + int(want_y) + splits) + R * D * 2 * (int(want_padded) + int(want_rows))),
+                    _rt.lib().ispk_ffn_combine_ln_fan_f32, None if attn_proj is not None else x2.data_ptr(), x2.stride(0),
+                    parts.data_ptr(), R * D, splits, _rt._ptr(mask), _rt._ptr(y), D, nw.data_ptr(), nb.data_ptr(), neps, nmask,
+                    ln.data_ptr(), D, key_len.data_ptr(), N, _rt._ptr(padded), _rt._ptr(rows16), D, R, D, _rt._stream())
+        return y, ln, padded, rows16
     _rt._launch("ffn_combine_ln_kernel", 0.0, float(R * D * 4 * (2 + splits) + (R * D * ln.element_size() if ln is not None else 0)),
                 _rt.lib().ispk_ffn_combine_ln_f32, None if attn_proj is not None else x2.data_ptr(), x2.stride(0), parts.data_ptr(), R * D,
                 splits, _rt._ptr(mask), y.data_ptr(),
diff --git a/isp_tts_amd/csrc/aligner.hip b/isp_tts_amd/csrc/aligner.hip
--- a/isp_tts_amd/csrc/aligner.hip
+++ b/isp_tts_amd/csrc/aligner.hip
@@ -1,5 +1,6 @@
 #include "common.h"
 #include "dec_len.h"
+#include "seam_core.h"
 
 namespace {
 
@@ -347,12 +348,21 @@
 }
 
 constexpr int kSaLanes = 16;
+struct SaProj {
+    const float* w;
+    int64_t ldw;
+    const float* bias;
+    float* out;
+    int64_t ldo;
+    int N;
+};
+template <bool kProj>
 __global__ __launch_bounds__(64 * kSaLanes) void soft_average_kernel(const float* __restrict__ attn,
                                                                      const float* __restrict__ pitch,
                                                                      const float* __restrict__ energy,
                                                                      const int64_t* __restrict__ dur,
                                                                      const int64_t* __restrict__ text_len,
-                                                                     float* __restrict__ feats, int M, int L) {
+                                                                     float* __restrict__ feats, int M, int L, SaProj pj) {
     __shared__ float red[3][kSaLanes][64];
     const int b = blockIdx.y, j = threadIdx.x & 63, l = blockIdx.x * 64 + j, ml = threadIdx.x >> 6;
     const bool ok = l < L;
@@ -398,9 +408,39 @@
         }
         const float mk = l < (int)text_len[b] ? 1.0f : 0.0f;
         float* f = feats + ((int64_t)b * L + l) * 3;
-        f[0] = dur ? log1pf((float)dur[(int64_t)b * L + l]) : 0.0f;
-        f[1] = pp / (a + 1e-5f) * mk;
-        f[2] = ee / (a + 1e-5f) * mk;
+        const float f1 = pp / (a + 1e-5f) * mk, f2 = ee / (a + 1e-5f) * mk;
+        f[0] = dur ? log1p_duration(dur[(int64_t)b * L + l]) : 0.0f;
+        f[1] = f1;
+        f[2] = f2;
+        if constexpr (kProj) {
+            red[0][0][j] = f1;
+            red[0][1][j] = f2;
+        }
+    }
+    if constexpr (kProj) {
+        __syncthreads();
+        constexpr int kThreads = 64 * kSaLanes;
+        const int cols = min(64, L - (int)blockIdx.x * 64);
+        float* ob = pj.out + ((int64_t)b * L + blockIdx.x * 64) * pj.ldo;
+        if (kThreads % pj.N == 0) {
+            const int n = threadIdx.x % pj.N;
+            const float wr[2] = {pj.w[(int64_t)n * pj.ldw], pj.w[(int64_t)n * pj.ldw + 1]};
+            const float bn = pj.bias ? pj.bias[n] : 0.f;
+            for (int col = threadIdx.x / pj.N; col < cols; col += kThreads / pj.N) {
+                const float ar[2] = {red[0][0][col], red[0][1][col]};
+                float acc = linear_small_dot(ar, wr, 2);
+                if (pj.bias) acc += bn;
+                ob[(int64_t)col * pj.ldo + n] = acc;
+            }
+        } else {
+            for (int idx = threadIdx.x; idx < cols * pj.N; idx += kThreads) {
+                const int col = idx / pj.N, n = idx - col * pj.N;
+                const float ar[2] = {red[0][0][col], red[0][1][col]};
+                float acc = linear_small_dot(ar, pj.w + (int64_t)n * pj.ldw, 2);
+                if (pj.bias) acc += pj.bias[n];
+                ob[(int64_t)col * pj.ldo + n] = acc;
+            }
+        }
     }
 }
 
@@ -408,15 +448,20 @@
 __global__ __launch_bounds__(256) void flow_mix_kernel(const float* __restrict__ x0, const float* __restrict__ x1,
                                                        const float* __restrict__ t, float s, float* __restrict__ xt,
                                                        float* __restrict__ flow, int per_batch, int64_t total) {
-#pragma clang fp contract(off)
     const int64_t i = (int64_t)blockIdx.x * 256 + threadIdx.x;
     if (i >= total) return;
-    const float tb = t[i / per_batch], a = x0[i], b = x1[i];
-    const float w0 = 1.0f - s * tb;
-    const float p0 = w0 * a, p1 = tb * b;
-    xt[i] = p0 + p1;
-    const float sa = s * a;
-    flow[i] = b - sa;
+    flow_mix_one(x0[i], x1[i], t[i / per_batch], s, xt + i, flow + i);
+}
+
+__global__ __launch_bounds__(256) void flow_mix_targets_kernel(const float* __restrict__ x0, const float* __restrict__ feats,
+                                                               const int64_t* __restrict__ dur, const float* __restrict__ t, float s,
+                                                               float* __restrict__ xt, float* __restrict__ flow, int per_batch,
+                                                               int64_t total) {
+    const int64_t i = (int64_t)blockIdx.x * 256 + threadIdx.x;
+    if (i >= total) return;
+    const int64_t row = i / 3;
+    const float x1 = i - row * 3 == 0 ? log1p_duration(dur[row]) : feats[i];
+    flow_mix_one(x0[i], x1, t[i / per_batch], s, xt + i, flow + i);
 }
 
 __global__ __launch_bounds__(1024) void flow_finish_kernel(const float* __restrict__ raw, const float* __restrict__ flow,
@@ -784,8 +829,25 @@
     ISPK_REQUIRE(attn_soft && pitch && energy && text_len && feats, ISPK_E_NULL, "soft_average: null pointer");
     ISPK_REQUIRE(B >= 0 && M >= 1 && L >= 1 && B <= 65535, ISPK_E_SHAPE, "soft_average: bad shape B=%d M=%d L=%d", B, M, L);
     if (B == 0) return 0;
-    hipLaunchKernelGGL(soft_average_kernel, dim3((L + 63) / 64, B), dim3(64 * kSaLanes), 0, reinterpret_cast<hipStream_t>(stream),
-                       attn_soft, pitch, energy, duration, text_len, feats, M, L);
+    hipLaunchKernelGGL(soft_average_kernel<false>, dim3((L + 63) / 64, B), dim3(64 * kSaLanes), 0,
+                       reinterpret_cast<hipStream_t>(stream), attn_soft, pitch, energy, duration, text_len, feats, M, L, SaProj{});
+    return ispk_launch_status();
+}
+
+extern "C" int32_t ispk_soft_average_proj_f32(const float* attn_soft, const float* pitch, const float* energy,
+                                              const int64_t* duration, const int64_t* text_len, float* feats, const float* w,
+                                              int64_t ldw, const float* bias, float* proj, int64_t ldp, int32_t B, int32_t M,
+                                              int32_t L, int32_t N, ispk_stream_t stream) {
+    ISPK_REQUIRE(attn_soft && pitch && energy && text_len && feats && w && proj, ISPK_E_NULL, "soft_average_proj: null pointer");
+    ISPK_REQUIRE(B >= 0 && M >= 1 && L >= 1 && B <= 65535 && N >= 1 && N <= 4096, ISPK_E_SHAPE,
+                 "soft_average_proj: bad shape B=%d M=%d L=%d N=%d", B, M, L, N);
+    ISPK_REQUIRE(ldw >= 2 && ldp >= N, ISPK_E_SHAPE, "soft_average_proj: bad strides (weight rows of >= 2, output rows of >= %d)", N);
+    ISPK_REQUIRE(ispk_aligned(w, 4) && ispk_aligned(proj, 4) && ispk_aligned(feats, 4) && (!bias || ispk_aligned(bias, 4)),
+                 ISPK_E_ALIGN, "soft_average_proj: 4-byte alignment required");
+    if (B == 0) return 0;
+    hipLaunchKernelGGL(soft_average_kernel<true>, dim3((L + 63) / 64, B), dim3(64 * kSaLanes), 0,
+                       reinterpret_cast<hipStream_t>(stream), attn_soft, pitch, energy, duration, text_len, feats, M, L,
+                       SaProj{w, ldw, bias, proj, ldp, N});
     return ispk_launch_status();
 }
 
@@ -798,6 +860,20 @@
     const float s = (float)(1.0 - (double)sigma);
     hipLaunchKernelGGL(flow_mix_kernel, dim3((unsigned)((total + 255) / 256)), dim3(256), 0,
                        reinterpret_cast<hipStream_t>(stream), x0, x1, t, s, x_t, flow, L * C, total);
+    return ispk_launch_status();
+}
+
+extern "C" int32_t ispk_flow_mix_targets_f32(const float* x0, const float* feats, const int64_t* duration, const float* t,
+                                             float sigma, float* x_t, float* flow, int32_t B, int32_t L, ispk_stream_t stream) {
+    ISPK_REQUIRE(x0 && feats && duration && t && x_t && flow, ISPK_E_NULL, "flow_mix_targets: null pointer");
+    ISPK_REQUIRE(B >= 0 && L >= 1, ISPK_E_SHAPE, "flow_mix_targets: bad shape B=%d L=%d", B, L);
+    ISPK_REQUIRE(ispk_aligned(x0, 4) && ispk_aligned(feats, 4) && ispk_aligned(duration, 8) && ispk_aligned(t, 4) &&
+                     ispk_aligned(x_t, 4) && ispk_aligned(flow, 4), ISPK_E_ALIGN, "flow_mix_targets: unaligned pointer");
+    if (B == 0) return 0;
+    const int64_t total = (int64_t)B * L * 3;
+    const float s = (float)(1.0 - (double)sigma);
+    hipLaunchKernelGGL(flow_mix_targets_kernel, dim3((unsigned)((total + 255) / 256)), dim3(256), 0,
+                       reinterpret_cast<hipStream_t>(stream), x0, feats, duration, t, s, x_t, flow, L * 3, total);
     return ispk_launch_status();
 }
 
diff --git a/isp_tts_amd/csrc/ffn2.hip b/isp_tts_amd/csrc/ffn2.hip
--- a/isp_tts_amd/csrc/ffn2.hip
+++ b/isp_tts_amd/csrc/ffn2.hip
@@ -816,12 +816,19 @@
     return ispk_launch_status();
 }
 
-template <typename TOut>
+struct CombineFan {
+    uint16_t* padded;
+    const int64_t* key_len;
+    int n;
+    uint16_t* rows_bf16;
+    int64_t ld_rows;
+};
+template <typename TOut, bool kFan = false>
 __global__ __launch_bounds__(256) void ffn_combine_ln_kernel(const float* __restrict__ x, int64_t ldx, const float* __restrict__ part,
                                                              int64_t part_stride, int splits, const uint8_t* __restrict__ mask,
                                                              float* __restrict__ y, int64_t ldy, const float* __restrict__ gamma,
                                                              const float* __restrict__ beta, float eps, int ln_mask,
-                                                             TOut* __restrict__ ln_out, int64_t ld_ln, int rows) {
+                                                             TOut* __restrict__ ln_out, int64_t ld_ln, int rows, CombineFan fan) {
     const int row = blockIdx.x * 8 + (threadIdx.x >> 5), l = threadIdx.x & 31;
     if (row >= rows) return;
     const float mk = mask ? (mask[row] ? 1.f : 0.f) : 1.f;
@@ -838,7 +845,7 @@
 #pragma unroll
     for (int j = 0; j < 3; ++j) {
         v[j] *= mk;
-        *reinterpret_cast<f32x4*>(y + (int64_t)row * ldy + 4 * (l + 32 * j)) = v[j];
+        if (!kFan || y) *reinterpret_cast<f32x4*>(y + (int64_t)row * ldy + 4 * (l + 32 * j)) = v[j];
         sum += (v[j][0] + v[j][1]) + (v[j][2] + v[j][3]);
     }
     if (!ln_out) return;
@@ -856,6 +863,15 @@
 #pragma unroll
     for (int off = 16; off > 0; off >>= 1) q += __shfl_xor(q, off, 64);
     const float rstd = 1.0f / sqrtf(q * (1.0f / kD) + eps), om = ln_mask ? mk : 1.f;
+    int fb = 0, ft = 0;
+    bool keep = false;
+    if constexpr (kFan) {
+        if (fan.padded) {
+            fb = row / fan.n;
+            ft = row - fb * fan.n;
+            keep = ft < (int)fan.key_len[fb];
+        }
+    }
 #pragma unroll
     for (int j = 0; j < 3; ++j) {
         const int c = 4 * (l + 32 * j);
@@ -863,6 +879,28 @@
         float o[4];
 #pragma unroll
         for (int e = 0; e < 4; ++e) o[e] = ((v[j][e] - mean) * rstd * g[e] + bt[e]) * om;
+        if constexpr (kFan) {
+            uint2 pk;
+            pk.x = (uint32_t)f32_to_bf16(o[0]) | ((uint32_t)f32_to_bf16(o[1]) << 16);
+            pk.y = (uint32_t)f32_to_bf16(o[2]) | ((uint32_t)f32_to_bf16(o[3]) << 16);
+            if (fan.rows_bf16) *reinterpret_cast<uint2*>(fan.rows_bf16 + (int64_t)row * fan.ld_rows + c) = pk;
+            if (fan.padded) {
+                const uint2 zero{0u, 0u};
+                uint2 kept;
+                kept.x = keep ? pk.x : 0u;
+                kept.y = keep ? pk.y : 0u;
+                uint16_t* item = fan.padded + (int64_t)fb * (fan.n + 4) * kD + c;
+                *reinterpret_cast<uint2*>(item + (int64_t)(ft + 2) * kD) = kept;
+                if (ft == 0) {
+                    *reinterpret_cast<uint2*>(item) = zero;
+                    *reinterpret_cast<uint2*>(item + kD) = zero;
+                }
+                if (ft == fan.n - 1) {
+                    *reinterpret_cast<uint2*>(item + (int64_t)(fan.n + 2) * kD) = zero;
+                    *reinterpret_cast<uint2*>(item + (int64_t)(fan.n + 3) * kD) = zero;
+                }
+            }
+        }
         if constexpr (std::is_same<TOut, float>::value) {
             *reinterpret_cast<f32x4*>(ln_out + (int64_t)row * ld_ln + c) = f32x4{o[0], o[1], o[2], o[3]};
         } else {
@@ -969,10 +1007,37 @@
     const dim3 grid((rows + 7) / 8);
     if (ln_out && ln_bf16)
         hipLaunchKernelGGL(ffn_combine_ln_kernel<uint16_t>, grid, dim3(256), 0, s, x, ldx, parts, part_stride, splits, mask, y, ldy,
-                           ln_gamma, ln_beta, ln_eps, ln_mask, static_cast<uint16_t*>(ln_out), ld_ln, rows);
+                           ln_gamma, ln_beta, ln_eps, ln_mask, static_cast<uint16_t*>(ln_out), ld_ln, rows, CombineFan{});
     else
         hipLaunchKernelGGL(ffn_combine_ln_kernel<float>, grid, dim3(256), 0, s, x, ldx, parts, part_stride, splits, mask, y, ldy,
-                           ln_gamma, ln_beta, ln_eps, ln_mask, static_cast<float*>(ln_out), ld_ln, rows);
+                           ln_gamma, ln_beta, ln_eps, ln_mask, static_cast<float*>(ln_out), ld_ln, rows, CombineFan{});
+    return ispk_launch_status();
+}
+
+extern "C" int32_t ispk_ffn_combine_ln_fan_f32(const float* x, int64_t ldx, const float* parts, int64_t part_stride, int32_t splits,
+                                               const uint8_t* mask, float* y, int64_t ldy, const float* ln_gamma,
+                                               const float* ln_beta, float ln_eps, int32_t ln_mask, float* ln_out, int64_t ld_ln,
+                                               const int64_t* key_len, int32_t positions, uint16_t* padded_bf16,
+                                               uint16_t* rows_bf16, int64_t ld_rows, int32_t rows, int32_t dim,
+                                               ispk_stream_t stream) {
+    ISPK_REQUIRE(parts && ln_out && ln_gamma && ln_beta && (!padded_bf16 || key_len), ISPK_E_NULL,
+                 "ffn_combine_ln_fan: null pointer");
+    if (!x) ldx = dim;
+    if (!y) ldy = dim;
+    if (!rows_bf16) ld_rows = dim;
+    ISPK_REQUIRE(dim == kD && rows >= 0 && splits >= 1 && ldx >= dim && ldy >= dim && ld_ln >= dim && ld_rows >= dim &&
+                     ldx % 4 == 0 && ldy % 4 == 0 && ld_ln % 4 == 0 && ld_rows % 4 == 0 && part_stride % 4 == 0 &&
+                     (!padded_bf16 || (positions >= 1 && rows % positions == 0)),
+                 ISPK_E_SHAPE, "ffn_combine_ln_fan: bad shape rows=%d dim=%d splits=%d positions=%d (rows: whole items)", rows, dim,
+                 splits, positions);
+    ISPK_REQUIRE((!x || ispk_aligned(x, 16)) && ispk_aligned(parts, 16) && (!y || ispk_aligned(y, 16)) && ispk_aligned(ln_out, 16) &&
+                     ispk_aligned(ln_gamma, 16) && ispk_aligned(ln_beta, 16) && (!padded_bf16 || ispk_aligned(padded_bf16, 8)) &&
+                     (!rows_bf16 || ispk_aligned(rows_bf16, 8)) && (!key_len || ispk_aligned(key_len, 8)),
+                 ISPK_E_ALIGN, "ffn_combine_ln_fan: 16-byte alignment required (bf16 outputs: 8)");
+    if (rows == 0) return 0;
+    hipLaunchKernelGGL((ffn_combine_ln_kernel<float, true>), dim3((rows + 7) / 8), dim3(256), 0, reinterpret_cast<hipStream_t>(stream),
+                       x, ldx, parts, part_stride, splits, mask, y, ldy, ln_gamma, ln_beta, ln_eps, ln_mask, ln_out, ld_ln, rows,
+                       CombineFan{padded_bf16, key_len, positions, rows_bf16, ld_rows});
     return ispk_launch_status();
 }
 
diff --git a/isp_tts_amd/csrc/norm.hip b/isp_tts_amd/csrc/norm.hip
--- a/isp_tts_amd/csrc/norm.hip
+++ b/isp_tts_amd/csrc/norm.hip
@@ -1,4 +1,5 @@
 #include "common.h"
+#include "seam_core.h"
 
 namespace {
 
@@ -205,26 +206,7 @@
     const int i = (int)(idx / N), j = (int)(idx - (int64_t)i * N);
     const float* ar = a + (int64_t)i * lda;
     const float* wr = w + (int64_t)j * ldw;
-    float acc = 0.f;
-    int k = 0;
-    for (; k + 8 <= K; k += 8) {
-        float av[8], wv[8];
-#pragma unroll
-        for (int u = 0; u < 8; ++u) { av[u] = ar[k + u]; wv[u] = wr[k + u]; }
-#pragma unroll
-        for (int u = 0; u < 8; ++u) acc = fmaf(av[u], wv[u], acc);
-    }
-    if (k < K) {
-        float av[8], wv[8];
-#pragma unroll
-        for (int u = 0; u < 7; ++u) {
-            const int kk = k + u < K ? k + u : K - 1;
-            av[u] = ar[kk];
-            wv[u] = k + u < K ? wr[kk] : 0.0f;
-        }
-#pragma unroll
-        for (int u = 0; u < 7; ++u) acc = fmaf(av[u], wv[u], acc);
-    }
+    float acc = linear_small_dot(ar, wr, K);
     if (bias) acc += bias[j];
     if (act & ISPK_EP_GELU) acc = gelu_erf(acc);
     if (act & ISPK_EP_SILU) acc = silu(acc);
diff --git a/isp_tts_amd/csrc/seam_core.h b/isp_tts_amd/csrc/seam_core.h
--- /dev/null
+++ b/isp_tts_amd/csrc/seam_core.h
@@ -0,0 +1,38 @@
+#pragma once
+#include <hip/hip_runtime.h>
+#include <stdint.h>
+
+__device__ __forceinline__ float linear_small_dot(const float* __restrict__ ar, const float* __restrict__ wr, int K) {
+    float acc = 0.f;
+    int k = 0;
+    for (; k + 8 <= K; k += 8) {
+        float av[8], wv[8];
+#pragma unroll
+        for (int u = 0; u < 8; ++u) { av[u] = ar[k + u]; wv[u] = wr[k + u]; }
+#pragma unroll
+        for (int u = 0; u < 8; ++u) acc = fmaf(av[u], wv[u], acc);
+    }
+    if (k < K) {
+        float av[8], wv[8];
+#pragma unroll
+        for (int u = 0; u < 7; ++u) {
+            const int kk = k + u < K ? k + u : K - 1;
+            av[u] = ar[kk];
+            wv[u] = k + u < K ? wr[kk] : 0.0f;
+        }
+#pragma unroll
+        for (int u = 0; u < 7; ++u) acc = fmaf(av[u], wv[u], acc);
+    }
+    return acc;
+}
+
+__device__ __forceinline__ float log1p_duration(int64_t dur) { return log1pf((float)dur); }
+
+__device__ __forceinline__ void flow_mix_one(float a, float b, float tb, float s, float* __restrict__ xt, float* __restrict__ flow) {
+#pragma clang fp contract(off)
+    const float w0 = 1.0f - s * tb;
+    const float p0 = w0 * a, p1 = tb * b;
+    *xt = p0 + p1;
+    const float sa = s * a;
+    *flow = b - sa;
+}
diff --git a/isp_tts_amd/modules/transformer/feedforward.py b/isp_tts_amd/modules/transformer/feedforward.py
--- a/isp_tts_amd/modules/transformer/feedforward.py
+++ b/isp_tts_amd/modules/transformer/feedforward.py
@@ -86,11 +86,11 @@
         return (res, None) if stats_eps is None else res
 
     def prenorm_split(self, x: Tensor, norm, mask: Optional[Tensor], splits: int, consumer: Optional[Consumer] = None,
-                      dtype: Optional[torch.dtype] = None, attn_proj: Optional[tuple] = None):
+                      dtype: Optional[torch.dtype] = None, attn_proj: Optional[tuple] = None, fan: Optional[tuple] = None):
         w1, _ = self._staged(torch.bfloat16)
         nn_ = None if consumer is None else (consumer.weight, consumer.bias, consumer.eps, consumer.apply_mask, dtype)
         return runtime.ffn_prenorm2_split(x, norm.weight, norm.bias, w1, self._chunked_w2(), mask, splits, next_norm=nn_,
-                                          norm_eps=norm.eps, attn_proj=attn_proj)
+                                          norm_eps=norm.eps, attn_proj=attn_proj, fan=fan)
 
     def lnin_gemm(self, x: Tensor, norm, mask: Optional[Tensor]) -> Tensor:
         w1, w2 = self._staged(torch.bfloat16)
diff --git a/isp_tts_amd/modules/transformer/transformer.py b/isp_tts_amd/modules/transformer/transformer.py
--- a/isp_tts_amd/modules/transformer/transformer.py
+++ b/isp_tts_amd/modules/transformer/transformer.py
@@ -26,6 +26,7 @@
     intermediates: Optional[TransformerLayerIntermediates] = None
     shared_intermediates: Optional[AttentionSharedIntermediates] = None
     handed: Handed = Handed()
+    fanned: Optional[tuple] = None
 
 
 @dataclass
@@ -68,7 +69,7 @@
                 adaptive_condition: Optional[Tensor] = None, cache: Optional[TransformerLayerIntermediates] = None,
                 shared_cache: Optional[AttentionSharedIntermediates] = None, *, key_len: Optional[Tensor] = None,
                 ada: Optional[tuple] = None, prev: Handed = Handed(), consumer: Consumer = Consumer(),
-                seams: Optional[Seams] = None):
+                seams: Optional[Seams] = None, fan: Optional[tuple] = None):
         assert not self.adaptive_norm or adaptive_condition is not None or ada is not None, \
             "`adaptive_condition` should be provided for AdaptiveLayerNorm"
         if cache is not None:
@@ -96,22 +97,29 @@
         h = x if qkv is not None else prev.tensor if p.qkv is Qkv.HANDED_ROWS else norm(self.attention_norm, x, ada and ada[0])
         x1, inter, shared = att(h, mask=mask, key_len=key_len, residual=x, qkv=qkv, defer_out=p.defer_out)
 
-        second = None
+        second = fanned = None
         served = consumer if p.hands is not Hand.NONE else None
+        if not (fan is not None and p.form in (Form.SPLIT, Form.SPLIT_PROJ) and p.hands is Hand.ROWS
+                and p.hand_dtype == torch.float32 and x.ndim == 3):
+            fan = None
+        elif fan is not None:
+            fan = (*fan, not consumer.only_normed)
         if p.form in ATTN_OUT_FFN_FORMS:
             y, second = ff.attn_out_ffn(x, x1, att._chunked_wo(), fn, mask, p.form, served, p.store_out)
         elif p.form in (Form.FFN_PRENORM2, Form.FFN_PRENORM):
             y, second = ff.prenorm(x1, fn, mask, p.form is Form.FFN_PRENORM2, served.eps if served is not None else None)
         elif p.form is Form.SPLIT_PROJ:
-            y, second = ff.prenorm_split(x, fn, mask, p.splits, served, p.hand_dtype, attn_proj=(x1, att._chunked_wo()))
+            y, second, *fanned = ff.prenorm_split(x, fn, mask, p.splits, served, p.hand_dtype, attn_proj=(x1, att._chunked_wo()),
+                                                  fan=fan)
         elif p.form is Form.SPLIT:
-            y, second = ff.prenorm_split(x1, fn, mask, p.splits, served, p.hand_dtype)
+            y, second, *fanned = ff.prenorm_split(x1, fn, mask, p.splits, served, p.hand_dtype, fan=fan)
         elif p.form is Form.LNIN_GEMM:
             y = ff.lnin_gemm(x1, fn, mask)
         else:
             y = ff(norm(fn, x1, ada and ada[1], mask), residual=x1, mask=mask, fused=p.form is Form.NORM_FFN_FUSED)
         return TransformerLayerOutput(out=y, intermediates=TransformerLayerIntermediates(attention=inter),
-                                      shared_intermediates=shared, handed=Handed(p.hands, second))
+                                      shared_intermediates=shared, handed=Handed(p.hands, second),
+                                      fanned=tuple(fanned) if fanned else None)
 
     def _norm_split(self, norm, x: Tensor, condition: Optional[Tensor], scale_shift: Optional[tuple],
                     row_mask: Optional[Tensor]) -> Tensor:
@@ -130,6 +138,7 @@
 class TransformerOutput(NamedTuple):
     out: Tensor
     intermediates: Optional[list] = None
+    fanned: Optional[tuple] = None
 
 
 @dataclass
@@ -201,7 +210,8 @@
                 context_mask: Optional[Tensor] = None, attention_mask: Optional[Tensor] = None,
                 adaptive_condition: Optional[Tensor] = None, return_intermediates: bool = False, *,
                 key_len: Optional[Tensor] = None, projected: Optional[Tensor] = None,
-                out_dtype: torch.dtype = torch.float32, final_norm: bool = True, handed: Handed = Handed()):
+                out_dtype: torch.dtype = torch.float32, final_norm: bool = True, handed: Handed = Handed(),
+                fan: Optional[tuple] = None):
         if projected is not None:
             out = projected
         elif isinstance(self.project_emb, nn.Identity):
@@ -215,15 +225,16 @@
         for li, layer in enumerate(self.layers):
             res = layer(out, mask=mask, context=context, context_mask=context_mask, attention_mask=attention_mask,
                         adaptive_condition=adaptive_condition, key_len=key_len, ada=None if ada is None else ada[li],
-                        prev=handed, consumer=self._consumer(li, mask, out_dtype, final_norm), seams=self.seams)
+                        prev=handed, consumer=self._consumer(li, mask, out_dtype, final_norm), seams=self.seams,
+                        fan=fan if li + 1 == len(self.layers) and final_norm else None)
             out, handed = res.out, res.handed
             if return_intermediates:
                 intermediates.append(res.intermediates)
         if not final_norm:
             return TransformerOutput(out=out, intermediates=intermediates)
         if handed.kind is Hand.ROWS:
-            normed = handed.tensor
-        elif out_dtype == torch.float16:
+            return TransformerOutput(out=handed.tensor, intermediates=intermediates, fanned=res.fanned)
+        if out_dtype == torch.float16:
             normed = runtime.layernorm_split(out, self.norm.weight, self.norm.bias, row_mask=mask, eps=self.norm.eps)
         else:
             normed = runtime.layernorm(out, self.norm.weight, self.norm.bias, row_mask=mask, eps=self.norm.eps,
```

Result: no change. 16.85 million mel-frames/s (-0.1%).
